# jhollowed/PyTEMDiags

Hardware: AMD Instinct MI355X
Metric: grid-points/sec through full TEM pipeline (ncol*nlev*nt) (higher is better)
Workload: dtype f64; 1 GPU; ne120 (777602 cols) x 72 lev x 30 snapshots per GPU, L=50, 1-degree zonal grid (M=180), ten GM16 Table-A1 outputs; ncol=777602, nlev=72, nt=30, sweeps=latitude-class, single sweep, mirror_paired_sweeps=True

## Files before the change

### include/temx.h

```cpp
#ifndef TEMX_H
#define TEMX_H

#include <stdint.h>

#ifdef __cplusplus
extern "C" {
#endif

typedef struct temx_plan temx_plan;

enum { TEMX_F64 = 0, TEMX_F32 = 1 };

enum {
  TEMX_OK = 0,
  TEMX_EINVAL = -1,
  TEMX_EHIP = -2,
  TEMX_ENOMEM = -3,
  TEMX_ERANK = -4,
  TEMX_ESTATE = -5,
  TEMX_EUNSUPPORTED = -6,
  TEMX_EINTERNAL = -7
};

enum {
  TEMX_DEFER_FINALIZE = 1,
  TEMX_NO_SYMMETRY = 2,
  TEMX_NO_CLASSES = 4,
  TEMX_NO_QR = 8,
  TEMX_LAT_TOL_F32 = 16
};

enum {
  TEMX_OPT_FORM = 1,
  TEMX_OPT_OS_MAP = 2,
  TEMX_OPT_OP_MAP = 3,
  TEMX_OPT_OS_SUBSAMPLE = 4,
  TEMX_OPT_TRACER_ONE_PASS = 5,
  TEMX_OPT_SINGLE_SWEEP_MIN_GROUPS = 6,
  TEMX_OPT_OS_CONTRACT = 7,
  TEMX_OPT_MISSING = 8,
  TEMX_OPT_MIN_COVERAGE = 9,
  TEMX_OPT_MISSING_WEIGHT = 10,
  TEMX_OPT_LAT_BINS = 12,
  TEMX_OPT_BIN_DEGREE = 13,
  TEMX_OPT_OS_SYNC = 11
};
enum {
  TEMX_FORM_AUTO = -1,
  TEMX_FORM_TWO_PASS = 0,
  TEMX_FORM_CLASS_SUMS = 1,
  TEMX_FORM_SINGLE_SWEEP = 2,
  TEMX_FORM_NO_SINGLE_SWEEP = 3,
  TEMX_FORM_MASKED = 4,
  TEMX_FORM_BINNED = 5
};

enum {
  TEMX_MAT_Y0 = 0,
  TEMX_MAT_Y0P = 1,
  TEMX_MAT_GRAM = 2,
  TEMX_MAT_GINV = 3,
  TEMX_MAT_Y0INV = 4,
  TEMX_MAT_GRAM2 = 5,
  TEMX_MAT_GX = 6,
  TEMX_MAT_GSUB = 7,
  TEMX_MAT_COVERAGE = 8
};

enum {
  TEMX_R_VTEM = 0, TEMX_R_OMEGATEM, TEMX_R_WTEM, TEMX_R_PSITEM, TEMX_R_EPFY, TEMX_R_EPFZ,
  TEMX_R_EPDIV, TEMX_R_UTENDEPFD, TEMX_R_UTENDVTEM, TEMX_R_UTENDWTEM, TEMX_NRESULTS
};

enum {
  TEMX_Z_UB = 0, TEMX_Z_VB, TEMX_Z_THETAB, TEMX_Z_WAPB, TEMX_Z_UPVPB, TEMX_Z_UPWAPPB,
  TEMX_Z_VPTPB, TEMX_Z_DUB_DP, TEMX_Z_DTHETAB_DP, TEMX_Z_UBCOSLAT, TEMX_Z_DUBCOSLAT_DLAT,
  TEMX_Z_PSI, TEMX_Z_PSICOSLAT, TEMX_Z_DPSICOSLAT_DLAT, TEMX_Z_DPSI_DP, TEMX_Z_INT_VBDP,
  TEMX_NZONAL
};

enum {
  TEMX_E_UP = 0, TEMX_E_VP, TEMX_E_THETAP, TEMX_E_WAPP, TEMX_E_UPVP, TEMX_E_UPWAPP, TEMX_E_VPTP,
  TEMX_NEDDY
};

int temx_version(void);
const char* temx_last_error(void);
int temx_device_count(void);

int temx_plan_create(temx_plan** out, int device, int64_t ncol, int L, int M,
                     const double* lat_deg_host, const double* lat_out_deg_host, int flags);

int temx_plan_finalize(temx_plan* plan, const double* G_host );

int temx_plan_refine(temx_plan* plan, const double* G2_host );

int temx_plan_set_weights(temx_plan* plan, const double* weights_host );

void temx_plan_destroy(temx_plan* plan);

int temx_plan_is_paired(const temx_plan* plan);
int temx_plan_sweep_mode(const temx_plan* plan);
int temx_plan_one_pass(const temx_plan* plan);
int temx_plan_single_sweep(const temx_plan* plan);

int temx_get_matrix(temx_plan* plan, int which, double* dst, void* stream);

int temx_plan_configure(temx_plan* plan, int option, int value);
int temx_plan_option(const temx_plan* plan, int option);

int temx_plan_set_os_matrices(temx_plan* plan, const double* Gx_host , const double* Gsub_host );


int temx_project(temx_plan* plan, const void* A, int dtype, int64_t D, double* B, void* stream);

int temx_zonal_mean(temx_plan* plan, const void* A, int dtype, int64_t D, double* out,
                    int native, void* stream);

int temx_zonal_mean_from_sums(temx_plan* plan, const double* B, int64_t D, double* out,
                              int native, void* stream);

int temx_plan_set_tem(temx_plan* plan, int nlev, int64_t nt, const double* p_pa_host, double p0);

int temx_tem_stage1(temx_plan* plan, const void* ua, const void* va, const void* ta,
                    const void* wap, int dtype, double* B4, void* stream);

int temx_tem_stage2(temx_plan* plan, const void* ua, const void* va, const void* ta,
                    const void* wap, int dtype, const double* B4, double* B3, void* stream);

int temx_tem_stage2_from_sums(temx_plan* plan, const double* B4, double* B3, void* stream);

int temx_tem_stage3(temx_plan* plan, const double* B3, double* results, double* zonal,
                    void* stream);

int temx_tem_run(temx_plan* plan, const void* ua, const void* va, const void* ta,
                 const void* wap, int dtype, double* results, double* zonal, void* stream);

int temx_tem_os_prepass(temx_plan* plan, const void* ua, const void* va, const void* ta, const void* wap, int dtype,
                        double* As, void* stream);
int temx_tem_os_sweep(temx_plan* plan, const void* ua, const void* va, const void* ta, const void* wap, int dtype,
                      const double* As, int nslices, double* proj, void* stream);
int temx_tem_os_tail(temx_plan* plan, const double* proj_slice, int64_t t0, int64_t nts, double* results,
                     double* zonal, void* stream);
int temx_tracers_os_prepass(temx_plan* plan, int nq, const void* const* q_host, const void* va, const void* wap,
                            int dtype, double* Asq, void* stream);
int temx_tracers_os_sweep(temx_plan* plan, int nq, const void* const* q_host, const void* va, const void* wap,
                          int dtype, const double* Asq, int nslices, double* projq, void* stream);
int temx_tracers_os_tail(temx_plan* plan, int nq, const double* projq_slice, double* const* tres_host,
                         double* const* tzon_host, void* stream);

int temx_tem_tail_from_sums(temx_plan* plan, const double* B4s, const double* B3s, int64_t t0, int64_t nts,
                            double* results, double* zonal, void* stream);
int temx_time_slices(temx_plan* plan, const double* B, int64_t rows, int nslices, double* out, void* stream);

int temx_tem_eddy(temx_plan* plan, const void* ua, const void* va, const void* ta,
                  const void* wap, int dtype, double* const* eddy_ptrs_host, void* stream);

int temx_tem_eddy_rows(temx_plan* plan, const void* ua, const void* va, const void* ta, const void* wap,
                       int dtype, int64_t row0, int64_t nrows, double* const* eddy_ptrs_host ,
                       void* stream);

enum { TEMX_T_ETFY = 0, TEMX_T_ETFZ, TEMX_T_ETDIV, TEMX_T_QTENDETFD, TEMX_T_QTENDVTEM, TEMX_T_QTENDWTEM,
       TEMX_NTRES };
enum { TEMX_TZ_QB = 0, TEMX_TZ_QPVPB, TEMX_TZ_QPWAPPB, TEMX_TZ_DQB_DP, TEMX_TZ_QBCOSLAT,
       TEMX_TZ_DQBCOSLAT_DLAT, TEMX_NTZON };
int temx_tracer_stage1(temx_plan* plan, const void* q, int dtype, double* Bq, void* stream);
int temx_tracer_stage2(temx_plan* plan, const void* q, const void* va, const void* wap, int dtype,
                       const double* Bq, double* Bq2, void* stream);
int temx_tracer_stage3(temx_plan* plan, const double* Bq2, double* tres, double* tzon, void* stream);
int temx_tracer_stage1_sums(temx_plan* plan, const void* q, const void* va, const void* wap, int dtype,
                            double* Bq, void* stream);
int temx_tracer_stage2_from_sums(temx_plan* plan, const double* Bq, double* Bq2, void* stream);
int temx_tracer_run(temx_plan* plan, const void* q, const void* va, const void* wap, int dtype,
                    double* tres, double* tzon, void* stream);
int temx_tracers_run(temx_plan* plan, int nq, const void* const* q_host, const void* va, const void* wap, int dtype,
                     double* const* tres_host, double* const* tzon_host, void* stream);
int temx_tem_tracer_stage1(temx_plan* plan, const void* ua, const void* va, const void* ta, const void* wap,
                           const void* q, int dtype, double* B4, double* Bq, void* stream);
int temx_tem_tracer_run(temx_plan* plan, const void* ua, const void* va, const void* ta, const void* wap,
                        const void* q, int dtype, double* results, double* zonal, double* tres, double* tzon,
                        void* stream);
int temx_tracer_eddy(temx_plan* plan, const void* q, const void* va, const void* wap, int dtype,
                     double* const* ptrs3_host, void* stream);

int temx_status(temx_plan* plan, int* nonfinite, void* stream);


int temx_synth_fields(int device, int64_t ncol, int nlev, int64_t nt, int64_t t0,
                      const double* lat_deg, const double* lon_deg, const double* plev_hpa,
                      int dtype, uint64_t seed, void* ua, void* va, void* ta, void* wap,
                      void* stream);

int temx_mfma_f64_peak(int device, int iters, double* tflops_out);

int temx_kernel_timing(temx_plan* plan, int enable);
int temx_kernel_timing_read(temx_plan* plan, int which, double* avg_ms, int* launches);

// ... 7 lines not shown
```

### pytemdiags_amd/_lib.py

```python
from __future__ import annotations

import ctypes as C
import os

_HERE = os.path.dirname(os.path.abspath(__file__))
LIB_PATH = os.environ.get("TEMX_LIB") or os.path.join(_HERE, "libtemx.so")

ABI_VERSION = 402
F64, F32 = 0, 1
DEFER_FINALIZE = 1
NO_SYMMETRY = 2
NO_CLASSES = 4
NO_QR = 8
LAT_TOL_F32 = 16
MAT_Y0, MAT_Y0P, MAT_GRAM, MAT_GINV, MAT_Y0INV, MAT_GRAM2, MAT_GX, MAT_GSUB = 0, 1, 2, 3, 4, 5, 6, 7
MAT_COVERAGE = 8
OPT_FORM, OPT_OS_MAP, OPT_OP_MAP, OPT_OS_SUBSAMPLE, OPT_TRACER_ONE_PASS, OPT_SINGLE_SWEEP_MIN_GROUPS, OPT_OS_CONTRACT = 1, 2, 3, 4, 5, 6, 7
OPT_MISSING, OPT_MIN_COVERAGE, OPT_MISSING_WEIGHT = 8, 9, 10
OPT_OS_SYNC = 11
OPT_LAT_BINS, OPT_BIN_DEGREE = 12, 13
LAT_BINS_ALLOWED = (128, 256, 512, 1024, 2048)
LAT_BINS_DEFAULT = 512
MISSING_MODES = {"raise": 0, "mask": 1}
FORM_AUTO, FORM_TWO_PASS, FORM_CLASS_SUMS, FORM_SINGLE_SWEEP, FORM_NO_SINGLE_SWEEP = -1, 0, 1, 2, 3
FORM_MASKED = 4
FORM_BINNED = 5
FORM_NAMES = {FORM_TWO_PASS: "two-pass", FORM_CLASS_SUMS: "class-sums", FORM_SINGLE_SWEEP: "single-sweep",
              FORM_MASKED: "masked", FORM_BINNED: "binned"}
FORMS = {"auto": FORM_AUTO, "two-pass": FORM_TWO_PASS, "class-sums": FORM_CLASS_SUMS,
         "single-sweep": FORM_SINGLE_SWEEP, "no-single-sweep": FORM_NO_SINGLE_SWEEP}

RESULT_NAMES = ("vtem", "omegatem", "wtem", "psitem", "epfy", "epfz", "epdiv",
                "utendepfd", "utendvtem", "utendwtem")
ZONAL_NAMES = ("ub", "vb", "thetab", "wapb", "upvpb", "upwappb", "vptpb", "dub_dp", "dthetab_dp",
               "ubcoslat", "dubcoslat_dlat", "psi", "psicoslat", "dpsicoslat_dlat", "dpsi_dp",
               "int_vbdp")
EDDY_NAMES = ("up", "vp", "thetap", "wapp", "upvp", "upwapp", "vptp")
TRACER_RESULT_NAMES = ("etfy", "etfz", "etdiv", "qtendetfd", "qtendvtem", "qtendwtem")
TRACER_ZONAL_NAMES = ("qb", "qpvpb", "qpwappb", "dqb_dp", "qbcoslat", "dqbcoslat_dlat")
TRACER_EDDY_NAMES = ("qp", "qpvp", "qpwapp")

ERRORS = {0: "TEMX_OK", -1: "TEMX_EINVAL", -2: "TEMX_EHIP", -3: "TEMX_ENOMEM", -4: "TEMX_ERANK",
          -5: "TEMX_ESTATE", -6: "TEMX_EUNSUPPORTED", -7: "TEMX_EINTERNAL"}

_vp, _i, _i64, _dp, _u64 = C.c_void_p, C.c_int, C.c_int64, C.POINTER(C.c_double), C.c_uint64
SIGNATURES = [
    ("temx_version", _i, []),
    ("temx_last_error", C.c_char_p, []),
    ("temx_device_count", _i, []),
    ("temx_plan_create", _i, [C.POINTER(_vp), _i, _i64, _i, _i, _dp, _dp, _i]),
    ("temx_plan_finalize", _i, [_vp, _dp]),
    ("temx_plan_refine", _i, [_vp, _dp]),
    ("temx_plan_set_weights", _i, [_vp, _dp]),
    ("temx_plan_destroy", None, [_vp]),
    ("temx_plan_is_paired", _i, [_vp]),
    ("temx_plan_sweep_mode", _i, [_vp]),
    ("temx_plan_one_pass", _i, [_vp]),
    ("temx_plan_single_sweep", _i, [_vp]),
    ("temx_get_matrix", _i, [_vp, _i, _vp, _vp]),
    ("temx_plan_configure", _i, [_vp, _i, _i]),
    ("temx_plan_option", _i, [_vp, _i]),
    ("temx_plan_set_os_matrices", _i, [_vp, _dp, _dp]),
    ("temx_project", _i, [_vp, _vp, _i, _i64, _vp, _vp]),
    ("temx_zonal_mean", _i, [_vp, _vp, _i, _i64, _vp, _i, _vp]),
    ("temx_zonal_mean_from_sums", _i, [_vp, _vp, _i64, _vp, _i, _vp]),
    ("temx_plan_set_tem", _i, [_vp, _i, _i64, _dp, C.c_double]),
    ("temx_tem_stage1", _i, [_vp, _vp, _vp, _vp, _vp, _i, _vp, _vp]),
    ("temx_tem_stage2", _i, [_vp, _vp, _vp, _vp, _vp, _i, _vp, _vp, _vp]),
    ("temx_tem_stage2_from_sums", _i, [_vp, _vp, _vp, _vp]),
    ("temx_tem_stage3", _i, [_vp, _vp, _vp, _vp, _vp]),
    ("temx_tem_run", _i, [_vp, _vp, _vp, _vp, _vp, _i, _vp, _vp, _vp]),
    ("temx_tem_os_prepass", _i, [_vp, _vp, _vp, _vp, _vp, _i, _vp, _vp]),
    ("temx_tem_os_sweep", _i, [_vp, _vp, _vp, _vp, _vp, _i, _vp, _i, _vp, _vp]),
    ("temx_tem_os_tail", _i, [_vp, _vp, _i64, _i64, _vp, _vp, _vp]),
    ("temx_tracers_os_prepass", _i, [_vp, _i, C.POINTER(_vp), _vp, _vp, _i, _vp, _vp]),
    ("temx_tracers_os_sweep", _i, [_vp, _i, C.POINTER(_vp), _vp, _vp, _i, _vp, _i, _vp, _vp]),
    ("temx_tracers_os_tail", _i, [_vp, _i, _vp, C.POINTER(_vp), C.POINTER(_vp), _vp]),
    ("temx_tracers_run", _i, [_vp, _i, C.POINTER(_vp), _vp, _vp, _i, C.POINTER(_vp), C.POINTER(_vp), _vp]),
    ("temx_tem_tail_from_sums", _i, [_vp, _vp, _vp, _i64, _i64, _vp, _vp, _vp]),
    ("temx_time_slices", _i, [_vp, _vp, _i64, _i, _vp, _vp]),
    ("temx_tem_eddy", _i, [_vp, _vp, _vp, _vp, _vp, _i, C.POINTER(_vp), _vp]),
    ("temx_tem_eddy_rows", _i, [_vp, _vp, _vp, _vp, _vp, _i, _i64, _i64, C.POINTER(_vp), _vp]),
    ("temx_tracer_stage1", _i, [_vp, _vp, _i, _vp, _vp]),
    ("temx_tracer_stage2", _i, [_vp, _vp, _vp, _vp, _i, _vp, _vp, _vp]),
    ("temx_tracer_stage3", _i, [_vp, _vp, _vp, _vp, _vp]),
    ("temx_tracer_stage1_sums", _i, [_vp, _vp, _vp, _vp, _i, _vp, _vp]),
    ("temx_tracer_stage2_from_sums", _i, [_vp, _vp, _vp, _vp]),
    ("temx_tracer_run", _i, [_vp, _vp, _vp, _vp, _i, _vp, _vp, _vp]),
    ("temx_tem_tracer_stage1", _i, [_vp, _vp, _vp, _vp, _vp, _vp, _i, _vp, _vp, _vp]),
    ("temx_tem_tracer_run", _i, [_vp, _vp, _vp, _vp, _vp, _vp, _i, _vp, _vp, _vp, _vp, _vp]),
    ("temx_tracer_eddy", _i, [_vp, _vp, _vp, _vp, _i, C.POINTER(_vp), _vp]),
    ("temx_status", _i, [_vp, C.POINTER(_i), _vp]),
    ("temx_synth_fields", _i, [_i, _i64, _i, _i64, _i64, _vp, _vp, _vp, _i, _u64, _vp, _vp, _vp, _vp, _vp]),
    ("temx_mfma_f64_peak", _i, [_i, _i, _dp]),
    ("temx_kernel_timing", _i, [_vp, _i]),
    ("temx_kernel_timing_read", _i, [_vp, _i, _dp, C.POINTER(_i)]),
    ("temx_selftest_exception", _i, [_i]),
]


class TemxError(RuntimeError):
    def __init__(self, code, msg):
        super().__init__("%s (%d): %s" % (ERRORS.get(code, "TEMX_E?"), code, msg))
        self.code = code


_lib = None


def load():
    global _lib
    if _lib is not None:
        return _lib
    if not os.path.exists(LIB_PATH):
        raise RuntimeError(
            "pytemdiags_amd: HIP extension %s is missing. Build it with `make -C pytemdiags_amd/csrc` "
            "or `python -c 'import __graft_entry__ as g; g.build()'`. There is no CPU fallback." % LIB_PATH)
    try:
        import torch
    except ImportError:
        pass
    lib = C.CDLL(LIB_PATH)
    ab_build = "TEMX_LIB" in os.environ
    lib.temx_version.restype = _i
    have = int(lib.temx_version())
    if have != ABI_VERSION:
        msg = "pytemdiags_amd: %s reports ABI version %d, these bindings expect %d" % (LIB_PATH, have, ABI_VERSION)
        if not ab_build:
            raise RuntimeError(msg + "; rebuild it (make -C pytemdiags_amd/csrc)")
        import warnings
        warnings.warn(msg + " (TEMX_LIB build: continuing)")
    for name, res, args in SIGNATURES:
        if ab_build and not hasattr(lib, name):
            def _missing(*_a, _n=name):
                raise TemxError(-6, "symbol %s is missing in the TEMX_LIB build %s" % (_n, LIB_PATH))
            setattr(lib, name, _missing)
            continue
        fn = getattr(lib, name)
        fn.restype = res
        fn.argtypes = args
    _lib = lib
    return lib


_bound = {}


def bind(signatures, version_symbol, expected, header):
    if version_symbol not in _bound:
        lib = load()
        for name, res, args in signatures:
            fn = getattr(lib, name)
            fn.restype = res
            fn.argtypes = args
        have = int(getattr(lib, version_symbol)())
        if have != expected:
            raise RuntimeError("pytemdiags_amd: %s reports %s version %d, these bindings expect %d; rebuild it "
                               "(make -C pytemdiags_amd/csrc)" % (LIB_PATH, header, have, expected))
        _bound[version_symbol] = lib
    return _bound[version_symbol]


def check(rc):
    if rc != 0:
        raise TemxError(rc, load().temx_last_error().decode("utf-8", "replace"))
```

### pytemdiags_amd/csrc/kernels.hpp

```cpp
#pragma once
#include <hip/hip_runtime.h>
#include <stdint.h>

#include <type_traits>

#define TEMX_MFMA4(a, b, c) __builtin_amdgcn_mfma_f64_4x4x4f64((a), (b), (c), 0, 0, 0)

namespace temx {

template <int NF>
struct FieldPtrs {
  const void* p[NF];
};

struct EddyOut {
  double* p[7];
};

template <int KMAX>
__device__ __forceinline__ void basis_row(double xv, int K, const double* __restrict__ norm,
                                          const double* __restrict__ T, double* q) {
  double pm1 = 1.0, pc = xv;
  for (int l = 0; l < K; ++l) {
    double P;
// ... 89 lines not shown
    for (int t = 0; t < TB; ++t) acc[f][t] = 0.0;

  constexpr int YE = 4 * TB * 16;
  constexpr int YJ = (YE + 255) / 256;
  T xn[PD][NFW][4];
  double ys[YJ];
  const int nfull = (int)(N >> 4);
  auto load_x = [&](int chunk, auto slotc, int ti, auto fastc) __attribute__((always_inline)) {
    constexpr int slot = decltype(slotc)::value;
    const int64_t gb = (int64_t)chunk * 16 + ti * 4;
    if (decltype(fastc)::value) {
#pragma unroll
      for (int f = 0; f < NFW; ++f) xn[slot][f][ti] = (fb[f] + gb * D)[loff];
    } else {
      int64_t row = gb + g;
      row = row < N ? row : N - 1;
#pragma unroll
      for (int f = 0; f < NFW; ++f) xn[slot][f][ti] = fb[f][row * D + dcl];
    }
  };
  uint32_t yso[YJ];
#pragma unroll
  for (int j = 0; j < YJ; ++j) {
    const int li = tid + 256 * j;
    const int gi = li / (TB * 16), rem = li % (TB * 16);
    yso[j] = (uint32_t)((gi < 4 ? gi : 3) * gstride * 16 + tb_off * 16 + rem);
  }
  const int64_t ychunk = (int64_t)4 * gstride * 16;
  auto load_ys = [&](int chunk) __attribute__((always_inline)) {
#pragma unroll
    for (int j = 0; j < YJ; ++j) ys[j] = (yblk + (int64_t)chunk * ychunk)[yso[j]];
  };
  auto do_chunk = [&](int chunk, auto slotc, auto fastc) __attribute__((always_inline)) {
    constexpr bool FAST = decltype(fastc)::value;
    constexpr int slot = decltype(slotc)::value;
    double* yst = ystage[(chunk - c0) & 1];
#pragma unroll
    for (int j = 0; j < YJ; ++j)
      if (tid + 256 * j < YE) yst[tid + 256 * j] = ys[j];
    __syncthreads();
    if (FAST || chunk + 1 < c1) load_ys(chunk + 1);
    const bool more = FAST || chunk + PD < c1;
    if (active) {
#pragma unroll
      for (int ti = 0; ti < 4; ++ti) {
        double xs[NFW];
#pragma unroll
        for (int f = 0; f < NFW; ++f) xs[f] = (double)xn[slot][f][ti] * sc[f];
        if (more) load_x(chunk + PD, slotc, ti, fastc);
#pragma unroll
        for (int t = 0; t < TB; ++t) {
          const double ya = yst[(ti * TB + t) * 16 + yoff];
#pragma unroll
          for (int f = 0; f < NFW; ++f) acc[f][t] = TEMX_MFMA4(ya, xs[f], acc[f][t]);
        }
      }
    }
  };
  auto do_group = [&](int chunk, auto fastc) __attribute__((always_inline)) {
    do_chunk(chunk, std::integral_constant<int, 0>{}, fastc);
    if (PD > 1 && (decltype(fastc)::value || chunk + 1 < c1))
      do_chunk(chunk + 1, std::integral_constant<int, (PD > 1 ? 1 : 0)>{}, fastc);
    if (PD > 2 && (decltype(fastc)::value || chunk + 2 < c1))
      do_chunk(chunk + 2, std::integral_constant<int, (PD > 2 ? 2 : 0)>{}, fastc);
  };

  if (c0 < c1) {
    load_ys(c0);
    if (active) {
#pragma unroll
      for (int ti = 0; ti < 4; ++ti) load_x(c0, std::integral_constant<int, 0>{}, ti, std::false_type{});
      if (PD > 1 && c0 + 1 < c1) {
#pragma unroll
        for (int ti = 0; ti < 4; ++ti)
          load_x(c0 + 1, std::integral_constant<int, (PD > 1 ? 1 : 0)>{}, ti, std::false_type{});
      }
      if (PD > 2 && c0 + 2 < c1) {
#pragma unroll
        for (int ti = 0; ti < 4; ++ti)
          load_x(c0 + 2, std::integral_constant<int, (PD > 2 ? 2 : 0)>{}, ti, std::false_type{});
      }
    }
  }
  const int cfast = (c1 < nfull ? c1 : nfull) - (2 * PD - 1);
  int chunk = c0;
  for (; chunk < cfast; chunk += PD) do_group(chunk, std::true_type{});
  for (; chunk < c1; chunk += PD) do_group(chunk, std::false_type{});

  if (dvalid) {
#pragma unroll
    for (int f = 0; f < NFW; ++f)
#pragma unroll
      for (int t = 0; t < TB; ++t) {
        const int l = t * 4 + g;
        if (l < K) partial[(((int64_t)split * NF + f0 + f) * K + l) * D + d] = acc[f][t];
      }
  }
}

struct SliceMap {
  int64_t D = 0;
  int nt = 1, W = 1;
  int64_t chunk = 0;
  int64_t row0 = 0;
};
__device__ __forceinline__ int64_t slice_index(const SliceMap& m, int64_t idx) {
  if (m.D == 0) return idx;
  const int64_t row = idx / m.D, d = idx - row * m.D;
  const int lev = (int)(d / m.nt), t = (int)(d - (int64_t)lev * m.nt);
  const int base = m.nt / m.W, extra = m.nt - base * m.W, tb = extra * (base + 1);
  int w, tl, ntw;
  if (t < tb) { w = t / (base + 1); tl = t - w * (base + 1); ntw = base + 1; }
  else { const int u = t - tb; w = extra + u / base; tl = u - (w - extra) * base; ntw = base; }
  const int nlev = (int)(m.D / m.nt);
  return (int64_t)w * m.chunk + ((m.row0 + row) * nlev + lev) * ntw + tl;
}

__global__ void __launch_bounds__(256)
reduce_partials_kernel(const double* __restrict__ partial, int nsplit, int64_t stride, int64_t n,
                       const double* __restrict__ addend, double* __restrict__ B, int* __restrict__ flag,
                       SliceMap map) {
  __shared__ double sh[16][17];
  const int e = threadIdx.x & 15, sl = threadIdx.x >> 4;
  const int64_t idx = (int64_t)blockIdx.x * 16 + e;
  double s = 0.0;
  if (idx < n)
    for (int sp = sl; sp < nsplit; sp += 16) s += partial[(int64_t)sp * stride + idx];
  sh[sl][e] = s;
  __syncthreads();
  if (sl == 0 && idx < n) {
    double t = 0.0;
#pragma unroll
    for (int j = 0; j < 16; ++j) t += sh[j][e];
    if (addend != nullptr) t += addend[idx];
    B[slice_index(map, idx)] = t;
    if (!(fabs(t) <= 1.79769313486231570815e308)) atomicOr(flag, 1);
  }
}

template <int NS>
__global__ void __launch_bounds__(256)
reduce_partials_flat_kernel(const double* __restrict__ partial, int nsplit, int64_t stride, int64_t n,
                            const double* __restrict__ addend, double* __restrict__ B, int* __restrict__ flag,
                            SliceMap map) {
  const int64_t idx = (int64_t)blockIdx.x * 256 + threadIdx.x;
  if (idx >= n) return;
  double v[NS];
#pragma unroll
  for (int sp = 0; sp < NS; ++sp) v[sp] = partial[(int64_t)(sp < nsplit ? sp : 0) * stride + idx];
  double t = 0.0;
#pragma unroll
  for (int sp = 0; sp < NS; ++sp) t += sp < nsplit ? v[sp] : 0.0;
  if (addend != nullptr) t += addend[idx];
  B[slice_index(map, idx)] = t;
  if (!(fabs(t) <= 1.79769313486231570815e308)) atomicOr(flag, 1);
}

__global__ void __launch_bounds__(256)
reduce_rows_kernel(const double* __restrict__ partial, int nsplit, int64_t stride, int nf, int rows_in, int rows,
                   int64_t D, double* __restrict__ out, int* __restrict__ flag) {
  const int64_t idx = (int64_t)blockIdx.x * 256 + threadIdx.x;
  const int64_t per = (int64_t)rows * D;
  if (idx >= per * nf) return;
  const int64_t f = idx / per, rem = idx - f * per;
  const double* src = partial + f * rows_in * D + rem;
  double t = 0.0;
  for (int sp = 0; sp < nsplit; ++sp) t += src[(int64_t)sp * stride];
  out[idx] = t;
  if (!(fabs(t) <= 1.79769313486231570815e308)) atomicOr(flag, 1);
}
__global__ void __launch_bounds__(256)
reduce_rows_wide_kernel(const double* __restrict__ partial, int nsplit, int64_t stride, int nf, int rows_in, int rows,
                        int64_t D, double* __restrict__ out, int* __restrict__ flag) {
  __shared__ double sh[16][17];
  const int e = threadIdx.x & 15, sl = threadIdx.x >> 4;
  const int64_t idx = (int64_t)blockIdx.x * 16 + e;
  const int64_t per = (int64_t)rows * D;
  const bool ok = idx < per * nf;
  double s = 0.0;
  if (ok) {
    const int64_t f = idx / per, rem = idx - f * per;
    const double* src = partial + f * rows_in * D + rem;
    for (int sp = sl; sp < nsplit; sp += 16) s += src[(int64_t)sp * stride];
  }
  sh[sl][e] = s;
  __syncthreads();
  if (sl == 0 && ok) {
    double t = 0.0;
#pragma unroll
    for (int j = 0; j < 16; ++j) t += sh[j][e];
    out[idx] = t;
    if (!(fabs(t) <= 1.79769313486231570815e308)) atomicOr(flag, 1);
  }
}

__global__ void __launch_bounds__(1024)
solve_kernel(const double* __restrict__ B, int K, int K4, int M, int64_t D,
             const double* __restrict__ Ginv, const double* __restrict__ Y0p,
             double* __restrict__ C, double* __restrict__ Xb) {
  extern __shared__ double slds[];
  double* sb = slds;
  double* scf = slds + (size_t)K4 * 17;
  const int f = blockIdx.y;
  const int64_t d0 = (int64_t)blockIdx.x * 16;
  const int tid = threadIdx.x;
  const int mper = (M + gridDim.z - 1) / gridDim.z;
  const int m0 = blockIdx.z * mper;
  const int m1 = m0 + mper < M ? m0 + mper : M;
  for (int idx = tid; idx < K * 16; idx += 1024) {
    const int k = idx >> 4, dd = idx & 15;
    const int64_t d = d0 + dd;
    sb[k * 17 + dd] = d < D ? B[((int64_t)f * K + k) * D + d] : 0.0;
  }
  __syncthreads();
  for (int idx = tid; idx < K4 * 16; idx += 1024) {
    const int k = idx >> 4, dd = idx & 15;
    const int64_t d = d0 + dd;
    double v = 0.0;
    if (k < K) {
      const double* gr = Ginv + (int64_t)k * K;
      double v0 = 0.0, v1 = 0.0, v2 = 0.0, v3 = 0.0;
      int kk = 0;
      for (; kk + 4 <= K; kk += 4) {
        v0 += gr[kk] * sb[kk * 17 + dd];
        v1 += gr[kk + 1] * sb[(kk + 1) * 17 + dd];
        v2 += gr[kk + 2] * sb[(kk + 2) * 17 + dd];
        v3 += gr[kk + 3] * sb[(kk + 3) * 17 + dd];
      }
      for (; kk < K; ++kk) v0 += gr[kk] * sb[kk * 17 + dd];
      v = (v0 + v1) + (v2 + v3);
    }
    scf[k * 17 + dd] = v;
    if (C != nullptr && blockIdx.z == 0 && d < D) C[((int64_t)f * K4 + k) * D + d] = v;
  }
  __syncthreads();
  if (Xb != nullptr) {
    for (int idx = tid; idx < (m1 - m0) * 16; idx += 1024) {
      const int m = m0 + (idx >> 4), dd = idx & 15;
      const int64_t d = d0 + dd;
      if (d >= D) continue;
      const double* yr = Y0p + (int64_t)m * K;
      double v0 = 0.0, v1 = 0.0, v2 = 0.0, v3 = 0.0;
      int kk = 0;
      for (; kk + 4 <= K; kk += 4) {
        v0 += yr[kk] * scf[kk * 17 + dd];
        v1 += yr[kk + 1] * scf[(kk + 1) * 17 + dd];
        v2 += yr[kk + 2] * scf[(kk + 2) * 17 + dd];
        v3 += yr[kk + 3] * scf[(kk + 3) * 17 + dd];
      }
      for (; kk < K; ++kk) v0 += yr[kk] * scf[kk * 17 + dd];
      Xb[((int64_t)f * M + m) * D + d] = (v0 + v1) + (v2 + v3);
    }
  }
}

constexpr int SOLVE_MB = 16;

template <int TB>
__global__ void __launch_bounds__(256)
solve_mfma_kernel(const double* __restrict__ B, int K, int M, int64_t D, const double* __restrict__ gblk,
                  const double* __restrict__ ypblk, double* __restrict__ C, double* __restrict__ Xb,
                  int mbs ) {
  extern __shared__ double slds[];
  double* sg = slds;
  double* sy = slds + TB * TB * 16;
  const int f = blockIdx.y;
  const int tid = threadIdx.x, lane = tid & 63, wave = tid >> 6;
  const int g = lane >> 4, c = lane & 15;
  const int64_t d = ((int64_t)blockIdx.x * 4 + wave) * 16 + c;
  const bool dvalid = d < D;
  const int64_t dcl = dvalid ? d : D - 1;
  const int mb0 = blockIdx.z * mbs;
  const int nmb_all = (M + 3) >> 2;
  const int nmb = Xb != nullptr ? (nmb_all - mb0 < mbs ? nmb_all - mb0 : mbs) : 0;

  double breg[TB];
#pragma unroll
  for (int t = 0; t < TB; ++t) {
    const int row = 4 * t + g;
    const int rc = row < K ? row : K - 1;
    const double v = B[((int64_t)f * K + rc) * D + dcl];
    breg[t] = row < K ? v : 0.0;
  }
  {
    constexpr int JG = (TB * TB * 16 + 255) / 256, JY = (SOLVE_MB * TB * 16 + 255) / 256;
    double tg[JG], ty[JY];
    const double* yp = ypblk + (int64_t)mb0 * TB * 16;
    const int ny = nmb * TB * 16;
#pragma unroll
    for (int j = 0; j < JG; ++j) tg[j] = gblk[tid + 256 * j < TB * TB * 16 ? tid + 256 * j : 0];
#pragma unroll
    for (int j = 0; j < JY; ++j) ty[j] = yp[tid + 256 * j < ny ? tid + 256 * j : 0];
#pragma unroll
    for (int j = 0; j < JG; ++j)
      if (tid + 256 * j < TB * TB * 16) sg[tid + 256 * j] = tg[j];
#pragma unroll
    for (int j = 0; j < JY; ++j)
      if (tid + 256 * j < ny) sy[tid + 256 * j] = ty[j];
  }
  __syncthreads();

  const uint32_t yoff = (uint32_t)(g * 4 + (lane & 3));
  double creg[TB];
#pragma unroll
  for (int r = 0; r < TB; ++r) creg[r] = 0.0;
#pragma unroll
// ... 618 lines not shown
```

### pytemdiags_amd/csrc/kernels_osc.hpp

```cpp
#pragma once
#include "kernels_op2.hpp"

namespace temx {

struct OscMats {
  const double* Tt;
  const double* G2inv;
  const double* T;
  const double* Gk;
  const double* YqK;
  const double* Yq;
  const double* YqKt;
  const double* Yqt;
  const double* Gx;
};

#ifndef TEMX_OSC_PF
#define TEMX_OSC_PF 4
#endif
constexpr int OSC_PF = TEMX_OSC_PF;

#ifndef TEMX_OSC_W
#define TEMX_OSC_W 4
#endif
constexpr int OSC_W = TEMX_OSC_W;

typedef double osc_d4 __attribute__((ext_vector_type(4)));

template <int MO, int KI, typename Init, typename Out>
__device__ __forceinline__ void osc_mm(const double* __restrict__ blk, int wave, const double* xl, int lane,
                                       Init init, Out out) {
  constexpr int MO16 = (MO + 3) / 4;
  constexpr int MC = (MO16 + OSC_W - 1) / OSC_W;
  constexpr int PF = OSC_PF < KI ? OSC_PF : KI;
  osc_d4 acc[MC];
  double ring[PF][MC];
  const double* __restrict__ b[MC];
#pragma unroll
  for (int j = 0; j < MC; ++j) {
    const int MB = wave + j * OSC_W < MO16 ? wave + j * OSC_W : MO16 - 1;
    b[j] = blk + (size_t)MB * KI * 64 + lane;
#pragma unroll
    for (int i = 0; i < 4; ++i) {
      const int mb = 4 * MB + i;
      acc[j][i] = mb < MO ? init(mb) : 0.0;
    }
  }
  static_for<PF - 1>([&](auto pc) __attribute__((always_inline)) {
    constexpr int p = decltype(pc)::value;
#pragma unroll
    for (int j = 0; j < MC; ++j) ring[p][j] = b[j][p * 64];
  });
  auto step = [&](auto jc, int k) __attribute__((always_inline)) {
    constexpr int r = decltype(jc)::value;
    const int kn = k + PF - 1 < KI ? k + PF - 1 : KI - 1;
#pragma unroll
    for (int j = 0; j < MC; ++j) ring[(r + PF - 1) % PF][j] = b[j][kn * 64];
    const double x = xl[k * 64];
#pragma unroll
    for (int j = 0; j < MC; ++j) acc[j] = __builtin_amdgcn_mfma_f64_16x16x4f64(ring[r][j], x, acc[j], 0, 0, 0);
  };
  constexpr int TRIPS = KI / PF, REM = KI % PF;
#pragma unroll 1
  for (int t = 0; t < TRIPS; ++t)
    static_for<PF>([&](auto jc) __attribute__((always_inline)) { step(jc, t * PF + decltype(jc)::value); });
  static_for<REM>([&](auto jc) __attribute__((always_inline)) { step(jc, TRIPS * PF + decltype(jc)::value); });
#pragma unroll
  for (int j = 0; j < MC; ++j)
    if (wave + j * OSC_W < MO16) {
#pragma unroll
      for (int i = 0; i < 4; ++i) {
        const int mb = 4 * (wave + j * OSC_W) + i;
        if (mb < MO) out(mb, acc[j][i]);
      }
    }
}

struct OscFieldsIn {
  const double* A[4];
  const double* rho[4];
};

__host__ __device__ constexpr int osc_fields_lds(int NBK) { return (2 * NBK + 2 * NBK + 4) * 64; }
__host__ __device__ constexpr int osc_pairs_lds(int NBK) { return (3 * 2 * NBK + 2 * NBK) * 64; }

template <int NBK>
__global__ void __launch_bounds__(OSC_W * 64)
osc_fields_kernel(OscFieldsIn in, OscMats m, int K, int KX, int KR, int NQ, int64_t Dt, int nout,
                  double* __restrict__ B4 , double* __restrict__ At ,
                  double* __restrict__ ab , int64_t Drho, int nts, int nt, int t0) {
  constexpr int NBX = 2 * NBK;
  extern __shared__ double sm[];
  const int f = blockIdx.y;
  const int lane = threadIdx.x & 63, wave = threadIdx.x >> 6;
  const int g = lane >> 4, c = lane & 15;
  const int64_t d = (int64_t)blockIdx.x * 16 + c;
  const bool dvalid = d < Dt;
  const int64_t dcl = dvalid ? d : Dt - 1;
  double* va = sm + lane;
  double* vt0 = va + NBX * 64;
  double* vt1 = vt0 + NBK * 64;
  double* vr = vt1 + NBK * 64;
  const double* __restrict__ Af = in.A[f];
  for (int kb = wave; kb < NBX; kb += OSC_W) {
    const int row = 4 * kb + g;
    const double v = Af[(int64_t)(row < KX ? row : KX - 1) * Dt + dcl];
    va[kb * 64] = row < KX ? v : 0.0;
  }
  if (wave == 0 && f < nout) {
    const int64_t lev = dcl / nts, dg = lev * nt + t0 + (dcl - lev * nts);
#pragma unroll
    for (int kb = 0; kb < 4; ++kb) {
      const int row = 4 * kb + g;
      const double v = in.rho[f][(int64_t)(row < KR ? row : KR - 1) * Drho + dg];
      vr[kb * 64] = row < KR ? v : 0.0;
    }
  }
  __syncthreads();
  auto zero = [](int) { return 0.0; };
  if (gridDim.z == 2 && blockIdx.z == 1) {
    osc_mm<NBX, NBX>(m.Yq, wave, va, lane, zero, [&](int mb, double v) {
      if (dvalid && 4 * mb + g < NQ) At[((int64_t)f * NQ + 4 * mb + g) * Dt + d] = v;
    });
    return;
  }
  osc_mm<NBK, NBK>(m.Tt, wave, va, lane, zero, [&](int mb, double v) { vt0[mb * 64] = v; });
  __syncthreads();
  osc_mm<NBK, NBK>(m.G2inv, wave, vt0, lane, zero, [&](int mb, double v) { vt1[mb * 64] = v; });
  __syncthreads();
  osc_mm<NBK, NBK>(m.T, wave, vt1, lane, zero, [&](int mb, double v) { vt0[mb * 64] = v; });
  __syncthreads();
  if (f < nout) {
    osc_mm<NBK, 4>(m.Gk, wave, vr, lane, [&](int mb) { return va[mb * 64]; }, [&](int mb, double v) { vt1[mb * 64] = v; });
    __syncthreads();
    osc_mm<NBK, NBK>(m.Tt, wave, vt1, lane, zero, [&](int mb, double v) {
      if (dvalid && 4 * mb + g < K) B4[((int64_t)f * K + 4 * mb + g) * Dt + d] = v;
    });
  }
  osc_mm<NBX, NBK>(m.YqK, wave, vt0, lane, zero, [&](int mb, double v) {
    if (dvalid && 4 * mb + g < NQ) ab[((int64_t)f * NQ + 4 * mb + g) * Dt + d] = v;
  });
  if (gridDim.z == 1)
    osc_mm<NBX, NBX>(m.Yq, wave, va, lane, zero, [&](int mb, double v) {
      if (dvalid && 4 * mb + g < NQ) At[((int64_t)f * NQ + 4 * mb + g) * Dt + d] = v;
    });
}

struct OscPairsIn {
  const double* At_a[4];
  const double* At_b[4];
  const double* ab_a[4];
  const double* ab_b[4];
  const double* P[4];
};

template <int NBK>
__global__ void __launch_bounds__(OSC_W * 64)
osc_pairs_kernel(OscPairsIn in, OscMats m, const double* __restrict__ wq2, int K, int KX, int NQ, int64_t Dt,
                 double* __restrict__ B3 ) {
  constexpr int NBX = 2 * NBK;
  extern __shared__ double sm[];
  const int p = blockIdx.y;
  const int lane = threadIdx.x & 63, wave = threadIdx.x >> 6;
  const int g = lane >> 4, c = lane & 15;
  const int64_t d = (int64_t)blockIdx.x * 16 + c;
  const bool dvalid = d < Dt;
  const int64_t dcl = dvalid ? d : Dt - 1;
  double* vU = sm + lane;
  double* vV = vU + NBX * 64;
  double* vc = vV + NBX * 64;
  double* vx = vc + NBX * 64;
  double* vF = vx + NBK * 64;
  const double* __restrict__ Ata = in.At_a[p];
  const double* __restrict__ Atb = in.At_b[p];
  const double* __restrict__ aba = in.ab_a[p];
  const double* __restrict__ abb = in.ab_b[p];
  for (int kb = wave; kb < NBX; kb += OSC_W) {
    const int q = 4 * kb + g;
    const int qc = q < NQ ? q : NQ - 1;
    const double w = q < NQ ? wq2[qc] : 0.0;
    const int64_t o = (int64_t)qc * Dt + dcl;
    const double ta = Ata[o], tb = Atb[o], aa = aba[o], bb = abb[o];
    vU[kb * 64] = w * (bb * ta + aa * tb);
    vV[kb * 64] = w * (aa * bb);
  }
  __syncthreads();
  auto zero = [](int) { return 0.0; };
  osc_mm<NBK, NBX>(m.YqKt, wave, vU, lane, zero, [&](int mb, double v) { vx[mb * 64] = v; });
  osc_mm<NBX, NBX>(m.Yqt, wave, vV, lane, zero, [&](int mb, double v) { vc[mb * 64] = v; });
  __syncthreads();
  const double* __restrict__ Pp = in.P[p];
  osc_mm<NBK, NBX>(m.Gx, wave, vc, lane,
                   [&](int mb) {
                     const int row = 4 * mb + g;
                     const double v = Pp[(int64_t)(row < K ? row : K - 1) * Dt + dcl];
                     return (row < K ? v : 0.0) - vx[mb * 64];
                   },
                   [&](int mb, double v) { vF[mb * 64] = v; });
  __syncthreads();
  osc_mm<NBK, NBK>(m.Tt, wave, vF, lane, zero, [&](int mb, double v) {
    if (dvalid && 4 * mb + g < K) B3[((int64_t)p * K + 4 * mb + g) * Dt + d] = v;
  });
}

}
```

### pytemdiags_amd/csrc/temx.hip

```cpp
#include "../../include/temx.h"
#include "../../include/temx_vert.h"
#include "../../include/temx_layout.h"
#include "../../include/temx_ingest.h"
#include "../../include/temx_clim.h"
#include "../../include/temx_mtracer.h"
#include "../../include/temx_nclim.h"
#include "../../include/temx_gclim.h"
#include "../include/temx_mgclim.h"
#include "../include/temx_wave.h"

#include <hip/hip_runtime.h>

#include <algorithm>
#include <cmath>
#include <cstdarg>
#include <cstdio>
#include <cstdlib>
#include <cstring>
#include <map>
#include <mutex>
#include <new>
#include <stdexcept>
#include <string>
#include <thread>
#include <atomic>
#include <vector>

#include "kernels.hpp"
#include "kernels_sym.hpp"
#include "kernels_cls.hpp"
#include "kernels_op.hpp"
#include "kernels_op2.hpp"
#include "kernels_osc.hpp"
#include "kernels_miss.hpp"
#include "kernels_mtracer.hpp"
#include "kernels_bin.hpp"
#include "kernels_vert.hpp"
#include "kernels_layout.hpp"
#include "kernels_ingest.hpp"
#include "kernels_clim.hpp"
#include "kernels_nclim.hpp"
#include "kernels_gclim.hpp"
#include "kernels_mgclim.hpp"
#include "kernels_wave.hpp"
#include "bin_tables.hpp"
#include "class_tables.hpp"
#include "clim_shapes.hpp"
#include "nclim_shapes.hpp"
#include "dispatch.hpp"
#include "field_args.hpp"
#include "gclim_tables.hpp"
#include "host_math.hpp"
#include "launch_shapes.hpp"
#include "mgclim_shapes.hpp"
#include "wave_tables.hpp"

using namespace temx;

static thread_local std::string g_err;

static int fail(int code, const char* fmt, ...) {
  char buf[512];
  va_list ap;
  va_start(ap, fmt);
  vsnprintf(buf, sizeof buf, fmt, ap);
  va_end(ap);
  g_err = buf;
  return code;
}

#define HIPCHK(expr)                                                                     \
  do {                                                                                   \
    hipError_t e_ = (expr);                                                              \
    if (e_ != hipSuccess) {                                                              \
      (void)hipGetLastError();                                                           \
      return fail(e_ == hipErrorOutOfMemory ? TEMX_ENOMEM : TEMX_EHIP, "%s failed: %s",  \
                  #expr, hipGetErrorString(e_));                                         \
    }                                                                                    \
  } while (0)

#define ARGCHK(expr) \
  do { if (const Refusal r_ = (expr)) return fail(r_.code, "%s", r_.msg); } while (0)

struct DevBuf {
  void* p = nullptr;
  size_t bytes = 0;
  int ensure(size_t need) {
    if (need <= bytes) return TEMX_OK;
    if (p) (void)hipFree(p);
    p = nullptr;
    bytes = 0;
    hipError_t e = hipMalloc(&p, need);
    if (e != hipSuccess) return fail(TEMX_ENOMEM, "hipMalloc(%zu) failed: %s", need, hipGetErrorString(e));
    bytes = need;
    return TEMX_OK;
  }
  void release() {
    if (p) (void)hipFree(p);
    p = nullptr;
    bytes = 0;
  }
  double* d() const { return static_cast<double*>(p); }
};

struct TimedLaunch {
  hipEvent_t a, b;
};

struct temx_plan {
  int device = 0, num_cu = 256;
  int64_t N = 0, nchunk = 0;
  int L = 0, K = 0, TB = 0, K4 = 0, M = 0;
  int stride = 0, nslice = 1;
  bool large = false;
  DevBuf Bs, XB, P3;
  bool finalized = false;
  bool weighted = false;
  int rank = 0;
  DevBuf x, Y0, yblk, yblk_w, Y0p, G, Ginv, norm, flag;
  DevBuf gblk, ypblk;
  bool qbasis = false;
  bool g_checker = false;
  bool ext_G = false;
  bool os_need_global = false;
  DevBuf T, Qp, GinvA, G2, xo, xc;
  int64_t cls_npad = 0;
  const double* yproj_ptr() const { return yblk_w.p ? yblk_w.d() : yblk.d(); }
  std::vector<double> lat_out_deg;
  bool tem = false;
  int nlev = 0;
  int64_t nt = 0, D = 0;
  double p0 = 101325.0;
  DevBuf p, pg, lg, coslat, fcor, colscale;
  DevBuf B4, B3, C4, zb;
  DevBuf Bq, Bq2, Ct, tz;
  Split sp_proj1;
  bool sym = false;
  int TBS = 0;
  int64_t npair = 0, npg = 0, npg_alloc = 0;
  DevBuf rows, ysym;
  Split sp_sproj4, sp_sproj1, sp_seddy;
  Split sp_proj4, sp_eddy;
  bool cls = false;
  int64_t cgroups = 0, cbatches = 0, ncls = 0;
  int64_t cls_max_side = 0;
  std::vector<int> gbatch0;
  DevBuf crow, ycls;
  std::map<int, DevBuf> csplits;
  Split sp_cproj4, sp_cproj1, sp_ceddy, sp_cflux;
  bool os_built = false, os_on = false;
  bool os_valid = false;
  DevBuf Axq, rho_t;
  int TBX = 0, KX = 0, KR = 0, NQ = 0;
  std::vector<double> h_xc, h_cnt;
  std::vector<int> h_crow;
  std::vector<int> sgbatch0;
  int64_t sgroups = 0, sbatches = 0;
  DevBuf ycx, ycx_s, crow_s, rho, rho0, gaunt , wq2, Gx, Gsinv, Ax , Axs ;
  std::vector<double> h_G_own;
  std::vector<double> h_Gx_own;
  std::vector<double> h_Gx, h_Gs;
  std::vector<double> h_T, h_Ginv, h_G, h_Yq;
  DevBuf oscblk, osAt, osAb, osAtq, osAbq, Bqp;
  OscMats osc{};
  bool osc_lds = false;
  int opt_os_contract = -1;
  bool os_barrier = false;
  int opt_os_sync = -1;
  int os_keep = 32;
  int64_t tD = 0, tnt = 0, tt0 = 0;
  int opt_form = -1, opt_os_map = -1, opt_op_map = -1, opt_tracer_one_pass = -1, opt_single_sweep_min_groups = -1;
  bool os_tile = false, op_tile = false;
  bool no_qr = false;
  DevBuf side_crow[2][2], side_gfirst[2][2];
  std::map<int, DevBuf> csplits_s;
  Split sp_os, sp_os_s;
  Split sp_copw;
  bool lcls = false, lone = false, xb_valid = false;
  DevBuf ycls_l, pbuf;
  int64_t ycls_lstride = 0;
  Split sp_lflux;
  bool onepass = false, op_valid = false;
  bool c4_valid = false;
  DevBuf csum, ccnt;
  DevBuf Pq;
  DevBuf csq, Pq2;
  bool tq_valid = false;
  DevBuf partial;
  DevBuf opB, opC;
  int opt_missing = 0, opt_min_cov = 500, opt_miss_w = 10;
  bool miss_built = false;
  bool miss_valid = false;
  int64_t miss_cov_D = -1;
  int NE = 0, NQM = 0;
  DevBuf eblk;
  DevBuf mtab;
  DevBuf mB, mC, mCcov, mcov, mZ;
  bool mt_valid = false;
  DevBuf mtB, mtB2, mtC, mtCcov, mtz;
  int opt_lat_bins = 0;
  int bin_J = 0, bin_KP = 0;
  int bin_built = 0;
  int bin_pass = 0;
  int64_t bin_nchunk = 0;
  std::vector<double> h_lat;
  DevBuf bin_a, bin_chunk, bin_c0, bin_rows, bin_s;
  DevBuf bin_T;
  DevBuf bin_cm, bin_z, bin_cy;
  bool timing = false;
  std::vector<TimedLaunch> timed[2];
};

static int upload(DevBuf& b, const void* src, size_t bytes) {
  int rc = b.ensure(bytes);
  if (rc) return rc;
  HIPCHK(hipMemcpy(b.p, src, bytes, hipMemcpyHostToDevice));
  return TEMX_OK;
}

__global__ void fill_zero_kernel(double2* __restrict__ p, int64_t n) {
  const double2 z = make_double2(0.0, 0.0);
  for (int64_t i = blockIdx.x * (int64_t)blockDim.x + threadIdx.x; i < n; i += (int64_t)gridDim.x * blockDim.x) p[i] = z;
}

static int alloc_write_stream(DevBuf& b, size_t need) {
  need = (need + 15) & ~(size_t)15;
  if (b.bytes >= need) return TEMX_OK;
  int tries = 4;
  if (const char* e = getenv("TEMX_PLACE_TRIES")) tries = std::max(1, std::min(8, atoi(e)));
  if (need < ((size_t)1 << 30)) tries = 1;
  b.release();
  std::vector<DevBuf> cand;
  std::vector<float> ms;
  hipEvent_t ea = nullptr, eb = nullptr;
  if (tries > 1 && (hipEventCreate(&ea) != hipSuccess || hipEventCreate(&eb) != hipSuccess)) tries = 1;
  int best = -1;
  float slowest = 0.f;
  for (int t = 0; t < tries; ++t) {
    size_t fr = 0, tot = 0;
    if (t > 0 && (hipMemGetInfo(&fr, &tot) != hipSuccess || need > fr / 2)) break;
    DevBuf c;
    if (c.ensure(need) != TEMX_OK) {
      if (t == 0) return TEMX_ENOMEM;
      break;
    }
    float best_ms = 1e30f;
    for (int rep = 0; rep < (tries > 1 ? 2 : 1); ++rep) {
      if (ea) (void)hipEventRecord(ea, nullptr);
      hipLaunchKernelGGL(fill_zero_kernel, dim3(2048), dim3(256), 0, nullptr, static_cast<double2*>(c.p), (int64_t)(need / 16));
      if (ea) {
        float m = 0.f;
        (void)hipEventRecord(eb, nullptr);
        if (hipEventSynchronize(eb) == hipSuccess && hipEventElapsedTime(&m, ea, eb) == hipSuccess) best_ms = std::min(best_ms, m);
      }
    }
    cand.push_back(c);
    ms.push_back(best_ms);
    if (best < 0 || best_ms < ms[(size_t)best]) best = t;
    slowest = std::max(slowest, best_ms);
    if ((double)need / (best_ms * 1e-3) >= 6.1e12 || ms[(size_t)best] < 0.92f * slowest) break;
  }
  if (ea) (void)hipEventDestroy(ea);
  if (eb) (void)hipEventDestroy(eb);
  HIPCHK(hipDeviceSynchronize());
  HIPCHK(hipGetLastError());
  for (size_t i = 0; i < cand.size(); ++i)
    if ((int)i == best) b = cand[i]; else cand[i].release();
  return TEMX_OK;
}

static int lds_attr_once(std::atomic<uint64_t>& done, int device, const void* fn, int bytes) {
  const uint64_t bit = 1ull << (device & 63);
  if (done.load(std::memory_order_acquire) & bit) return TEMX_OK;
  HIPCHK(hipFuncSetAttribute(fn, hipFuncAttributeMaxDynamicSharedMemorySize, bytes));
  done.fetch_or(bit, std::memory_order_release);
  return TEMX_OK;
}

template <auto Kern>
static std::atomic<uint64_t> lds_attr_done{0};

template <auto Kern, typename... A>
__attribute__((noinline))
static int launch(dim3 grid, dim3 block, size_t lds_bytes, hipStream_t st, A... args) {
  hipLaunchKernelGGL(Kern, grid, block, lds_bytes, st, args...);
  HIPCHK(hipGetLastError());
  return TEMX_OK;
}
template <auto Kern, int attr_bytes = 0, typename... A>
static int launch_lds(int device, dim3 grid, dim3 block, size_t lds_bytes, hipStream_t st, A... args) {
  const int limit = attr_bytes ? attr_bytes : (int)lds_bytes;
  if (int rc = lds_attr_once(lds_attr_done<Kern>, device, reinterpret_cast<const void*>(Kern), limit)) return rc;
  return launch<Kern>(grid, block, lds_bytes, st, args...);
}

static int bad_dtype() { return fail(TEMX_EINVAL, "dtype must be TEMX_F64 or TEMX_F32"); }
template <typename F>
static int by_dtype(int dtype, F&& f) {
  int rc = TEMX_OK;
  return dispatch_dtype(dtype, rc, f) ? rc : bad_dtype();
}

template <typename F>
static int by_basis_rows(int K, F&& f) { return K <= 64 ? f(Int<64>{}) : f(Int<512>{}); }

template <typename T>
static int upload(DevBuf& b, const std::vector<T>& v) { return upload(b, v.data(), v.size() * sizeof(T)); }
static int os_upload_blocks(temx_plan* pl);

static int set_ginv(temx_plan* pl, const double* Gi_host) {
  HIPCHK(hipMemcpy(pl->Ginv.p, Gi_host, (size_t)pl->K * pl->K * 8, hipMemcpyHostToDevice));
  pl->h_Ginv.assign(Gi_host, Gi_host + (size_t)pl->K * pl->K);
  if (pl->os_built)
    if (int rc = os_upload_blocks(pl)) return rc;
  if (pl->K > 64) return TEMX_OK;
  std::vector<double> Gp((size_t)4 * pl->TB * pl->K, 0.0);
  std::copy(Gi_host, Gi_host + (size_t)pl->K * pl->K, Gp.begin());
  return upload(pl->gblk, pack_blocks4(Gp.data(), 4 * pl->TB, pl->K, pl->TB));
}

constexpr size_t kMaxTimedLaunches = 256;

static void time_begin(temx_plan* pl, int which, hipStream_t st, TimedLaunch& tl) {
  tl.a = tl.b = nullptr;
  if (!pl->timing || pl->timed[which].size() >= kMaxTimedLaunches) return;
  (void)hipEventCreate(&tl.a);
  (void)hipEventCreate(&tl.b);
  (void)hipEventRecord(tl.a, st);
}
static void time_end(temx_plan* pl, int which, hipStream_t st, TimedLaunch& tl) {
  if (!pl->timing || tl.a == nullptr) return;
  (void)hipEventRecord(tl.b, st);
  pl->timed[which].push_back(tl);
}

struct ProjCfgC { static constexpr int NFW = 4, PD = 1, WPS = 2; };
struct ProjCfgE { static constexpr int NFW = 1, PD = 2, WPS = 3; };
struct ProjCfg1 { static constexpr int NFW = 1, PD = 2, WPS = 2; };

static int pick_dpw(int ndt, int maxdpw) {
  int best = maxdpw;
  double bw = 1e9;
  for (int d = maxdpw; d >= 1; d >>= 1) {
    const double w = (double)(((ndt + d - 1) / d) * d) / ndt;
    if (w < bw - 0.05) {
      bw = w;
      best = d;
    }
  }
  return best;
}
static int proj_dpw(int NF, int ndt) {
  if (NF == 1) return 4;
  return pick_dpw(ndt, 4) == 1 ? 1 : 4;
}
static int proj_wps(int NF, int dpw) {
  if (NF == 1) return ProjCfg1::WPS;
  return dpw == 1 ? ProjCfgE::WPS : ProjCfgC::WPS;
}

constexpr int SYM_PROJ_E_WPS = 3;
struct ProjCfg3 { static constexpr int NFW = 3, PD = 1, WPS = 2; };

template <int NF>
static int launch_project(temx_plan* pl, const FieldPtrs<NF>& fp, int dtype, int64_t D,
                          const double* colscale, int sfield, double* partial, const Split& sp,
                          hipStream_t st, int tb_off = 0, int Kloc = -1) {
  if (Kloc < 0) Kloc = pl->K;
  return by_dtype(dtype, [&](auto t) {
    using T = typename decltype(t)::type;
    auto go = [&](auto cfg) {
      using Cfg = decltype(cfg);
      return dispatch(TBValues{}, pl->TB, [&](auto tb) {
        return launch<project_kernel<T, NF, Cfg::NFW, decltype(tb)::value, Cfg::PD, Cfg::WPS>>(
            dim3(sp.grid), dim3(256), 0, st, fp, pl->N, D, Kloc, pl->yproj_ptr(), pl->stride, tb_off, pl->nchunk, colscale,
            sfield, partial, sp.nsplit, sp.ndt);
      });
    };
    if constexpr (NF == 1) return go(ProjCfg1{});
    else if constexpr (NF == 3) return go(ProjCfg3{});
    else return sp.dpw == 1 ? go(ProjCfgE{}) : go(ProjCfgC{});
  });
}

static int launch_reduce(temx_plan* pl, const double* partial, int nsplit, int64_t n, double* B,
                         hipStream_t st, int64_t stride = -1, const double* addend = nullptr,
                         const SliceMap& map = SliceMap(), int* flag = nullptr) {
  if (stride < 0) stride = n;
  if (flag == nullptr) flag = static_cast<int*>(pl->flag.p);
  if (nsplit <= 16 && n >= 32768) {
    const dim3 grid((unsigned)((n + 255) / 256));
    if (nsplit <= 2)
      hipLaunchKernelGGL(reduce_partials_flat_kernel<2>, grid, dim3(256), 0, st, partial, nsplit, stride, n, addend, B, flag, map);
    else if (nsplit <= 4)
      hipLaunchKernelGGL(reduce_partials_flat_kernel<4>, grid, dim3(256), 0, st, partial, nsplit, stride, n, addend, B, flag, map);
    else if (nsplit <= 8)
      hipLaunchKernelGGL(reduce_partials_flat_kernel<8>, grid, dim3(256), 0, st, partial, nsplit, stride, n, addend, B, flag, map);
    else
      hipLaunchKernelGGL(reduce_partials_flat_kernel<16>, grid, dim3(256), 0, st, partial, nsplit, stride, n, addend, B, flag, map);
    HIPCHK(hipGetLastError());
    return TEMX_OK;
  }
  const int64_t blocks = (n + 15) / 16;
  hipLaunchKernelGGL(reduce_partials_kernel, dim3((unsigned)blocks), dim3(256), 0, st, partial, nsplit, stride, n,
                     addend, B, flag, map);
  HIPCHK(hipGetLastError());
  return TEMX_OK;
}

static int launch_reduce_rows(temx_plan* pl, const double* partial, int nsplit, int64_t stride, int nf, int rows_in,
                              int rows, int64_t D, double* out, hipStream_t st) {
  const int64_t n = (int64_t)nf * rows * D;
  if (nsplit > 16)
    hipLaunchKernelGGL(reduce_rows_wide_kernel, dim3((unsigned)((n + 15) / 16)), dim3(256), 0, st, partial, nsplit, stride,
                       nf, rows_in, rows, D, out, static_cast<int*>(pl->flag.p));
  else
    hipLaunchKernelGGL(reduce_rows_kernel, dim3((unsigned)((n + 255) / 256)), dim3(256), 0, st, partial, nsplit, stride,
                       nf, rows_in, rows, D, out, static_cast<int*>(pl->flag.p));
  HIPCHK(hipGetLastError());
  return TEMX_OK;
}

static int launch_solve(temx_plan* pl, const double* B, int NF, int64_t D, double* C, double* Xb,
                        hipStream_t st) {
  if (pl->K <= 64) {
    const int nmb = (pl->M + 3) / 4;
    const int gx = (int)(((D + 15) / 16 + 3) / 4);
    int mbs = SOLVE_MB;
    while (mbs > 4 && (int64_t)gx * NF * ((nmb + mbs - 1) / mbs) < pl->num_cu / 2) mbs -= 4;
    dim3 grid((unsigned)gx, NF, Xb ? (nmb + mbs - 1) / mbs : 1);
    return dispatch(TBValues{}, pl->TB, [&](auto tb) {
      constexpr int TBv = decltype(tb)::value;
      const size_t slds = ((size_t)TBv * TBv + (size_t)SOLVE_MB * TBv) * 16 * sizeof(double);
      return launch_lds<solve_mfma_kernel<TBv>>(pl->device, grid, dim3(256), slds, st, B, pl->K, pl->M, D, pl->gblk.d(),
                                                pl->ypblk.d(), C, Xb, mbs);
    });
  }
  const int ms = Xb ? (pl->M + 63) / 64 : 1;
  dim3 grid((unsigned)((D + 15) / 16), NF, ms);
  const size_t slds = (size_t)2 * pl->K4 * 17 * sizeof(double);
  return launch_lds<solve_kernel, 160 * 1024>(pl->device, grid, dim3(1024), slds, st, B, pl->K, pl->K4, pl->M, D,
      pl->Ginv.d(), pl->Qp.d(), C, Xb);
}

template <typename T, int MODE, int KIND>
static int launch_eddy_t(temx_plan* pl, const FieldPtrs<4>& fp, const double* C, double* partial,
                         const Split& sp, const EddyOut& eo, hipStream_t st) {
  constexpr int NFR = (KIND == 1 || KIND == 3) ? 3 : 4;
  return dispatch(DpwValues{}, sp.dpw, [&](auto dpw) {
    return dispatch(TBValues{}, pl->TB, [&](auto tb) {
      constexpr int DPW = decltype(dpw)::value, TBv = decltype(tb)::value;
      const size_t lds = ((size_t)DPW * NFR * TBv * 64 + 8 * EDDY_GR * TBv * 16) * sizeof(double);
      return launch_lds<eddy_kernel<T, TBv, MODE, DPW, KIND>>(pl->device, dim3(sp.grid), dim3(512), lds, st, fp, pl->N, pl->D,
                                                              pl->K, pl->yblk.d(), pl->nchunk, pl->colscale.d(), C, partial,
                                                              sp.nsplit, sp.ndt, eo);
    });
  });
}

static int launch_recon(temx_plan* pl, int64_t D, const double* C, double* out, hipStream_t st,
                        int64_t row0 = 0, int64_t nrows = -1) {
  if (nrows < 0) nrows = pl->N - row0;
  const int64_t nch = (nrows + 15) / 16;
  const double* yb0 = pl->yblk.d() + (row0 / 4) * pl->stride * 16;
  Split sp = choose_split(D, nch, 2 * pl->num_cu);
  dim3 grid(sp.grid), block(256);
  if (pl->large) {
    for (int sl = 0; sl < pl->nslice; ++sl)
      hipLaunchKernelGGL(recon_kernel<16>, grid, block, (size_t)4 * 16 * 64 * sizeof(double), st, nrows, D, yb0, pl->stride,
          16 * sl, nch, C + (int64_t)64 * sl * D, out, sl > 0 ? 1 : 0, sp.nsplit, sp.ndt);
    HIPCHK(hipGetLastError());
    return TEMX_OK;
  }
  return dispatch(TBValues{}, pl->TB, [&](auto tb) {
    constexpr int TBv = decltype(tb)::value;
    return launch<recon_kernel<TBv>>(grid, block, (size_t)4 * TBv * 64 * sizeof(double), st, nrows, D, yb0, pl->stride, 0,
        nch, C, out, 0, sp.nsplit, sp.ndt);
  });
}

template <int NF>
static int project_all(temx_plan* pl, const FieldPtrs<NF>& fp, int dtype, int64_t D, const double* colscale,
                       int sfield, const Split& sp, double* B, hipStream_t st) {
  int rc;
  if (!pl->large) {
    if ((rc = launch_project<NF>(pl, fp, dtype, D, colscale, sfield, pl->partial.d(), sp, st))) return rc;
    return launch_reduce(pl, pl->partial.d(), sp.nsplit, (int64_t)NF * pl->K * D, B, st);
  }
  if ((rc = pl->Bs.ensure((size_t)NF * 64 * D * 8))) return rc;
  for (int sl = 0; sl < pl->nslice; ++sl) {
    const int Ks = std::min(64, pl->K - 64 * sl);
    if ((rc = launch_project<NF>(pl, fp, dtype, D, colscale, sfield, pl->partial.d(), sp, st, 16 * sl, Ks))) return rc;
    if ((rc = launch_reduce(pl, pl->partial.d(), sp.nsplit, (int64_t)NF * Ks * D, pl->Bs.d(), st))) return rc;
    for (int f = 0; f < NF; ++f)
      HIPCHK(hipMemcpyAsync(B + ((int64_t)f * pl->K + 64 * sl) * D, pl->Bs.d() + (int64_t)f * Ks * D,
                            (size_t)Ks * D * 8, hipMemcpyDeviceToDevice, st));
  }
  return TEMX_OK;
}

static double sym_tol_deg(double dflt) {
  double tol = dflt;
  if (const char* e = getenv("TEMX_SYM_TOL_DEG")) {
    const double t = atof(e);
    if (t > 0.0 && t < 1e-3) tol = t;
  }
  return tol;
}

static int cached_cuts(std::map<int, DevBuf>& cache, const std::vector<int>& gbatch0, int64_t ngroups, int64_t nbatches,
                       int nsub, bool group_aligned, const int2** out) {
  const int key = group_aligned ? -nsub : nsub;
  auto it = cache.find(key);
  if (it == cache.end()) {
    DevBuf b;
    if (int rc = upload(b, work_cuts(gbatch0, ngroups, nbatches, nsub, group_aligned))) return rc;
    it = cache.emplace(key, b).first;
  }
  *out = static_cast<const int2*>(it->second.p);
  return TEMX_OK;
}
static int class_cuts_dev(temx_plan* pl, int nsub, const int2** out, bool group_aligned = false) {
  return cached_cuts(pl->csplits, pl->gbatch0, pl->cgroups, pl->cbatches, nsub, group_aligned, out);
}
static int os_cuts_dev(temx_plan* pl, bool sub, int nsub, const int2** out) {
  if (!sub) return class_cuts_dev(pl, nsub, out, true);
  return cached_cuts(pl->csplits_s, pl->sgbatch0, pl->sgroups, pl->sbatches, nsub, true, out);
}

#ifndef TEMX_CLS_E_WPS
#define TEMX_CLS_E_WPS 3
#endif
#ifndef TEMX_CLS_E_PD
#define TEMX_CLS_E_PD 2
#endif
#ifndef TEMX_CLS_OP_WPS
#define TEMX_CLS_OP_WPS 1
#endif
#ifndef TEMX_CLS_OP_PD
#define TEMX_CLS_OP_PD 3
#endif
#ifndef TEMX_CLS_MINCHUNK
#define TEMX_CLS_MINCHUNK 1
#endif
#ifndef TEMX_CLS_OP_PD_F32
#define TEMX_CLS_OP_PD_F32 6
#endif
#ifndef TEMX_CLS_E_PD_F32
#define TEMX_CLS_E_PD_F32 4
#endif
#ifndef TEMX_CLS_Q_PD_F32
#define TEMX_CLS_Q_PD_F32 2
#endif
constexpr int CLS_PROJ_E_WPS = TEMX_CLS_E_WPS, CLS_PROJ_E_PD = TEMX_CLS_E_PD;
template <typename T>
constexpr int cls_proj_pd(bool op, int nfw) {
  constexpr bool f32 = sizeof(T) == 4;
  return op ? (f32 ? TEMX_CLS_OP_PD_F32 : TEMX_CLS_OP_PD)
            : (nfw == 1 ? (f32 ? TEMX_CLS_E_PD_F32 : CLS_PROJ_E_PD) : (f32 ? TEMX_CLS_Q_PD_F32 : 2));
}

template <int NF>
static int launch_project_cls(temx_plan* pl, const FieldPtrs<NF>& fp, int dtype, int64_t D,
                              const double* colscale, int sfield, double* partial, const Split& sp,
                              hipStream_t st) {
  return by_dtype(dtype, [&](auto t) {
    using T = typename decltype(t)::type;
    const int2* cuts = nullptr;
    if (int rc = class_cuts_dev(pl, sp.nsplit, &cuts)) return rc;
    auto go = [&](auto nfw, auto wps) {
      return dispatch(TBSValues{}, pl->TBS, [&](auto tbs) {
        constexpr int NFW = decltype(nfw)::value, WPS = decltype(wps)::value;
        return launch<project_cls_kernel<T, NF, NFW, decltype(tbs)::value, WPS, cls_proj_pd<T>(false, NFW), false>>(
            dim3(sp.grid), dim3(256), 0, st, fp, D, pl->K, pl->ycls.d(), static_cast<const int4*>(pl->crow.p), cuts, colscale,
            sfield, partial, sp.nsplit, sp.ndt, (double*)nullptr);
      });
    };
    return NF == 1 || sp.dpw == 1 ? go(Int<1>{}, Int<CLS_PROJ_E_WPS>{}) : go(Int<NF>{}, Int<2>{});
  });
}

template <int KIND>
static int launch_sweep_op(temx_plan* pl, const FieldPtrs<4>& fp, int dtype, double* partial, const Split& sp,
                           hipStream_t st) {
  double* sums = KIND == 0 ? pl->csum.d() : pl->csq.d();
  return by_dtype(dtype, [&](auto t) {
    using T = typename decltype(t)::type;
    const int2* cuts = nullptr;
    if (int rc = class_cuts_dev(pl, sp.nsplit, &cuts, true)) return rc;
    dim3 grid(sp.grid), block(256);
    constexpr int PDv = KIND == 1 ? (sizeof(T) == 4 ? 4 : 2) : (sizeof(T) == 4 ? TEMX_CLS_OP_PD_F32 : TEMX_CLS_OP_PD);
    const int64_t wcols = (pl->D + 63) / 64 * 64;
    const bool row_map = sizeof(T) == 8 && !pl->op_tile && wcols * 100 <= pl->D * 115;
    constexpr int PDr = 2;
    return dispatch(TBSValues{}, pl->TBS, [&](auto tbs) {
      constexpr int TBSv = decltype(tbs)::value;
      if (row_map)
        return launch<sweep_opr_kernel<double, TBSv, PDr, KIND>>(grid, block, 0, st, fp, pl->D, pl->K, pl->ycls.d(),
                                                                 static_cast<const int4*>(pl->crow.p), cuts, pl->colscale.d(),
                                                                 partial, sp.nsplit, sp.ndt, sums);
      return launch<sweep_op_kernel<T, TBSv, PDv, KIND>>(grid, block, 0, st, fp, pl->D, pl->K, pl->ycls.d(),
          static_cast<const int4*>(pl->crow.p), cuts, pl->colscale.d(), partial, sp.nsplit, sp.ndt, sums);
    });
  });
}

template <typename T>
static int launch_sweep_opw2_t(temx_plan* pl, const FieldPtrs<5>& fp, double* partial, const Split& sp, hipStream_t st) {
  const int2* cuts = nullptr;
  if (int rc = class_cuts_dev(pl, sp.nsplit * 4, &cuts, true)) return rc;
  dim3 grid(sp.grid), block(256);
  constexpr int PDv = sizeof(T) == 4 ? TEMX_CLS_OP_PD_F32 : TEMX_CLS_OP_PD;
  return dispatch(TBSValues{}, pl->TBS, [&](auto tbs) {
    return launch<sweep_opw_kernel<T, decltype(tbs)::value, PDv, 2>>(grid, block, 0, st, fp, pl->D, pl->K, pl->ycls.d(),
        static_cast<const int4*>(pl->crow.p), cuts, pl->colscale.d(), partial, sp.nsplit, sp.ndt, pl->csum.d(),
        pl->csq.d());
  });
}

template <typename T, int MODE, int KIND>
static int launch_eddy_cls_t(temx_plan* pl, const FieldPtrs<4>& fp, const double* C, double* partial,
                             const Split& sp, const EddyOut& eo, hipStream_t st) {
  constexpr int NFR = KIND == 0 ? 4 : 3;
  return dispatch(DpwValues{}, sp.dpw, [&](auto dpw) {
    constexpr int DPW = decltype(dpw)::value;
    const int2* cuts = nullptr;
    if (int rc = class_cuts_dev(pl, sp.nsplit * (8 / DPW), &cuts)) return rc;
    return dispatch(TBSValues{}, pl->TBS, [&](auto tbs) {
      constexpr int TBSv = decltype(tbs)::value;
      const size_t lds = ((size_t)DPW * NFR * 2 * TBSv * 64 + 8 * 2 * TBSv * 16) * sizeof(double);
      return launch_lds<eddy_cls_kernel<T, TBSv, MODE, DPW, KIND>>(pl->device, dim3(sp.grid), dim3(512), lds, st, fp, pl->D,
          pl->K, pl->K4, pl->ycls.d(), static_cast<const int4*>(pl->crow.p), cuts, pl->colscale.d(), C, partial, sp.nsplit,
          sp.ndt, eo);
    });
  });
}

template <int KIND>
static int launch_flux_cls(temx_plan* pl, const double* C, double* partial, const Split& sp, hipStream_t st) {
  return dispatch(DpwValues{}, sp.dpw, [&](auto dpw) {
    return dispatch(TBSValues{}, pl->TBS, [&](auto tbs) {
      constexpr int DPW = decltype(dpw)::value, TBSv = decltype(tbs)::value;
      const size_t lds = ((size_t)DPW * 4 * 2 * TBSv * 64 + 8 * 2 * TBSv * 16) * sizeof(double);
      return launch_lds<flux_cls_kernel<TBSv, DPW, KIND>>(pl->device, dim3(sp.grid), dim3(512), lds, st, pl->D, pl->K,
          pl->K4, pl->ycls.d(), pl->csum.d(), pl->csq.d(), pl->ccnt.d(), pl->cgroups, C, partial, sp.nsplit, sp.ndt);
    });
  });
}

static int launch_class_sums(temx_plan* pl, const FieldPtrs<4>& fp, int dtype, hipStream_t st) {
  const Split& sp = pl->sp_cproj4;
  const int2* cuts = nullptr;
  if (int rc = class_cuts_dev(pl, sp.nsplit, &cuts, true)) return rc;
  dim3 grid(sp.grid), block(256);
  return by_dtype(dtype, [&](auto t) {
    using T = typename decltype(t)::type;
    return launch<project_cls_kernel<T, 4, 4, 2, TEMX_CLS_OP_WPS, cls_proj_pd<T>(true, 4), true, false>>(grid, block, 0,
        st, fp, pl->D, pl->K, (const double*)nullptr, static_cast<const int4*>(pl->crow.p), cuts, pl->colscale.d(), 2,
        (double*)nullptr, sp.nsplit, sp.ndt, pl->csum.d());
  });
}

template <int NQ>
static int project_sums(temx_plan* pl, const double* rec, int RS, int row0, double* B, hipStream_t st) {
  const Split& sp = pl->sp_cflux;
  const int64_t D = pl->D;
  dim3 grid(sp.grid), block(512);
  int rc;
  for (int sl = 0; sl < pl->nslice; ++sl) {
    const int Ks = std::min(64, pl->K - 64 * sl);
    rc = dispatch(DpwValues{}, sp.dpw, [&](auto dpw) {
      constexpr int DPW = decltype(dpw)::value;
      const size_t lds = ((size_t)DPW * NQ * 16 * 64 + 8 * 256) * sizeof(double);
      return launch_lds<sums_project_kernel<NQ, DPW>>(pl->device, grid, block, lds, st, D, pl->K, 64 * sl,
                                                      pl->ycls_l.d() + sl * pl->ycls_lstride, rec, RS, row0, pl->cgroups,
                                                      pl->partial.d(), sp.nsplit, sp.ndt);
    });
    if (rc) return rc;
    if ((rc = launch_reduce(pl, pl->partial.d(), sp.nsplit, (int64_t)NQ * Ks * D, pl->Bs.d(), st))) return rc;
    for (int q = 0; q < NQ; ++q)
      HIPCHK(hipMemcpyAsync(B + ((int64_t)q * pl->K + 64 * sl) * D, pl->Bs.d() + (int64_t)q * Ks * D,
                            (size_t)Ks * D * 8, hipMemcpyDeviceToDevice, st));
  }
  return TEMX_OK;
}

static int launch_flux_large(temx_plan* pl, const double* C, hipStream_t st) {
  const Split& sp = pl->sp_lflux;
  dim3 grid(sp.grid), block(512);
  return dispatch(SliceValues{}, pl->nslice, [&](auto ns) {
    constexpr int NS = decltype(ns)::value;
    const size_t lds = ((size_t)NS * 4 * 16 * 64 + 8 * 256) * sizeof(double);
    return launch_lds<flux_large_kernel<NS>>(pl->device, grid, block, lds, st, pl->D, pl->K, pl->K4, pl->ycls_l.d(),
        pl->ycls_lstride, pl->csum.d(), pl->ccnt.d(), pl->cgroups, C, pl->pbuf.d(), sp.nsplit, sp.ndt);
  });
}

template <int NF>
static int launch_project_sym(temx_plan* pl, const FieldPtrs<NF>& fp, int dtype, int64_t D,
                              const double* colscale, int sfield, double* partial, const Split& sp,
                              hipStream_t st) {
  return by_dtype(dtype, [&](auto t) {
    using T = typename decltype(t)::type;
    auto go = [&](auto nfw, auto wps) {
      return dispatch(TBSValues{}, pl->TBS, [&](auto tbs) {
        return launch<project_sym_kernel<T, NF, decltype(nfw)::value, decltype(tbs)::value, decltype(wps)::value>>(
            dim3(sp.grid), dim3(256), 0, st, fp, D, pl->K, pl->ysym.d(), static_cast<const int*>(pl->rows.p), pl->npg,
            pl->npg_alloc * 4, colscale, sfield, partial, sp.nsplit, sp.ndt);
      });
    };
    return NF == 4 && sp.dpw == 1 ? go(Int<1>{}, Int<SYM_PROJ_E_WPS>{}) : go(Int<NF>{}, Int<2>{});
  });
}

template <typename T, int MODE, int KIND>
static int launch_eddy_sym_t(temx_plan* pl, const FieldPtrs<4>& fp, const double* C, double* partial,
                             const Split& sp, const EddyOut& eo, hipStream_t st) {
  constexpr int NFR = KIND == 0 ? 4 : 3;
  return dispatch(DpwValues{}, sp.dpw, [&](auto dpw) {
    return dispatch(TBSValues{}, pl->TBS, [&](auto tbs) {
      constexpr int DPW = decltype(dpw)::value, TBSv = decltype(tbs)::value;
      const size_t lds = ((size_t)DPW * NFR * 2 * TBSv * 64 + 8 * 2 * TBSv * 16) * sizeof(double);
      return launch_lds<eddy_sym_kernel<T, TBSv, MODE, DPW, KIND>>(pl->device, dim3(sp.grid), dim3(512), lds, st, fp, pl->D,
          pl->K, pl->K4, pl->ysym.d(), static_cast<const int*>(pl->rows.p), pl->npg, pl->npg_alloc * 4, pl->npair,
          pl->colscale.d(), C, partial, sp.nsplit, sp.ndt, eo);
    });
  });
}

static inline bool unfused_stage2(const temx_plan* pl) { return pl->large || pl->weighted; }

static inline hipStream_t S_(void* s) { return static_cast<hipStream_t>(s); }
static inline const Split& eddy_split(const temx_plan* pl) {
  return pl->cls ? pl->sp_ceddy : (pl->sym ? pl->sp_seddy : pl->sp_eddy);
}
static inline int eddy_slabs(const temx_plan* pl) {
  if (pl->cls) return pl->sp_ceddy.nsplit;
  return eddy_split(pl).nsplit * (8 / eddy_split(pl).dpw);
}
static inline bool sym_project(const temx_plan* pl, int nf) {
  return pl->sym && (nf == 4 ? pl->sp_sproj4.nsplit : pl->sp_sproj1.nsplit) > 0;
}

template <int KIND>
static int run_eddy(temx_plan* pl, const FieldPtrs<4>& fp, int dtype, const double* C, double* partial,
                    const EddyOut* eo, hipStream_t st) {
  const EddyOut none{};
  return by_dtype(dtype, [&](auto t) {
    using T = typename decltype(t)::type;
    auto go = [&](auto mode) {
      constexpr int MODE = decltype(mode)::value;
      const EddyOut& o = MODE ? *eo : none;
      if (pl->cls) return launch_eddy_cls_t<T, MODE, KIND>(pl, fp, C, partial, pl->sp_ceddy, o, st);
      if (pl->sym) return launch_eddy_sym_t<T, MODE, KIND>(pl, fp, C, partial, pl->sp_seddy, o, st);
      return launch_eddy_t<T, MODE, KIND>(pl, fp, C, partial, pl->sp_eddy, o, st);
    };
    return eo ? go(Int<1>{}) : go(Int<0>{});
  });
}

static FieldPtrs<4> four(const void* a, const void* b, const void* c, const void* d) {
  FieldPtrs<4> fp;
  fp.p[0] = a; fp.p[1] = b; fp.p[2] = c; fp.p[3] = d;
  return fp;
}


static int build_os_tables(temx_plan* pl) {
  if (pl->os_built) return TEMX_OK;
  const int K = pl->K, L = pl->L;
  const int KX = 2 * L + 1;
  const int TBX = pl->TBS == 7 ? 13 : (pl->TBS == 4 ? 8 : 4);
  const int KR = std::min(16, K);
  pl->KX = KX;
  pl->TBX = TBX;
  pl->KR = KR;
  int rc;
  const char* ess = getenv("TEMX_OS_SUBSAMPLE");
  const ClassSubsample ss = class_subsample(pl->h_crow, pl->h_xc, pl->gbatch0, pl->cgroups, ess ? std::max(4, atoi(ess)) : pl->os_keep);
  pl->sgbatch0 = ss.gbatch0;
  pl->sgroups = ss.ngroups;
  pl->sbatches = ss.nbatch;
  if ((rc = upload(pl->crow_s, ss.crow))) return rc;
  for (int sub = 0; sub < 2; ++sub) {
    SideTables stb;
    if (sub) build_side_tables(ss.crow, ss.gbatch0, ss.ngroups, stb);
    else build_side_tables(pl->h_crow, pl->gbatch0, pl->cgroups, stb);
    for (int sd = 0; sd < 2; ++sd) {
      if ((rc = upload(pl->side_crow[sub][sd], stb.crow[sd]))) return rc;
      if ((rc = upload(pl->side_gfirst[sub][sd], stb.gfirst[sd]))) return rc;
    }
  }
  {
    std::vector<double> nx((size_t)8 * TBX + 8, 0.0);
    for (int l = 0; l < KX; ++l) nx[(size_t)l] = std::sqrt((2.0 * l + 1.0) / (4.0 * M_PI));
    DevBuf nd, xs;
    if (!(rc = upload(nd, nx)) && !(rc = upload(xs, ss.xc)) && !(rc = pl->ycx.ensure((size_t)(pl->cgroups + 1) * 2 * TBX * 16 * 8)) &&
        !(rc = pl->ycx_s.ensure((size_t)(pl->sgroups + 1) * 2 * TBX * 16 * 8))) {
      hipLaunchKernelGGL(cls_basis_kernel<512>, dim3((unsigned)((pl->cls_npad + 255) / 256)), dim3(256), 0, 0, pl->xc.d(),
                         pl->ncls, pl->cls_npad, KX, TBX, nd.d(), (const double*)nullptr, pl->ycx.d());
      const int64_t np = (pl->sgroups + 1) * 4;
      hipLaunchKernelGGL(cls_basis_kernel<512>, dim3((unsigned)((np + 255) / 256)), dim3(256), 0, 0, xs.d(), pl->sgroups * 4,
                         np, KX, TBX, nd.d(), (const double*)nullptr, pl->ycx_s.d());
      const hipError_t e = hipDeviceSynchronize();
      if (e != hipSuccess) rc = fail(TEMX_EHIP, "extended class basis failed: %s", hipGetErrorString(e));
    }
    nd.release();
    xs.release();
    if (rc) return rc;
  }
  {
    pl->h_Gs = subsample_gram(pl->h_xc, pl->h_cnt, pl->cgroups, ss.S, KR);
    std::vector<long double> Li;
    std::vector<double> Gi((size_t)KR * KR, 0.0);
    if (spd_factor(pl->h_Gs.data(), KR, Li) == 0) {
      inverse_from_factor(Li, KR, Gi.data());
    } else if (pl->ext_G) {
      pl->os_need_global = true;
    } else {
      return fail(TEMX_ERANK, "the subsample of latitude classes does not determine a degree-%d reference", KR - 1);
    }
    if ((rc = upload(pl->Gsinv, Gi))) return rc;
  }
  {
    const int nq = 2 * L + 2;
    pl->NQ = nq;
    const QuadBasis qb = quadrature_basis(nq, KX);
    pl->h_Yq.assign(qb.Y.begin(), qb.Y.end());
    if ((rc = upload(pl->gaunt, pl->h_Yq))) return rc;
    if ((rc = upload(pl->wq2, std::vector<double>(qb.w2.begin(), qb.w2.end())))) return rc;
  }
  pl->h_Gx = extended_gram(pl->h_xc, pl->h_cnt, pl->ncls, K, KX, (int)std::max(1u, std::min(16u, std::thread::hardware_concurrency())));
  pl->h_Gx_own = pl->h_Gx;
  if ((rc = upload(pl->Gx, pl->h_Gx))) return rc;
  pl->os_built = true;
  return os_upload_blocks(pl);
}

static int os_upload_blocks(temx_plan* pl) {
  if (pl->h_T.empty() || pl->h_Ginv.empty() || pl->h_G.empty() || pl->h_Yq.empty() || pl->h_Gx.empty()) return TEMX_OK;
  const int K = pl->K, KX = pl->KX, KR = pl->KR, NQ = pl->NQ;
  const int NBK = pl->TB, NBX = 2 * pl->TBX;
  if (4 * NBK < K || 4 * NBX < KX || 4 * NBX < NQ) return fail(TEMX_EUNSUPPORTED, "single-sweep contraction: no instantiation for L = %d", pl->L);
  std::vector<double> blk;
  size_t off[9];
  const double* T = pl->h_T.data();
  const double* Yq = pl->h_Yq.data();
  off[0] = blk.size(); append_blocks16(blk, T, K, K, K, true, NBK, NBK);
  off[1] = blk.size(); append_blocks16(blk, pl->h_Ginv.data(), K, K, K, false, NBK, NBK);
  off[2] = blk.size(); append_blocks16(blk, T, K, K, K, false, NBK, NBK);
  off[3] = blk.size(); append_blocks16(blk, pl->h_G.data(), K, KR, K, false, NBK, 4);
  off[4] = blk.size(); append_blocks16(blk, Yq, NQ, K, KX, false, NBX, NBK);
  off[5] = blk.size(); append_blocks16(blk, Yq, NQ, KX, KX, false, NBX, NBX);
  off[6] = blk.size(); append_blocks16(blk, Yq, K, NQ, KX, true, NBK, NBX);
  off[7] = blk.size(); append_blocks16(blk, Yq, KX, NQ, KX, true, NBX, NBX);
  off[8] = blk.size(); append_blocks16(blk, pl->h_Gx.data(), K, KX, KX, false, NBK, NBX);
  HIPCHK(hipDeviceSynchronize());
  if (int rc = upload(pl->oscblk, blk.data(), blk.size() * 8)) return rc;
  const double* b = pl->oscblk.d();
  pl->osc = OscMats{b + off[0], b + off[1], b + off[2], b + off[3], b + off[4], b + off[5], b + off[6], b + off[7], b + off[8]};
  return TEMX_OK;
}

#ifndef TEMX_OS_DEFER
#define TEMX_OS_DEFER 1
#endif
template <typename T, int KIND>
static int launch_sweep_os_t(temx_plan* pl, const FieldPtrs<4>& fp, bool sub, const double* rho, double* partial,
                             const Split& sp, hipStream_t st) {
  using KD = OsKind<KIND>;
  const int2* cuts = nullptr;
  if (int rc = os_cuts_dev(pl, sub, sp.nsplit, &cuts)) return rc;
  dim3 grid(sp.grid), block(256);
  constexpr int NBR = 2;
  constexpr int PDv = sizeof(T) == 4 ? 4 : 2;
  constexpr int DF = TEMX_OS_DEFER;
  const bool tile_map = pl->os_tile;
  double* px = partial;
  double* pp = sub ? nullptr : partial + (int64_t)sp.nsplit * KD::NFX * pl->KX * pl->D;
  int rc = TEMX_OK;
  const bool listed = dispatch_strict(OsPairs{}, pl->TBS, pl->TBX, rc, [&](auto pair) {
    constexpr int TBSv = decltype(pair)::first, TBXv = decltype(pair)::second;
    if constexpr (KIND == 3) {
      if (tile_map) return fail(TEMX_EUNSUPPORTED, "two tracers per sweep: row-map sweeps only");
    }
    if constexpr (KIND != 3) if (tile_map) {
      const size_t lds = ((size_t)4 * (DF ? 2 : 1) * 2 * TBXv * 16 + (size_t)4 * KD::NF * 2 * NBR * 64 +
                          (size_t)4 * KD::NP * 2 * TBSv * 64) * 8;
      return launch_lds<sweep_os_kernel<T, TBSv, TBXv, NBR, PDv, KIND, DF>>(pl->device, grid, block, lds, st, fp, pl->D,
          pl->K, pl->KX, sub ? pl->ycx_s.d() : pl->ycx.d(), static_cast<const int4*>(sub ? pl->crow_s.p : pl->crow.p), cuts,
          pl->colscale.d(), rho, pl->KR, px, pp, sp.nsplit, sp.ndt);
    }
    if (sizeof(T) == 4) {
      if (pl->cls_max_side > 8 * TEMX_F32_SIDE_CAP)
        return fail(TEMX_EUNSUPPORTED, "single sweep of fp32 fields: a latitude class of this plan has %lld members on one "
                    "side, and the sweep sums a side in fp32; create the plan with TEMX_LAT_TOL_F32",
                    (long long)pl->cls_max_side);
      const size_t lds = ((size_t)2 * 2 * TBXv * 16 + 16 + (size_t)4 * KD::NF * 2 * NBR * 64 +
                          (size_t)8 * (KD::NP - KD::NPR) * TBSv * 64 + (size_t)(KD::NF + KD::NP) * 512) * 8;
      const int si = sub ? 1 : 0;
      return launch_lds<sweep_os2_kernel<float, TBSv, TBXv, NBR, 2, KIND>>(
          pl->device, grid, dim3(512), lds, st, fp, pl->D, pl->K, pl->KX, sub ? pl->ycx_s.d() : pl->ycx.d(),
          static_cast<const int4*>(pl->side_crow[si][0].p), static_cast<const int4*>(pl->side_crow[si][1].p),
          static_cast<const int*>(pl->side_gfirst[si][0].p), static_cast<const int*>(pl->side_gfirst[si][1].p),
          cuts, pl->colscale.d(), rho, pl->KR, px, pp, sp.nsplit, sp.ndt);
    }
    constexpr size_t lds = ((size_t)2 * 2 * TBXv * 16 + 16 + (size_t)4 * KD::NF * 2 * NBR * 64 +
                            (size_t)4 * (KD::NP - KD::NPR) * 2 * TBSv * 64 + (size_t)2 * (KD::NF + KD::NP) * 256 + 2) * 8;
    static_assert(lds <= 163840, "the single sweep's workgroup fits the LDS of a compute unit");
    auto go = [&](auto handoff) {
      return launch_lds<sweep_osr_kernel<double, TBSv, TBXv, NBR, 2, KIND, decltype(handoff)::value>>(pl->device, grid,
          block, lds, st, fp, pl->D, pl->K, pl->KX, sub ? pl->ycx_s.d() : pl->ycx.d(),
          static_cast<const int4*>(sub ? pl->crow_s.p : pl->crow.p), cuts, pl->colscale.d(), rho, pl->KR, px, pp, sp.nsplit,
          sp.ndt, static_cast<int*>(pl->flag.p) + 1);
    };
    return pl->os_barrier ? go(Int<0>{}) : go(Int<1>{});
  });
  return listed ? rc : fail(TEMX_EUNSUPPORTED, "single-sweep form: no instantiation for L = %d", pl->L);
}

template <int KIND>
static int launch_sweep_os(temx_plan* pl, const FieldPtrs<4>& fp, int dtype, bool sub, const double* rho, double* partial,
                           const Split& sp, hipStream_t st) {
  return dtype == TEMX_F64 ? launch_sweep_os_t<double, KIND>(pl, fp, sub, rho, partial, sp, st)
                           : launch_sweep_os_t<float, KIND>(pl, fp, sub, rho, partial, sp, st);
}

static bool os_supported(const temx_plan* pl) {
  if (!pl->cls || pl->large || pl->weighted || !pl->qbasis || pl->h_crow.empty()) return false;
  const int tbx = (pl->L + 1 + 3) / 4;
  return (pl->TBS == 7 && tbx <= 13) || (pl->TBS == 4 && tbx <= 8) || (pl->TBS == 2 && tbx <= 4);
}

static bool os_active(const temx_plan* pl, int dtype) {
  (void)dtype;
  return pl->os_on;
}

static void set_tail(temx_plan* pl, int64_t t0, int64_t nts) {
  if (pl->tt0 != t0 || pl->tnt != nts) pl->c4_valid = pl->os_valid = pl->op_valid = pl->tq_valid = pl->xb_valid = false;
  pl->tt0 = t0;
  pl->tnt = nts;
  pl->tD = (int64_t)pl->nlev * nts;
}
static inline bool tail_is_whole(const temx_plan* pl) { return pl->tt0 == 0 && pl->tnt == pl->nt; }

static int tem_stage3_impl(temx_plan* pl, const double* B3, double* results, double* zonal, hipStream_t st);
static int tem_epilogue(temx_plan* pl, double* results, double* zonal, hipStream_t st);
static int bin_project_op(temx_plan* pl, const void* A, int dtype, int64_t D, double* B, hipStream_t st);
static int bin_zonal_mean(temx_plan* pl, const void* A, int dtype, int64_t D, double* out, int native, hipStream_t st);
static int miss_check(const temx_plan* pl);
static int miss_zonal_mean(temx_plan* pl, const void* A, int dtype, int64_t D, double* out, int native, hipStream_t st);
static int tracer_stage3_impl(temx_plan* pl, const double* Bq2, double* tres, double* tzon, hipStream_t st);

static SliceMap slice_map(const temx_plan* pl, int nsl, int64_t rows_total, int64_t row0) {
  SliceMap m;
  if (nsl <= 1) return m;
  m.D = pl->D;
  m.nt = (int)pl->nt;
  m.W = nsl;
  m.chunk = rows_total * pl->nlev * ((pl->nt + nsl - 1) / nsl);
  m.row0 = row0;
  return m;
}

template <int NBK>
static int launch_osc_t(temx_plan* pl, const OscFieldsIn& fin, int nf, int nout, double* Bf, double* At, double* ab,
                        const OscPairsIn& pin, int np, double* Bp, int64_t Dt, hipStream_t st) {
  const unsigned gx = (unsigned)((Dt + 15) / 16);
  hipLaunchKernelGGL((osc_fields_kernel<NBK>), dim3(gx, nf, 2), dim3(OSC_W * 64), (size_t)osc_fields_lds(NBK) * 8, st, fin, pl->osc, pl->K,
                     pl->KX, pl->KR, pl->NQ, Dt, nout, Bf, At, ab, pl->D, (int)pl->tnt, (int)pl->nt, (int)pl->tt0);
  HIPCHK(hipGetLastError());
  hipLaunchKernelGGL((osc_pairs_kernel<NBK>), dim3(gx, np), dim3(OSC_W * 64), (size_t)osc_pairs_lds(NBK) * 8, st, pin, pl->osc, pl->wq2.d(),
                     pl->K, pl->KX, pl->NQ, Dt, Bp);
  HIPCHK(hipGetLastError());
  return TEMX_OK;
}
static int launch_osc(temx_plan* pl, const OscFieldsIn& fin, int nf, int nout, double* Bf, double* At, double* ab,
                      const OscPairsIn& pin, int np, double* Bp, int64_t Dt, hipStream_t st) {
  if (pl->TB == 13 && pl->TBX == 13) return launch_osc_t<13>(pl, fin, nf, nout, Bf, At, ab, pin, np, Bp, Dt, st);
  if (pl->TB == 8 && pl->TBX == 8) return launch_osc_t<8>(pl, fin, nf, nout, Bf, At, ab, pin, np, Bp, Dt, st);
  if (pl->TB == 4 && pl->TBX == 4) return launch_osc_t<4>(pl, fin, nf, nout, Bf, At, ab, pin, np, Bp, Dt, st);
  return fail(TEMX_EUNSUPPORTED, "single-sweep contraction: no instantiation for L = %d", pl->L);
}

static int os_prepass(temx_plan* pl, const FieldPtrs<4>& fp, int dtype, double* As, hipStream_t st) {
  int rc;
  const int64_t D = pl->D, KD4 = (int64_t)4 * pl->KX * D;
  pl->op_valid = pl->c4_valid = pl->tq_valid = pl->os_valid = false;
  if ((rc = launch_sweep_os<0>(pl, fp, dtype, true, pl->rho0.d(), pl->partial.d(), pl->sp_os_s, st))) return rc;
  return launch_reduce_rows(pl, pl->partial.d(), pl->sp_os_s.nsplit, KD4, 4, pl->KX, pl->KR, D, As, st);
}

static int os_sweep(temx_plan* pl, const FieldPtrs<4>& fp, int dtype, const double* As, int nsl, double* proj, hipStream_t st) {
  int rc;
  const int64_t D = pl->D;
  const int64_t KD4 = (int64_t)4 * pl->KX * D, KD3 = (int64_t)3 * pl->K * D;
  pl->op_valid = pl->c4_valid = pl->tq_valid = pl->os_valid = false;
  hipLaunchKernelGGL(os_ref_solve_kernel, dim3((unsigned)((D + 15) / 16), 4), dim3(256), 0, st, As, pl->KR, pl->KR, D,
                     pl->Gsinv.d(), pl->rho.d());
  HIPCHK(hipGetLastError());
  TimedLaunch tl{};
  time_begin(pl, 0, st, tl);
  rc = launch_sweep_os<0>(pl, fp, dtype, false, pl->rho.d(), pl->partial.d(), pl->sp_os, st);
  time_end(pl, 0, st, tl);
  if (rc) return rc;
  const int64_t rows = (int64_t)4 * pl->KX + 3 * pl->K;
  if ((rc = launch_reduce(pl, pl->partial.d(), pl->sp_os.nsplit, KD4, proj, st, -1, nullptr, slice_map(pl, nsl, rows, 0)))) return rc;
  return launch_reduce(pl, pl->partial.d() + (int64_t)pl->sp_os.nsplit * KD4, pl->sp_os.nsplit, KD3, nsl > 1 ? proj : proj + KD4, st, -1,
                       nullptr, slice_map(pl, nsl, rows, (int64_t)4 * pl->KX));
}

static int os_tail(temx_plan* pl, const double* proj_s, int64_t t0, int64_t nts, double* results, double* zonal, hipStream_t st) {
  int rc;
  set_tail(pl, t0, nts);
  const int64_t Dt = pl->tD;
  const int64_t rows = (int64_t)4 * pl->KX + 3 * pl->K;
  if (proj_s != pl->Ax.d())
    HIPCHK(hipMemcpyAsync(pl->Ax.p, proj_s, (size_t)rows * Dt * 8, hipMemcpyDeviceToDevice, st));
  {
    TimedLaunch t2{};
    time_begin(pl, 1, st, t2);
    const size_t lds = os_contract_lds(pl->K, pl->KX, pl->NQ) * 8;
    const double* Pp = pl->Ax.d() + (int64_t)4 * pl->KX * Dt;
    if (pl->osc_lds) {
      OsFields in;
      for (int f = 0; f < 4; ++f) {
        in.A[f] = pl->Ax.d() + (int64_t)f * pl->KX * Dt;
        in.rho[f] = pl->rho.d() + (int64_t)f * pl->KR * pl->D;
      }
      rc = launch_lds<os_contract_kernel<0>, 160 * 1024>(pl->device, dim3((unsigned)((Dt + OSC - 1) / OSC)), dim3(256), lds,
          st, in, Pp, pl->K, pl->KX, pl->KR, pl->NQ, Dt, pl->T.d(), pl->Ginv.d(), pl->G.d(), pl->Gx.d(), pl->gaunt.d(),
          pl->wq2.d(), pl->B4.d(), pl->B3.d(), pl->D, (int)nts, (int)pl->nt, (int)t0);
      if (rc) return rc;
    } else {
      using KD = OsKind<0>;
      const int64_t QD = (int64_t)pl->NQ * Dt;
      OscFieldsIn fin;
      OscPairsIn pin{};
      for (int f = 0; f < 4; ++f) {
        fin.A[f] = pl->Ax.d() + (int64_t)f * pl->KX * Dt;
        fin.rho[f] = pl->rho.d() + (int64_t)f * pl->KR * pl->D;
      }
      for (int k = 0; k < 3; ++k) {
        pin.At_a[k] = pl->osAt.d() + KD::pa(k) * QD; pin.At_b[k] = pl->osAt.d() + KD::pb(k) * QD;
        pin.ab_a[k] = pl->osAb.d() + KD::pa(k) * QD; pin.ab_b[k] = pl->osAb.d() + KD::pb(k) * QD;
        pin.P[k] = Pp + (int64_t)k * pl->K * Dt;
      }
      if ((rc = launch_osc(pl, fin, 4, 4, pl->B4.d(), pl->osAt.d(), pl->osAb.d(), pin, 3, pl->B3.d(), Dt, st))) return rc;
    }
    time_end(pl, 1, st, t2);
  }
  if ((rc = launch_solve(pl, pl->B4.d(), 4, Dt, pl->C4.d(), pl->zb.d(), st))) return rc;
  if ((rc = tem_stage3_impl(pl, pl->B3.d(), results, zonal, st))) return rc;
  pl->c4_valid = true;
  pl->os_valid = true;
  return TEMX_OK;
}

static int tem_run_os(temx_plan* pl, const FieldPtrs<4>& fp, int dtype, double* results, double* zonal, void* stream) {
  hipStream_t st = S_(stream);
  int rc;
  if ((rc = os_prepass(pl, fp, dtype, pl->Axs.d(), st))) return rc;
  if ((rc = os_sweep(pl, fp, dtype, pl->Axs.d(), 1, pl->Ax.d(), st))) return rc;
  return os_tail(pl, pl->Ax.d(), 0, pl->nt, results, zonal, st);
}

static int tracer_ws(temx_plan* pl);

static int tracer_os_ws(temx_plan* pl, int nq) {
  const int64_t D = pl->D;
  int rc;
  if ((rc = tracer_ws(pl))) return rc;
  if ((rc = pl->Axq.ensure((size_t)nq * (pl->KX + 2 * pl->K + pl->KR) * D * 8))) return rc;
  if ((rc = pl->osAtq.ensure((size_t)nq * pl->NQ * D * 8))) return rc;
  if ((rc = pl->osAbq.ensure((size_t)nq * pl->NQ * D * 8))) return rc;
  if ((rc = pl->Bqp.ensure((size_t)nq * 3 * pl->K * D * 8))) return rc;
  return pl->rho_t.ensure((size_t)4 * pl->KR * D * 8);
}

static int tracer_os_prepass(temx_plan* pl, int nq, const FieldPtrs<4>& fp, int dtype, double* Asq, hipStream_t st) {
  int rc;
  const int64_t D = pl->D;
  if ((rc = tracer_os_ws(pl, nq))) return rc;
  pl->tq_valid = false;
  rc = nq == 2 ? launch_sweep_os<3>(pl, fp, dtype, true, pl->rho0.d(), pl->partial.d(), pl->sp_os_s, st)
               : launch_sweep_os<1>(pl, fp, dtype, true, pl->rho0.d(), pl->partial.d(), pl->sp_os_s, st);
  if (rc) return rc;
  return launch_reduce_rows(pl, pl->partial.d(), pl->sp_os_s.nsplit, (int64_t)nq * pl->KX * D, nq, pl->KX, pl->KR, D, Asq, st);
}

static int tracer_os_sweep(temx_plan* pl, int nq, const FieldPtrs<4>& fp, int dtype, const double* Asq, int nsl, double* projq,
                           hipStream_t st) {
  int rc;
  const int64_t D = pl->D, KXD = (int64_t)pl->KX * D, KD = (int64_t)pl->K * D, KRD = (int64_t)pl->KR * D;
  if ((rc = tracer_os_ws(pl, nq))) return rc;
  pl->tq_valid = false;
  hipLaunchKernelGGL(os_ref_solve_kernel, dim3((unsigned)((D + 15) / 16), nq), dim3(256), 0, st, Asq, pl->KR, pl->KR, D,
                     pl->Gsinv.d(), pl->rho_t.d());
  HIPCHK(hipGetLastError());
  HIPCHK(hipMemcpyAsync(pl->rho_t.d() + nq * KRD, pl->rho.d() + 1 * KRD, (size_t)KRD * 8, hipMemcpyDeviceToDevice, st));
  HIPCHK(hipMemcpyAsync(pl->rho_t.d() + (nq + 1) * KRD, pl->rho.d() + 3 * KRD, (size_t)KRD * 8, hipMemcpyDeviceToDevice, st));
  rc = nq == 2 ? launch_sweep_os<3>(pl, fp, dtype, false, pl->rho_t.d(), pl->partial.d(), pl->sp_os, st)
               : launch_sweep_os<1>(pl, fp, dtype, false, pl->rho_t.d(), pl->partial.d(), pl->sp_os, st);
  if (rc) return rc;
  const int64_t rows = (int64_t)nq * (pl->KX + 2 * pl->K);
  if ((rc = launch_reduce(pl, pl->partial.d(), pl->sp_os.nsplit, nq * KXD, projq, st, -1, nullptr, slice_map(pl, nsl, rows, 0)))) return rc;
  return launch_reduce(pl, pl->partial.d() + (int64_t)pl->sp_os.nsplit * nq * KXD, pl->sp_os.nsplit, 2 * nq * KD,
                       nsl > 1 ? projq : projq + nq * KXD, st, -1, nullptr, slice_map(pl, nsl, rows, (int64_t)nq * pl->KX));
}

static int tracer_os_tail(temx_plan* pl, int nq, const double* projq_s, double* const* tres, double* const* tzon, hipStream_t st) {
  int rc;
  const int64_t Dt = pl->tD, KXD = (int64_t)pl->KX * Dt, KDt = (int64_t)pl->K * Dt, KRD = (int64_t)pl->KR * pl->D;
  double* Bq = pl->Bqp.d();
  double* Bq2 = pl->Bqp.d() + nq * KDt;
  if (pl->osc_lds) {
    if (nq != 1) return fail(TEMX_EUNSUPPORTED, "two tracers per sweep need the contraction on the matrix cores (TEMX_OPT_OS_CONTRACT = 0)");
    const size_t lds = os_contract_lds(pl->K, pl->KX, pl->NQ) * 8;
    OsFields in{};
    in.A[0] = projq_s;
    in.A[1] = pl->Ax.d() + 1 * KXD;
    in.A[2] = pl->Ax.d() + 3 * KXD;
    in.rho[0] = pl->rho_t.d();
    in.rho[1] = pl->rho.d() + 1 * KRD;
    in.rho[2] = pl->rho.d() + 3 * KRD;
    rc = launch_lds<os_contract_kernel<1>, 160 * 1024>(pl->device, dim3((unsigned)((Dt + OSC - 1) / OSC)), dim3(256), lds,
        st, in, projq_s + KXD, pl->K, pl->KX, pl->KR, pl->NQ, Dt, pl->T.d(), pl->Ginv.d(), pl->G.d(), pl->Gx.d(),
        pl->gaunt.d(), pl->wq2.d(), Bq, Bq2, pl->D, (int)pl->tnt, (int)pl->nt, (int)pl->tt0);
    if (rc) return rc;
  } else {
    const int64_t QD = (int64_t)pl->NQ * Dt;
    OscFieldsIn fin{};
    OscPairsIn pin{};
    const int other[2] = {1, 3};
    for (int i = 0; i < nq; ++i) {
      fin.A[i] = projq_s + i * KXD;
      fin.rho[i] = pl->rho_t.d() + i * KRD;
      for (int k = 0; k < 2; ++k) {
        const int p = 2 * i + k;
        pin.At_a[p] = pl->osAtq.d() + i * QD; pin.ab_a[p] = pl->osAbq.d() + i * QD;
        pin.At_b[p] = pl->osAt.d() + other[k] * QD; pin.ab_b[p] = pl->osAb.d() + other[k] * QD;
        pin.P[p] = projq_s + nq * KXD + (int64_t)p * KDt;
      }
    }
    if ((rc = launch_osc(pl, fin, nq, nq, Bq, pl->osAtq.d(), pl->osAbq.d(), pin, 2 * nq, Bq2, Dt, st))) return rc;
  }
  const size_t slab = (size_t)pl->K4 * Dt * 8;
  for (int i = 0; i < nq; ++i) {
    if ((rc = launch_solve(pl, Bq + i * KDt, 1, Dt, pl->Ct.d(), pl->tz.d(), st))) return rc;
    HIPCHK(hipMemcpyAsync((char*)pl->Ct.p + slab, (char*)pl->C4.p + slab, slab, hipMemcpyDeviceToDevice, st));
    HIPCHK(hipMemcpyAsync((char*)pl->Ct.p + 2 * slab, (char*)pl->C4.p + 3 * slab, slab, hipMemcpyDeviceToDevice, st));
    if ((rc = tracer_stage3_impl(pl, Bq2 + 2 * i * KDt, tres[i], tzon ? tzon[i] : nullptr, st))) return rc;
  }
  return TEMX_OK;
}

static FieldPtrs<4> tracer_fields(int nq, const void* const* q, const void* va, const void* wap) {
  return nq == 2 ? four(q[0], q[1], va, wap) : four(q[0], va, wap, nullptr);
}

static int tracer_run_os(temx_plan* pl, int nq, const void* const* q, const void* va, const void* wap, int dtype,
                         double* const* tres, double* const* tzon, void* stream) {
  hipStream_t st = S_(stream);
  int rc;
  if ((rc = tracer_os_ws(pl, nq))) return rc;
  const FieldPtrs<4> fp = tracer_fields(nq, q, va, wap);
  double* Asq = pl->Axq.d() + (int64_t)nq * (pl->KX + 2 * pl->K) * pl->D;
  if ((rc = tracer_os_prepass(pl, nq, fp, dtype, Asq, st))) return rc;
  if ((rc = tracer_os_sweep(pl, nq, fp, dtype, Asq, 1, pl->Axq.d(), st))) return rc;
  return tracer_os_tail(pl, nq, pl->Axq.d(), tres, tzon, st);
}

#define TEMX_CATCH                                                                                     \
  catch (const std::bad_alloc&) { return fail(TEMX_ENOMEM, "out of host memory"); }                   \
  catch (const std::exception& e_) { return fail(TEMX_EINTERNAL, "unexpected C++ exception: %s", e_.what()); } \
  catch (...) { return fail(TEMX_EINTERNAL, "unexpected C++ exception"); }

static inline bool miss_mode(const temx_plan* pl) { return pl->opt_missing == 1; }
static inline bool bin_mode(const temx_plan* pl) { return pl->opt_lat_bins > 0; }
static inline bool bin_refused(const temx_plan* pl) { return bin_mode(pl) && pl->bin_pass == 0; }
struct BinPass {
  temx_plan* pl;
  explicit BinPass(temx_plan* p) : pl(p) { ++pl->bin_pass; }
  ~BinPass() { --pl->bin_pass; }
};
static int bin_refuse(const char* what) {
  return fail(TEMX_EUNSUPPORTED, "%s is not available while latitude bins are in effect (TEMX_OPT_LAT_BINS): the binned form "
              "serves temx_tem_run, temx_project and temx_zonal_mean", what);
}

static inline dim3 bin_sweep_grid(const temx_plan* pl, int64_t D) {
  const int Dw = (int)((D + 63) / 64);
  return dim3((unsigned)(pl->bin_nchunk * ((Dw + 3) / 4)));
}

template <int NF>
static int launch_bin_moments(temx_plan* pl, const FieldPtrs<NF>& fp, int dtype, int64_t D, const double* colscale, int sfield,
                              hipStream_t st) {
  const int Dw = (int)((D + 63) / 64);
  if ((int64_t)pl->bin_nchunk * ((Dw + 3) / 4) >= ((int64_t)1 << 31)) return fail(TEMX_EUNSUPPORTED, "latitude bins: too many work units");
  const dim3 grid = bin_sweep_grid(pl, D);
  const int4* ch = static_cast<const int4*>(pl->bin_chunk.p);
  const int* rows = static_cast<const int*>(pl->bin_rows.p);
  return by_dtype(dtype, [&](auto t) {
    return dispatch(BinJValues{}, pl->bin_J, [&](auto j) {
      return launch<bin_moments_kernel<typename decltype(t)::type, NF, decltype(j)::value>>(
          grid, dim3(256), 0, st, fp, D, Dw, ch, rows, pl->bin_s.d(), colscale, sfield, pl->bin_cm.d());
    });
  });
}

static inline double miss_thr(const temx_plan* pl) { return pl->opt_min_cov / 1000.0; }
static inline double miss_omt(const temx_plan* pl) { return 1.0 - std::pow(10.0, -(double)pl->opt_miss_w); }
static int miss_refuse(const char* what) {
// ... 352 lines not shown
      w.ginv.release();
    }
    for (DevBuf* b : {&lat, &lon, &lat_out, &partial, &B, &C, &flag}) b->release();
  }
};

template <int NF, int TBv> struct WaveCfg {
  static constexpr int WPS = NF == 1 ? ProjCfg1::WPS : (TBv <= 16 ? ProjCfgE::WPS : 2), DPW = NF == 1 ? 4 : 1;
};
template <int NF>
static Split wave_split(const temx_plan* pl, int64_t D, int tb) {
  const int wps = tb <= 16 ? WaveCfg<NF, 16>::WPS : WaveCfg<NF, 32>::WPS;
  return choose_split(D, pl->nchunk, wps * pl->num_cu, WaveCfg<NF, 16>::DPW);
}

static int wave_reduce(temxk_wave* w, const double* partial, int nsplit, int64_t stride, int64_t n, double* B, hipStream_t st) {
  return launch_reduce(w->pl, partial, nsplit, n, B, st, stride, nullptr, SliceMap(), static_cast<int*>(w->flag.p));
}

template <int NF>
static int wave_sweep(temxk_wave* w, const WaveM& wm, const FieldPtrs<NF>& fp, int dtype, int64_t D, const double* colscale,
                      int sfield, double* B, hipStream_t st) {
  temx_plan* pl = w->pl;
  const WaveShape& sh = wm.sh;
  size_t need = 0;
  for (int sl = 0; sl < sh.nslice; ++sl)
    need = std::max(need, (size_t)wave_split<NF>(pl, D, wave_slice_tb(sh, sl)).nsplit * NF * wave_slice_cols(sh, sl) * D * 8);
  int rc = w->partial.ensure(need);
  if (rc) return rc;
  for (int sl = 0; sl < sh.nslice; ++sl) {
    const int Ks = wave_slice_cols(sh, sl);
    const Split sp = wave_split<NF>(pl, D, wave_slice_tb(sh, sl));
    rc = by_dtype(dtype, [&](auto t) {
      using T = typename decltype(t)::type;
      return dispatch(WaveTBValues{}, wave_slice_tb(sh, sl), [&](auto tb) {
        constexpr int TBv = decltype(tb)::value;
        return launch<project_kernel<T, NF, 1, TBv, 2, WaveCfg<NF, TBv>::WPS>>(
            dim3(sp.grid), dim3(256), 0, st, fp, pl->N, D, Ks, (const double*)wm.yblk.d(), sh.gstride, WAVE_SLICE_TB * sl,
            pl->nchunk, colscale, sfield, w->partial.d(), sp.nsplit, sp.ndt);
      });
    });
    if (rc) return rc;
    if (sh.nslice == 1) return wave_reduce(w, w->partial.d(), sp.nsplit, (int64_t)NF * Ks * D, (int64_t)NF * Ks * D, B, st);
    for (int f = 0; f < NF; ++f)
      if ((rc = wave_reduce(w, w->partial.d() + (int64_t)f * Ks * D, sp.nsplit, (int64_t)NF * Ks * D, (int64_t)Ks * D,
                            B + ((int64_t)f * sh.Kc + 4 * WAVE_SLICE_TB * sl) * D, st)))
        return rc;
  }
  return TEMX_OK;
}

static int wave_solve(const WaveM& wm, int nf, int64_t D, const double* B, double* C, hipStream_t st) {
  hipLaunchKernelGGL(wave_solve_kernel, dim3((unsigned)((D + 63) / 64), (unsigned)((wm.sh.Kc + 3) / 4), (unsigned)nf), dim3(256),
                     0, st, B, wm.sh.Kc, D, (const double*)wm.ginv.d(), C);
  HIPCHK(hipGetLastError());
  return TEMX_OK;
}

static int wave_ensure(temxk_wave* w, int nf, int64_t D) {
  int rc;
  if ((rc = w->B.ensure((size_t)nf * w->kc_max * D * 8))) return rc;
  return w->C.ensure((size_t)nf * w->kc_max * D * 8);
}

static int wave_build_m(temxk_wave* w, WaveM& wm) {
  temx_plan* pl = w->pl;
  const WaveShape& sh = wm.sh;
  const int m = wm.m, L = pl->L, Kc = sh.Kc;
  const int64_t N = pl->N, npad = pl->nchunk * 16;
  double r = (2.0 * m + 1.0) / (4.0 * M_PI);
  for (int k = 1; k <= m; ++k) r *= (2.0 * k - 1.0) / (2.0 * k);
  const double pmm_norm = ((m & 1) ? -1.0 : 1.0) * std::sqrt(2.0) * std::sqrt(r);
  int rc;
  if ((rc = wm.yblk.ensure((size_t)npad * sh.kpad * 8))) return rc;
  if ((rc = wm.pz.ensure((size_t)pl->M * sh.ndeg * 8))) return rc;
  if ((rc = wm.ginv.ensure((size_t)Kc * Kc * 8))) return rc;
  DevBuf Ym, Z;
  struct Free {
    DevBuf &a, &b;
    ~Free() { a.release(); b.release(); }
  } free_{Ym, Z};
  if ((rc = Ym.ensure((size_t)N * Kc * 8))) return rc;
  if ((rc = Z.ensure((size_t)N * Kc * 8))) return rc;
  hipLaunchKernelGGL(wave_basis_kernel, dim3((unsigned)((npad + 255) / 256)), dim3(256), 0, nullptr, (const double*)w->lat.d(),
                     (const double*)w->lon.d(), N, npad, m, L, pmm_norm, sh.gstride, Ym.d(), wm.yblk.d());
  HIPCHK(hipGetLastError());
  hipLaunchKernelGGL(wave_ztable_kernel, dim3((unsigned)((pl->M + 255) / 256)), dim3(256), 0, nullptr,
                     (const double*)w->lat_out.d(), pl->M, m, L, pmm_norm, wm.pz.d());
  HIPCHK(hipGetLastError());
  if ((rc = wave_ensure(w, 1, Kc))) return rc;
  FieldPtrs<1> fp;
  fp.p[0] = Ym.p;
  if ((rc = wave_sweep<1>(w, wm, fp, TEMX_F64, Kc, nullptr, -1, w->B.d(), nullptr))) return rc;
  std::vector<double> G((size_t)Kc * Kc), Gi((size_t)Kc * Kc), F;
  HIPCHK(hipMemcpy(G.data(), w->B.p, G.size() * 8, hipMemcpyDeviceToHost));
  for (double v : G)
    if (!std::isfinite(v)) return fail(TEMX_ERANK, "zonal wavenumber m = %d: the Gram matrix of the basis is not finite", m);
  if (const int piv = wave_cholesky(G.data(), Kc, F))
    return fail(TEMX_ERANK, "zonal wavenumber m = %d: the Gram matrix of its %d basis columns is not positive definite "
                "(pivot %d): the grid does not resolve this wavenumber at L = %d", m, Kc, piv - 1, L);
  wave_inverse_from_factor(F, Kc, Gi.data());
  HIPCHK(hipMemcpy(wm.ginv.p, Gi.data(), Gi.size() * 8, hipMemcpyHostToDevice));
  if ((rc = temx_zonal_mean(pl, Ym.p, TEMX_F64, Kc, Z.d(), 1, nullptr))) return rc;
  hipLaunchKernelGGL(wave_deflate_kernel, dim3((unsigned)((N * Kc + 255) / 256)), dim3(256), 0, nullptr, (const double*)Ym.d(),
                     (const double*)Z.d(), N, Kc, sh.gstride, wm.yblk.d());
  HIPCHK(hipGetLastError());
  HIPCHK(hipDeviceSynchronize());
  return TEMX_OK;
}

static int wave_plan_refused(const temx_plan* pl) {
  if (pl->weighted) return fail(TEMX_EUNSUPPORTED, "zonal wavenumbers are not available on a plan in weights mode");
  if (miss_mode(pl)) return fail(TEMX_EUNSUPPORTED, "zonal wavenumbers are not available in missing-value mode (TEMX_OPT_MISSING = 1)");
  if (bin_mode(pl)) return fail(TEMX_EUNSUPPORTED, "zonal wavenumbers are not available while latitude bins are in effect (TEMX_OPT_LAT_BINS)");
  if (pl->ext_G)
    return fail(TEMX_EUNSUPPORTED, "zonal wavenumbers are not available on a plan finalised with a Gram matrix from outside "
                "(an ncol-sharded job): the fit runs over all columns of the grid");
  return TEMX_OK;
}

extern "C" {

int temx_version(void) { return 402; }

const char* temx_last_error(void) { return g_err.c_str(); }

int temx_device_count(void) try {
  int n = 0;
  if (hipGetDeviceCount(&n) != hipSuccess) return 0;
  return n;
} TEMX_CATCH

void temx_plan_destroy(temx_plan* pl) {
  if (!pl) return;
  (void)hipSetDevice(pl->device);
  DevBuf* bufs[] = {&pl->x, &pl->Y0, &pl->yblk, &pl->yblk_w, &pl->Y0p, &pl->G, &pl->Ginv, &pl->norm,
                    &pl->flag, &pl->p, &pl->pg, &pl->lg, &pl->coslat, &pl->fcor, &pl->colscale,
                    &pl->B4, &pl->B3, &pl->C4, &pl->zb, &pl->partial, &pl->opB, &pl->opC,
                    &pl->Bq, &pl->Bq2, &pl->Ct, &pl->tz, &pl->rows, &pl->ysym, &pl->Bs, &pl->XB, &pl->P3};
  for (DevBuf* b : bufs) b->release();
  pl->crow.release();
  pl->ycls.release();
  pl->csum.release();
  pl->ccnt.release();
  pl->Pq.release();
  pl->csq.release();
  pl->Pq2.release();
  pl->ycls_l.release();
  pl->pbuf.release();
  pl->gblk.release();
  pl->ypblk.release();
  for (DevBuf* b : {&pl->T, &pl->Qp, &pl->GinvA, &pl->G2, &pl->xo, &pl->xc, &pl->ycx, &pl->ycx_s, &pl->crow_s, &pl->side_crow[0][0], &pl->side_crow[0][1], &pl->side_crow[1][0], &pl->side_crow[1][1],
                    &pl->side_gfirst[0][0], &pl->side_gfirst[0][1], &pl->side_gfirst[1][0], &pl->side_gfirst[1][1], &pl->rho,
                    &pl->rho0, &pl->gaunt, &pl->wq2, &pl->Axq, &pl->rho_t, &pl->Gx, &pl->Gsinv, &pl->Ax, &pl->Axs, &pl->oscblk, &pl->osAt, &pl->osAb, &pl->osAtq, &pl->osAbq, &pl->Bqp})
    b->release();
  for (DevBuf* b : {&pl->eblk, &pl->mtab, &pl->mB, &pl->mC, &pl->mCcov, &pl->mcov, &pl->mZ}) b->release();
  for (DevBuf* b : {&pl->mtB, &pl->mtB2, &pl->mtC, &pl->mtCcov, &pl->mtz}) b->release();
  for (DevBuf* b : {&pl->bin_a, &pl->bin_chunk, &pl->bin_c0, &pl->bin_rows, &pl->bin_s, &pl->bin_T, &pl->bin_cm, &pl->bin_z, &pl->bin_cy}) b->release();
  for (auto& kv : pl->csplits_s) kv.second.release();
  for (auto& kv : pl->csplits) kv.second.release();
  for (int w = 0; w < 2; ++w)
    for (auto& tl : pl->timed[w]) {
      (void)hipEventDestroy(tl.a);
      (void)hipEventDestroy(tl.b);
    }
  delete pl;
}

static int build_basis(temx_plan* pl, const double* rowscale_dev, const double* T, double* Y0c, double* yblk) {
  const int64_t npad = pl->nchunk * 16;
  return by_basis_rows(pl->K, [&](auto r) {
    return launch<basis_kernel<decltype(r)::value>>(dim3((unsigned)((npad + 255) / 256)), dim3(256), 0, nullptr, pl->x.d(),
        pl->N, npad, pl->K, pl->stride, pl->norm.d(), rowscale_dev, T, Y0c, yblk);
  });
}

static int build_out_basis(temx_plan* pl, const double* T, double* dst, bool blocks) {
  const int64_t mch = (pl->M + 15) / 16;
  const int rc = by_basis_rows(pl->K, [&](auto r) {
    return launch<basis_kernel<decltype(r)::value>>(dim3((unsigned)((mch * 16 + 255) / 256)), dim3(256), 0, nullptr,
        pl->xo.d(), (int64_t)pl->M, mch * 16, pl->K, pl->stride, pl->norm.d(), (const double*)nullptr, T, dst,
        (double*)nullptr);
  });
  if (rc) return rc;
  HIPCHK(hipDeviceSynchronize());
  if (blocks && pl->K <= 64) {
    std::vector<double> yp((size_t)pl->M * pl->K);
    HIPCHK(hipMemcpy(yp.data(), dst, yp.size() * 8, hipMemcpyDeviceToHost));
    return upload(pl->ypblk, pack_blocks4(yp.data(), pl->M, pl->K, pl->TB));
  }
  return TEMX_OK;
}

static int build_cls_basis(temx_plan* pl, const double* T) {
  const unsigned nb = (unsigned)((pl->cls_npad + 255) / 256);
  return by_basis_rows(pl->K, [&](auto r) {
    constexpr int R = decltype(r)::value;
    if (pl->lcls) {
      for (int sl = 0; sl < pl->nslice; ++sl)
        hipLaunchKernelGGL(cls_basis_slice_kernel<R>, dim3(nb), dim3(256), 0, 0, pl->xc.d(), pl->ncls, pl->cls_npad, pl->K,
            64 * sl, pl->norm.d(), T, pl->ycls_l.d() + sl * pl->ycls_lstride);
    } else if (pl->cls) {
      hipLaunchKernelGGL(cls_basis_kernel<R>, dim3(nb), dim3(256), 0, 0, pl->xc.d(), pl->ncls, pl->cls_npad, pl->K, pl->TBS,
                         pl->norm.d(), T, pl->ycls.d());
    }
    HIPCHK(hipGetLastError());
    return (int)TEMX_OK;
  });
}

static int build_sym_basis(temx_plan* pl, const double* T) {
  if (!pl->sym) return TEMX_OK;
  const int64_t n4 = pl->npg_alloc * 4;
  return by_basis_rows(pl->K, [&](auto r) {
    return launch<sym_basis_kernel<decltype(r)::value>>(dim3((unsigned)((n4 + 255) / 256)), dim3(256), 0, nullptr, pl->x.d(),
                                                        static_cast<const int*>(pl->rows.p), pl->npair, n4, pl->K, pl->TBS,
                                                        pl->norm.d(), T, pl->ysym.d());
  });
}

static int build_all_bases(temx_plan* pl, const double* T) {
  int rc;
  if ((rc = build_basis(pl, nullptr, T, nullptr, pl->yblk.d()))) return rc;
  if ((rc = build_cls_basis(pl, T))) return rc;
  if ((rc = build_sym_basis(pl, T))) return rc;
  if ((rc = build_out_basis(pl, T, pl->Qp.d(), true))) return rc;
  HIPCHK(hipDeviceSynchronize());
  return TEMX_OK;
}

int temx_plan_create(temx_plan** out, int device, int64_t ncol, int L, int M,
                     const double* lat_deg_host, const double* lat_out_deg_host, int flags) try {
  if (!out || !lat_deg_host || !lat_out_deg_host) return fail(TEMX_EINVAL, "null argument");
  *out = nullptr;
  if (ncol < 1 || M < 1 || L < 0) return fail(TEMX_EINVAL, "ncol, M must be >= 1 and L >= 0");
  if (L > 511) return fail(TEMX_EUNSUPPORTED, "L = %d: this version supports L <= 511", L);
  int ndev = 0;
  HIPCHK(hipGetDeviceCount(&ndev));
  if (device < 0 || device >= ndev) return fail(TEMX_EHIP, "device %d not available (%d visible)", device, ndev);
  HIPCHK(hipSetDevice(device));
  hipDeviceProp_t prop;
  HIPCHK(hipGetDeviceProperties(&prop, device));
  if (strncmp(prop.gcnArchName, "gfx950", 6) != 0)
    return fail(TEMX_EUNSUPPORTED, "libtemx is built for gfx950 (MI355X); device is %s", prop.gcnArchName);

  temx_plan* pl = new temx_plan();
  pl->device = device;
  pl->no_qr = (flags & TEMX_NO_QR) != 0;
  const double tol_dflt = (flags & TEMX_LAT_TOL_F32) ? 1e-8 : 1e-11;
  pl->num_cu = prop.multiProcessorCount > 0 ? prop.multiProcessorCount : 256;
  pl->N = ncol;
  pl->nchunk = (ncol + 15) / 16;
  pl->L = L;
  pl->K = L + 1;
  pl->TB = pl->K <= 16 ? 4 : (pl->K <= 32 ? 8 : (pl->K <= 52 ? 13 : 16));
  pl->stride = pl->TB;
  if (pl->K > 64) {
    pl->large = true;
    pl->nslice = (pl->K + 63) / 64;
    pl->stride = 16 * pl->nslice;
  }
  pl->K4 = 4 * pl->stride;
  pl->M = M;
  pl->lat_out_deg.assign(lat_out_deg_host, lat_out_deg_host + M);
  pl->h_lat.assign(lat_deg_host, lat_deg_host + ncol);
  int rc = TEMX_OK;
  auto bail = [&](int code) {
    temx_plan_destroy(pl);
    return code;
  };

  const double d2r = M_PI / 180.0;
  std::vector<double> xs((size_t)std::max<int64_t>(ncol, M));
  for (int64_t i = 0; i < ncol; ++i) xs[i] = std::cos((90.0 - lat_deg_host[i]) * d2r);
  if ((rc = upload(pl->x, xs.data(), (size_t)ncol * 8))) return bail(rc);
  std::vector<double> norm((size_t)std::max(64, pl->K4), 0.0);
  for (int l = 0; l < pl->K; ++l) norm[l] = std::sqrt((2.0 * l + 1.0) / (4.0 * M_PI));
  if ((rc = upload(pl->norm, norm.data(), norm.size() * 8))) return bail(rc);
  const int zero[2] = {0, 0};
  if ((rc = upload(pl->flag, zero, sizeof(zero)))) return bail(rc);

  if ((rc = pl->Y0.ensure((size_t)ncol * pl->K * 8))) return bail(rc);
  if ((rc = pl->yblk.ensure((size_t)(pl->nchunk + 1) * 4 * pl->stride * 16 * 8))) return bail(rc);
  if (hipMemset(pl->yblk.p, 0, pl->yblk.bytes) != hipSuccess) return bail(fail(TEMX_EHIP, "hipMemset of the Y0 blocks failed"));
  if ((rc = build_basis(pl, nullptr, nullptr, pl->Y0.d(), pl->yblk.d()))) return bail(rc);

  for (int m = 0; m < M; ++m) xs[m] = std::cos((90.0 - lat_out_deg_host[m]) * d2r);
  if ((rc = upload(pl->xo, xs.data(), (size_t)M * 8))) return bail(rc);
  if ((rc = pl->Y0p.ensure((size_t)M * pl->K * 8))) return bail(rc);
  if ((rc = pl->Qp.ensure((size_t)M * pl->K * 8))) return bail(rc);
  if ((rc = build_out_basis(pl, nullptr, pl->Y0p.d(), false))) return bail(rc);
  if ((rc = build_out_basis(pl, nullptr, pl->Qp.d(), true))) return bail(rc);

  {
    if ((rc = pl->G.ensure((size_t)pl->K * pl->K * 8))) return bail(rc);
    if ((rc = pl->Ginv.ensure((size_t)pl->K * pl->K * 8))) return bail(rc);
    Split sp = choose_split(pl->K, pl->nchunk, 2 * pl->num_cu);
    if ((rc = pl->partial.ensure((size_t)sp.nsplit * std::min(pl->K, 64) * pl->K * 8))) return bail(rc);
    FieldPtrs<1> fp;
    fp.p[0] = pl->Y0.p;
    if ((rc = project_all<1>(pl, fp, TEMX_F64, pl->K, nullptr, -1, sp, pl->G.d(), 0))) return bail(rc);
    hipError_t e = hipDeviceSynchronize();
    if (e != hipSuccess) return bail(fail(TEMX_EHIP, "gram kernel failed: %s", hipGetErrorString(e)));
  }
  {
    const int nhalf = (pl->K + 1) / 2;
    const int tbs = (nhalf + 3) / 4;
    pl->TBS = tbs <= 2 ? 2 : (tbs <= 4 ? 4 : (tbs <= 7 ? 7 : 8));
  }
  {
    const char* e0 = getenv("TEMX_NO_SYM");
    const char* e1 = getenv("TEMX_NO_CLS");
    ClassTables ct;
    if ((!pl->large || pl->K <= 256) && !(flags & (TEMX_NO_SYMMETRY | TEMX_NO_CLASSES)) && !(e0 && e0[0] == '1') &&
        !(e1 && e1[0] == '1') &&
        build_classes(lat_deg_host, ncol, ct, sym_tol_deg(tol_dflt), (flags & TEMX_LAT_TOL_F32) ? (size_t)TEMX_F32_SIDE_CAP : 0, TEMX_F32_SIDE_KEEP)) {
      if ((rc = upload(pl->crow, ct.crow.data(), ct.crow.size() * sizeof(int)))) return bail(rc);

      if ((rc = upload(pl->ccnt, ct.cnt.data(), ct.cnt.size() * 8))) return bail(rc);
      if ((rc = upload(pl->xc, ct.xc.data(), ct.xc.size() * 8))) return bail(rc);
      pl->h_xc = ct.xc;
      pl->h_cnt = ct.cnt;
      pl->h_crow = ct.crow;
      if (const char* dp = getenv("TEMX_DUMP_CROW")) {
        if (FILE* fh = fopen(dp, "wb")) {
          const int32_t hdr[2] = {(int32_t)ct.ngroups, (int32_t)ct.crow.size()};
          fwrite(hdr, 4, 2, fh);
          fwrite(ct.gbatch0.data(), 4, (size_t)ct.ngroups + 1, fh);
          fwrite(ct.crow.data(), 4, ct.crow.size(), fh);
          fclose(fh);
        }
      }
      pl->cls_npad = (ct.ngroups + 1) * 4;
      pl->gbatch0 = std::move(ct.gbatch0);
      pl->cgroups = ct.ngroups;
      pl->cbatches = ct.nbatch;
      pl->ncls = ct.ncls;
      pl->cls_max_side = ct.max_side;
      if (pl->large) {
        pl->ycls_lstride = (ct.ngroups + 1) * 256;
        if ((rc = pl->ycls_l.ensure((size_t)pl->nslice * pl->ycls_lstride * 8))) return bail(rc);
// ... 212 lines not shown
  HIPCHK(hipSetDevice(pl->device));
  hipStream_t st = S_(stream);
  const size_t KK = (size_t)pl->K * pl->K * 8;
  switch (which) {
    case TEMX_MAT_Y0:
      HIPCHK(hipMemcpyAsync(dst, pl->Y0.p, (size_t)pl->N * pl->K * 8, hipMemcpyDeviceToDevice, st));
      return TEMX_OK;
    case TEMX_MAT_Y0P:
      HIPCHK(hipMemcpyAsync(dst, pl->Y0p.p, (size_t)pl->M * pl->K * 8, hipMemcpyDeviceToDevice, st));
      return TEMX_OK;
    case TEMX_MAT_GRAM:
      if (!pl->h_G_own.empty()) {
        HIPCHK(hipStreamSynchronize(st));
        HIPCHK(hipMemcpy(dst, pl->h_G_own.data(), KK, hipMemcpyHostToDevice));
        return TEMX_OK;
      }
      HIPCHK(hipMemcpyAsync(dst, pl->G.p, KK, hipMemcpyDeviceToDevice, st));
      return TEMX_OK;
    case TEMX_MAT_GINV:
      if (!pl->finalized) return fail(TEMX_ESTATE, "plan not finalised");
      HIPCHK(hipMemcpyAsync(dst, pl->GinvA.p, KK, hipMemcpyDeviceToDevice, st));
      return TEMX_OK;
    case TEMX_MAT_Y0INV:
      if (!pl->finalized) return fail(TEMX_ESTATE, "plan not finalised");
      hipLaunchKernelGGL(y0inv_kernel, dim3((unsigned)((pl->N + 255) / 256)), dim3(256), 0, st, pl->Y0.d(),
                         pl->GinvA.d(), pl->N, pl->K, dst);
      HIPCHK(hipGetLastError());
      return TEMX_OK;
    case TEMX_MAT_GRAM2: {
      if (!pl->finalized) return fail(TEMX_ESTATE, "plan not finalised");
      if (!pl->qbasis) {
        std::vector<double> I((size_t)pl->K * pl->K, 0.0);
        for (int k = 0; k < pl->K; ++k) I[(size_t)k * pl->K + k] = 1.0;
        HIPCHK(hipStreamSynchronize(st));
        HIPCHK(hipMemcpy(dst, I.data(), KK, hipMemcpyHostToDevice));
        return TEMX_OK;
      }
      if (int rc2 = gram_of_q(pl)) return rc2;
      HIPCHK(hipMemcpyAsync(dst, pl->G2.p, KK, hipMemcpyDeviceToDevice, st));
      return TEMX_OK;
    }
    case TEMX_MAT_GX:
    case TEMX_MAT_GSUB: {
      if (!pl->os_built) return fail(TEMX_ESTATE, "the single-sweep tables are not built (temx_plan_set_tem on a plan that takes that form)");
      const std::vector<double>& h = which == TEMX_MAT_GX ? pl->h_Gx_own : pl->h_Gs;
      HIPCHK(hipStreamSynchronize(st));
      HIPCHK(hipMemcpy(dst, h.data(), h.size() * 8, hipMemcpyHostToDevice));
      return TEMX_OK;
    }
    case TEMX_MAT_COVERAGE:
      if (pl->miss_cov_D < 0) return fail(TEMX_ESTATE, "no masked run on this plan yet (TEMX_OPT_MISSING = 1)");
      HIPCHK(hipMemcpyAsync(dst, pl->mcov.p, (size_t)pl->M * pl->miss_cov_D * 8, hipMemcpyDeviceToDevice, st));
      return TEMX_OK;
    default:
      return fail(TEMX_EINVAL, "unknown matrix id %d", which);
  }
} TEMX_CATCH

int temx_plan_set_os_matrices(temx_plan* pl, const double* Gx_host, const double* Gs_host) try {
  if (!pl || !Gx_host || !Gs_host) return fail(TEMX_EINVAL, "null argument");
  if (!pl->os_built) return fail(TEMX_ESTATE, "the single-sweep tables are not built");
  HIPCHK(hipSetDevice(pl->device));
  const int KR = pl->KR;
  std::vector<long double> Li;
  std::vector<double> Gi((size_t)KR * KR);
  if (spd_factor(Gs_host, KR, Li) != 0)
    return fail(TEMX_ERANK, "the subsample of latitude classes does not determine a degree-%d reference", KR - 1);
  inverse_from_factor(Li, KR, Gi.data());
  HIPCHK(hipDeviceSynchronize());
  if (int rc = upload(pl->Gsinv, Gi.data(), Gi.size() * 8)) return rc;
  if (int rc = upload(pl->Gx, Gx_host, (size_t)pl->K * pl->KX * 8)) return rc;
  pl->h_Gx.assign(Gx_host, Gx_host + (size_t)pl->K * pl->KX);
  if (int rc = os_upload_blocks(pl)) return rc;
  pl->os_need_global = false;
  pl->os_valid = false;
  return TEMX_OK;
} TEMX_CATCH

int temx_project(temx_plan* pl, const void* A, int dtype, int64_t D, double* B, void* stream) try {
  if (pl && miss_mode(pl)) return miss_refuse("temx_project");
  if (!pl || !A || !B) return fail(TEMX_EINVAL, "null argument");
  if (D < 1 || D >= ((int64_t)1 << 28)) return fail(TEMX_EINVAL, "D must be in [1, 2^28)");
  HIPCHK(hipSetDevice(pl->device));
  if (bin_mode(pl)) return bin_project_op(pl, A, dtype, D, B, S_(stream));
  FieldPtrs<1> fp;
  fp.p[0] = A;
  if (pl->cls) {
    Split spc = choose_split(D, std::max<int64_t>(1, pl->cbatches / 4), CLS_PROJ_E_WPS * pl->num_cu, 4);
    int rcc = pl->partial.ensure((size_t)spc.nsplit * pl->K * D * 8);
    if (rcc) return rcc;
    if ((rcc = launch_project_cls<1>(pl, fp, dtype, D, nullptr, -1, pl->partial.d(), spc, S_(stream)))) return rcc;
    return launch_reduce(pl, pl->partial.d(), spc.nsplit, (int64_t)pl->K * D, B, S_(stream));
  }
  Split sp = choose_split(D, pl->nchunk, 2 * pl->num_cu);
  int rc = pl->partial.ensure((size_t)sp.nsplit * std::min(pl->K, 64) * D * 8);
  if (rc) return rc;
  return project_all<1>(pl, fp, dtype, D, nullptr, -1, sp, B, S_(stream));
} TEMX_CATCH

int temx_zonal_mean_from_sums(temx_plan* pl, const double* B, int64_t D, double* out, int native,
                              void* stream) try {
  if (pl && miss_mode(pl)) return miss_refuse("temx_zonal_mean_from_sums");
  if (pl && bin_refused(pl)) return bin_refuse("temx_zonal_mean_from_sums");
  if (!pl || !B || !out) return fail(TEMX_EINVAL, "null argument");
  if (!pl->finalized) return fail(TEMX_ESTATE, "plan not finalised");
  HIPCHK(hipSetDevice(pl->device));
  int rc;
  if (!native) return launch_solve(pl, B, 1, D, nullptr, out, S_(stream));
  if ((rc = pl->opC.ensure((size_t)pl->K4 * D * 8))) return rc;
  if ((rc = launch_solve(pl, B, 1, D, pl->opC.d(), nullptr, S_(stream)))) return rc;
  return launch_recon(pl, D, pl->opC.d(), out, S_(stream));
} TEMX_CATCH

int temx_zonal_mean(temx_plan* pl, const void* A, int dtype, int64_t D, double* out, int native,
                    void* stream) try {
  if (!pl || !A || !out) return fail(TEMX_EINVAL, "null argument");
  if (!pl->finalized) return fail(TEMX_ESTATE, "plan not finalised");
  if (miss_mode(pl)) return miss_zonal_mean(pl, A, dtype, D, out, native, S_(stream));
  if (bin_mode(pl)) return bin_zonal_mean(pl, A, dtype, D, out, native, S_(stream));
  int rc = pl->opB.ensure((size_t)pl->K * std::max<int64_t>(D, 1) * 8);
  if (rc) return rc;
  if ((rc = temx_project(pl, A, dtype, D, pl->opB.d(), stream))) return rc;
  return temx_zonal_mean_from_sums(pl, pl->opB.d(), D, out, native, stream);
} TEMX_CATCH

struct FormChoice {
  bool two_pass;
  bool force_op;
  int os;
};
static FormChoice form_choice(const temx_plan* pl) {
  FormChoice c{false, false, -1};
  if (bin_mode(pl)) return FormChoice{true, false, 0};
  switch (pl->opt_form) {
    case TEMX_FORM_TWO_PASS: c.two_pass = true; c.os = 0; break;
    case TEMX_FORM_CLASS_SUMS: c.force_op = true; c.os = 0; break;
    case TEMX_FORM_SINGLE_SWEEP: c.force_op = true; c.os = 1; break;
    case TEMX_FORM_NO_SINGLE_SWEEP: c.os = 0; break;
    default: break;
  }
  if (const char* e = getenv("TEMX_TWO_PASS")) c.two_pass = e[0] == '1';
  if (const char* e = getenv("TEMX_ONE_PASS")) c.force_op = c.force_op || e[0] == '1';
  if (const char* e = getenv("TEMX_SINGLE_SWEEP")) c.os = e[0] == '0' ? 0 : (e[0] == '1' ? 1 : c.os);
  return c;
}
static bool tile_map(int opt, const char* env) {
  if (const char* e = getenv(env)) return !strcmp(e, "tile");
  return opt == 1;
}
static bool os_barrier_wanted(const temx_plan* pl) {
  if (const char* e = getenv("TEMX_OS_SYNC")) return !strcmp(e, "barrier");
  return pl->opt_os_sync == 1;
}
static bool tracer_one_pass_wanted(const temx_plan* pl) {
  if (const char* e = getenv("TEMX_TRACER_ONE_PASS")) return e[0] == '1';
  return pl->opt_tracer_one_pass == 1;
}

static int bin_check(const temx_plan* pl);
static int bin_set_tem(temx_plan* pl);

int temx_plan_configure(temx_plan* pl, int option, int value) try {
  if (!pl) return fail(TEMX_EINVAL, "null plan");
  switch (option) {
    case TEMX_OPT_FORM:
      if (value < -1 || value > TEMX_FORM_NO_SINGLE_SWEEP) return fail(TEMX_EINVAL, "TEMX_OPT_FORM: unknown form %d", value);
      pl->opt_form = value;
      break;
    case TEMX_OPT_OS_MAP: pl->opt_os_map = value; break;
    case TEMX_OPT_OP_MAP: pl->opt_op_map = value; break;
    case TEMX_OPT_TRACER_ONE_PASS: pl->opt_tracer_one_pass = value; break;
    case TEMX_OPT_OS_SUBSAMPLE:
      if (value < 4) return fail(TEMX_EINVAL, "TEMX_OPT_OS_SUBSAMPLE: at least 4 class-groups");
      if (pl->os_built && value != pl->os_keep) return fail(TEMX_ESTATE, "the single-sweep tables of this plan are built: set the subsample before temx_plan_set_tem");
      pl->os_keep = value;
      break;
    case TEMX_OPT_SINGLE_SWEEP_MIN_GROUPS: pl->opt_single_sweep_min_groups = value; break;
    case TEMX_OPT_OS_CONTRACT: pl->opt_os_contract = value; break;
    case TEMX_OPT_MISSING:
      if (value != 0 && value != 1) return fail(TEMX_EINVAL, "TEMX_OPT_MISSING: 0 (raise) or 1 (mask), got %d", value);
      if (value == 1) {
        if (bin_mode(pl)) return fail(TEMX_EUNSUPPORTED, "missing-value mode is not available while latitude bins are in effect (TEMX_OPT_LAT_BINS)");
        if (int rc = miss_check(pl)) return rc;
      }
      pl->opt_missing = value;
      pl->miss_valid = false;
      break;
    case TEMX_OPT_MIN_COVERAGE:
      if (value < 0 || value > 1000) return fail(TEMX_EINVAL, "TEMX_OPT_MIN_COVERAGE: per mille in 0..1000, got %d", value);
      pl->opt_min_cov = value;
      break;
    case TEMX_OPT_MISSING_WEIGHT:
      if (value < 4 || value > 14) return fail(TEMX_EINVAL, "TEMX_OPT_MISSING_WEIGHT: tau = 10^-value, value in 4..14, got %d", value);
      pl->opt_miss_w = value;
      break;
    case TEMX_OPT_OS_SYNC:
      if (value != 0 && value != 1) return fail(TEMX_EINVAL, "TEMX_OPT_OS_SYNC: 0 (flags) or 1 (barriers), got %d", value);
      pl->opt_os_sync = value;
      break;
    case TEMX_OPT_LAT_BINS: {
      const int B = value == -1 ? BIN_DEFAULT : value;
      if (B != 0) {
        if (!bin_count_ok(B)) return fail(TEMX_EINVAL, "TEMX_OPT_LAT_BINS: 0 (off), -1 (default, %d) or one of 128, 256, 512, 1024, 2048, got %d", BIN_DEFAULT, value);
        if (int rc = bin_check(pl)) return rc;
        if (bin_degree(pl->L, B) == 0)
          return fail(TEMX_EINVAL, "TEMX_OPT_LAT_BINS: (L, B) = (%d, %d): no Chebyshev degree up to %d keeps the basis rows to %.0e; use more bins",
                      pl->L, B, BIN_MAX_DEGREE, BIN_BOUND);
      }
      pl->opt_lat_bins = B;
      pl->bin_J = B ? bin_degree(pl->L, B) : 0;
      break;
    }
    case TEMX_OPT_BIN_DEGREE: return fail(TEMX_EINVAL, "TEMX_OPT_BIN_DEGREE is chosen by the library (read it with temx_plan_option)");
    default: return fail(TEMX_EINVAL, "unknown option %d", option);
  }
  pl->tem = false;
  return TEMX_OK;
} TEMX_CATCH

int temx_plan_option(const temx_plan* pl, int option) try {
  if (!pl) return -1;
  switch (option) {
    case TEMX_OPT_FORM:
      if (miss_mode(pl)) return TEMX_FORM_MASKED;
      if (bin_mode(pl)) return TEMX_FORM_BINNED;
      return pl->os_on ? TEMX_FORM_SINGLE_SWEEP : ((pl->cls && pl->onepass) || (pl->lcls && pl->lone) ? TEMX_FORM_CLASS_SUMS : TEMX_FORM_TWO_PASS);
    case TEMX_OPT_OS_MAP: return tile_map(pl->opt_os_map, "TEMX_OS_MAP") ? 1 : 0;
    case TEMX_OPT_OP_MAP: return tile_map(pl->opt_op_map, "TEMX_OP_MAP") ? 1 : 0;
    case TEMX_OPT_TRACER_ONE_PASS: return tracer_one_pass_wanted(pl) ? 1 : 0;
    case TEMX_OPT_OS_SUBSAMPLE: return pl->os_keep;
    case TEMX_OPT_SINGLE_SWEEP_MIN_GROUPS: return pl->opt_single_sweep_min_groups;
    case TEMX_OPT_OS_CONTRACT: return pl->osc_lds ? 1 : 0;
    case TEMX_OPT_MISSING: return pl->opt_missing;
    case TEMX_OPT_MIN_COVERAGE: return pl->opt_min_cov;
    case TEMX_OPT_MISSING_WEIGHT: return pl->opt_miss_w;
    case TEMX_OPT_OS_SYNC: return os_barrier_wanted(pl) ? 1 : 0;
    case TEMX_OPT_LAT_BINS: return pl->opt_lat_bins;
    case TEMX_OPT_BIN_DEGREE: return pl->bin_J;
    default: return -1;
  }
} TEMX_CATCH

int temx_plan_set_tem(temx_plan* pl, int nlev, int64_t nt, const double* p_pa_host, double p0) try {
  if (!pl || !p_pa_host) return fail(TEMX_EINVAL, "null argument");
  if (nlev < 2 || nt < 1) return fail(TEMX_EINVAL, "need nlev >= 2 and nt >= 1");
  if ((int64_t)nlev * nt >= ((int64_t)1 << 28)) return fail(TEMX_EINVAL, "nlev*nt must be < 2^28");
  if (pl->M < 2) return fail(TEMX_EINVAL, "need at least 2 zonal-mean latitudes");
  HIPCHK(hipSetDevice(pl->device));
  std::vector<double> p(p_pa_host, p_pa_host + nlev);
  for (int j = 1; j < nlev; ++j)
    if (!(p[j] > p[j - 1])) return fail(TEMX_EINVAL, "pressure must be strictly ascending (front end flips)");
  pl->tem = false;
  pl->onepass = pl->lone = pl->op_valid = pl->xb_valid = pl->tq_valid = false;
  pl->os_on = pl->os_valid = false;
  pl->miss_valid = pl->mt_valid = false;
  pl->os_tile = tile_map(pl->opt_os_map, "TEMX_OS_MAP");
  {
    const char* e = getenv("TEMX_OS_CONTRACT");
    pl->osc_lds = e ? !strcmp(e, "lds") : pl->opt_os_contract == 1;
  }
  pl->op_tile = tile_map(pl->opt_op_map, "TEMX_OP_MAP");
  pl->os_barrier = os_barrier_wanted(pl);
  pl->nlev = nlev;
  pl->nt = nt;
  pl->D = (int64_t)nlev * nt;
  pl->tD = pl->D;
  pl->tnt = nt;
  pl->tt0 = 0;
  pl->p0 = p0;
  const int M = pl->M;
  const int64_t D = pl->D;
  int rc;
  const TemTables tt = tem_tables(p, nt, p0, pl->lat_out_deg);
  if ((rc = upload(pl->p, p))) return rc;
  if ((rc = upload(pl->pg, tt.pg))) return rc;
  if ((rc = upload(pl->lg, tt.lg))) return rc;
  if ((rc = upload(pl->coslat, tt.coslat))) return rc;
  if ((rc = upload(pl->fcor, tt.fcor))) return rc;
  if ((rc = upload(pl->colscale, tt.colscale))) return rc;

  const int ndt_ = (int)((D + 15) / 16);
  const int pdpw = proj_dpw(4, ndt_);
  pl->sp_proj4 = choose_split(D, pl->nchunk, proj_wps(4, pdpw) * pl->num_cu, pdpw);
  const int edpw = pick_dpw(ndt_, 4);
  pl->sp_eddy = choose_split(D, pl->nchunk / (8 / edpw), pl->num_cu, edpw);
  const size_t need =
      (size_t)std::max(pl->sp_proj4.nsplit * 4, pl->sp_eddy.nsplit * (8 / edpw) * 3) * pl->K * D * 8;
  if ((rc = pl->partial.ensure(need))) return rc;
  if ((rc = pl->B4.ensure((size_t)4 * pl->K * D * 8))) return rc;
  if ((rc = pl->B3.ensure((size_t)3 * pl->K * D * 8))) return rc;
  if ((rc = pl->C4.ensure((size_t)4 * pl->K4 * D * 8))) return rc;
  if ((rc = pl->zb.ensure((size_t)8 * M * D * 8))) return rc;
  pl->sp_proj1 = choose_split(D, pl->nchunk, 2 * pl->num_cu);
  if (unfused_stage2(pl)) {
    const size_t need3 = (size_t)pl->sp_proj1.nsplit * 3 * 64 * D * 8;
    if ((rc = pl->partial.ensure(std::max(need3, pl->partial.bytes)))) return rc;
  }
  pl->lone = false;
  pl->xb_valid = false;
  pl->op_valid = false;
  if (pl->lcls) {
    const size_t need_cs = (size_t)pl->cgroups * ndt_ * 14 * 64 * 8, need_pb = (size_t)pl->cgroups * ndt_ * 3 * 128 * 8;
    size_t fr = 0, tot = 0;
    if (ndt_ >= 4 && !form_choice(pl).two_pass && hipMemGetInfo(&fr, &tot) == hipSuccess &&
        (pl->csum.bytes >= need_cs || need_cs + need_pb < fr / 2) && alloc_write_stream(pl->csum, need_cs) == TEMX_OK &&
        pl->pbuf.ensure(need_pb) == TEMX_OK) {
      HIPCHK(hipMemset(pl->csum.p, 0, pl->csum.bytes));
      HIPCHK(hipMemset(pl->pbuf.p, 0, pl->pbuf.bytes));
      const int64_t cunits = std::max<int64_t>(1, pl->cbatches / 4);
      pl->sp_cproj4 = choose_split(D, cunits, TEMX_CLS_OP_WPS * pl->num_cu, 4, 8);
      pl->sp_cflux = choose_split(D, std::max<int64_t>(1, pl->cgroups / (8 / edpw)), pl->num_cu, edpw, TEMX_CLS_MINCHUNK);
      pl->sp_lflux = choose_split(D, std::max<int64_t>(1, pl->cgroups / 8), pl->num_cu, 1, TEMX_CLS_MINCHUNK);
      const size_t need4 = (size_t)pl->sp_cflux.nsplit * 4 * 64 * D * 8;
      if ((rc = pl->partial.ensure(std::max(need4, pl->partial.bytes)))) return rc;
      if ((rc = pl->Bs.ensure((size_t)4 * 64 * D * 8))) return rc;
      const int2* cuts_unused = nullptr;
      if ((rc = class_cuts_dev(pl, pl->sp_cproj4.nsplit, &cuts_unused, true))) return rc;
      pl->lone = true;
    }
  }
  if (pl->cls) {
    const bool quad = pick_dpw(ndt_, 4) == 4;
    const int64_t cunits = std::max<int64_t>(1, pl->cbatches / 4);
    pl->sp_cproj4 = choose_split(D, cunits, (quad ? 2 : CLS_PROJ_E_WPS) * pl->num_cu, quad ? 4 : 1, TEMX_CLS_MINCHUNK);
    Split sp_op = choose_split(D, cunits, TEMX_CLS_OP_WPS * pl->num_cu, 4, 8);
    pl->sp_cproj1 = choose_split(D, cunits, CLS_PROJ_E_WPS * pl->num_cu, 4, TEMX_CLS_MINCHUNK);
    pl->sp_ceddy = choose_split(D, cunits / (8 / edpw), pl->num_cu, edpw, TEMX_CLS_MINCHUNK);
    const size_t need3 = (size_t)std::max({pl->sp_cproj4.nsplit * 4, pl->sp_ceddy.nsplit * (8 / edpw) * 3,
                                           pl->sp_cproj1.nsplit}) * pl->K * D * 8;
    if ((rc = pl->partial.ensure(std::max(need3, pl->partial.bytes)))) return rc;
    pl->onepass = false;
    pl->op_valid = false;
    {
      const FormChoice fc = form_choice(pl);
      const bool force = fc.force_op;
      const bool quad_op = ndt_ >= 4 && (force || (double)pl->N * (double)D >= 1.2e7);
      if (quad_op && !fc.two_pass) {
        const size_t need_cs = (size_t)pl->cgroups * ndt_ * 8 * 64 * 8;
        size_t fr = 0, tot = 0;
        bool have = pl->csum.bytes >= need_cs;
        if (!have && hipMemGetInfo(&fr, &tot) == hipSuccess && need_cs < fr / 2 && alloc_write_stream(pl->csum, need_cs) == TEMX_OK) {
          HIPCHK(hipMemset(pl->csum.p, 0, pl->csum.bytes));
          have = true;
        }
        if (have) {
          pl->onepass = true;
          pl->sp_cproj4 = sp_op;
          pl->sp_cflux = choose_split(D, std::max<int64_t>(1, pl->cgroups / (8 / edpw)), pl->num_cu, edpw, TEMX_CLS_MINCHUNK);
          const size_t need4 = (size_t)std::max(pl->sp_cflux.nsplit * 3, sp_op.nsplit * 7) * pl->K * D * 8;
          if ((rc = pl->partial.ensure(std::max(need4, pl->partial.bytes)))) return rc;
          if ((rc = pl->Pq.ensure((size_t)3 * pl->K * D * 8))) return rc;
          pl->sp_copw = choose_split(D, std::max<int64_t>(1, cunits / 4), pl->num_cu, 1, 8);
          {
            const bool off = fc.os == 0, forced = fc.os == 1;
            const int64_t min_groups = pl->opt_single_sweep_min_groups >= 0 ? pl->opt_single_sweep_min_groups : 640;
            bool want = !off && os_supported(pl) && (forced || pl->cgroups >= min_groups);
            if (want) {
              rc = build_os_tables(pl);
              if (rc == TEMX_ERANK) want = false;
              else if (rc) return rc;
            }
            if (want) {
              pl->sp_os = choose_split(D, cunits, pl->num_cu, 4, 8);
              pl->sp_os_s = choose_split(D, std::max<int64_t>(1, pl->sbatches / 4), pl->num_cu, 4, 2);
              const size_t per = ((size_t)4 * pl->KX + 3 * pl->K) * D * 8;
              if ((rc = pl->partial.ensure(std::max((size_t)std::max(pl->sp_os.nsplit, pl->sp_os_s.nsplit) * per, pl->partial.bytes)))) return rc;
              if ((rc = pl->Ax.ensure(((size_t)4 * pl->KX + 3 * pl->K) * D * 8))) return rc;
              if ((rc = pl->Axs.ensure((size_t)4 * pl->KR * D * 8))) return rc;
              if ((rc = pl->osAt.ensure((size_t)4 * pl->NQ * D * 8))) return rc;
              if ((rc = pl->osAb.ensure((size_t)4 * pl->NQ * D * 8))) return rc;
              if ((rc = pl->rho.ensure((size_t)4 * pl->KR * D * 8))) return rc;
              if ((rc = pl->rho0.ensure((size_t)4 * pl->KR * D * 8))) return rc;
              HIPCHK(hipMemset(pl->rho0.p, 0, pl->rho0.bytes));
              const int2* cu = nullptr;
              if ((rc = os_cuts_dev(pl, false, pl->sp_os.nsplit, &cu))) return rc;
              if ((rc = os_cuts_dev(pl, true, pl->sp_os_s.nsplit, &cu))) return rc;
              pl->os_on = true;
            }
          }
        }
      }
    }
    const int2* cuts_unused = nullptr;
    if (pl->onepass && (rc = class_cuts_dev(pl, pl->sp_cproj4.nsplit, &cuts_unused, true))) return rc;
    if (pl->onepass && (rc = class_cuts_dev(pl, pl->sp_copw.nsplit * 4, &cuts_unused, true))) return rc;
    for (int nsub : {pl->sp_cproj4.nsplit, pl->sp_cproj1.nsplit, pl->sp_ceddy.nsplit * (8 / edpw)})
      if ((rc = class_cuts_dev(pl, nsub, &cuts_unused))) return rc;
  }
  if (pl->sym) {
    const int64_t nch = (pl->npg + SYM_PROJ_CH - 1) / SYM_PROJ_CH;
    pl->sp_sproj4 = Split();
    pl->sp_sproj1 = Split();
    if (pick_dpw(ndt_, 4) == 4) {
      pl->sp_sproj4 = choose_split(D, nch, 2 * pl->num_cu, 4);
      pl->sp_sproj1 = choose_split(D, nch, 2 * pl->num_cu, 4);
    } else {
      pl->sp_sproj4 = choose_split(D, nch, SYM_PROJ_E_WPS * pl->num_cu, 1);
    }
    pl->sp_seddy = choose_split(D, pl->npg / (8 / edpw), pl->num_cu, edpw);
    const size_t need2 = (size_t)std::max({pl->sp_sproj4.nsplit * 4, pl->sp_seddy.nsplit * (8 / edpw) * 3,
                                           pl->sp_sproj1.nsplit}) * pl->K * D * 8;
    if ((rc = pl->partial.ensure(std::max(need2, pl->partial.bytes)))) return rc;
  }
  if (bin_mode(pl) && (rc = bin_set_tem(pl))) return rc;
  pl->tem = true;
  return TEMX_OK;
} TEMX_CATCH

static int tem_ready(temx_plan* pl) {
  if (!pl) return fail(TEMX_EINVAL, "null plan");
  if (!pl->finalized) return fail(TEMX_ESTATE, "plan not finalised");
  if (!pl->tem) return fail(TEMX_ESTATE, "temx_plan_set_tem has not been called");
  return TEMX_OK;
}

int temx_tem_stage1(temx_plan* pl, const void* ua, const void* va, const void* ta, const void* wap,
                    int dtype, double* B4, void* stream) try {
  if (pl && miss_mode(pl)) return miss_refuse("temx_tem_stage1");
  if (pl && bin_refused(pl)) return bin_refuse("temx_tem_stage1");
  int rc = tem_ready(pl);
  if (rc) return rc;
  if (!ua || !va || !ta || !wap || !B4) return fail(TEMX_EINVAL, "null argument");
  HIPCHK(hipSetDevice(pl->device));
  hipStream_t st = S_(stream);
  FieldPtrs<4> fp;
  fp.p[0] = ua; fp.p[1] = va; fp.p[2] = ta; fp.p[3] = wap;
  if (pl->large) set_tail(pl, 0, pl->nt);
  if (pl->large && pl->lone) {
    pl->op_valid = false;
    if ((rc = launch_class_sums(pl, fp, dtype, st))) return rc;
    if ((rc = project_sums<4>(pl, pl->csum.d(), 7, 0, B4, st))) return rc;
    pl->op_valid = true;
    return TEMX_OK;
  }
  if (pl->large) return project_all<4>(pl, fp, dtype, pl->D, pl->colscale.d(), 2, pl->sp_proj4, B4, st);
  TimedLaunch tl{};
  time_begin(pl, 0, st, tl);
  const bool sp4 = sym_project(pl, 4);
  const Split& sp = pl->cls ? pl->sp_cproj4 : (sp4 ? pl->sp_sproj4 : pl->sp_proj4);
  const bool op = pl->cls && pl->onepass;
  set_tail(pl, 0, pl->nt);
  pl->op_valid = false;
  pl->os_valid = false;
  pl->c4_valid = false;
  pl->tq_valid = false;
  rc = op      ? launch_sweep_op<0>(pl, fp, dtype, pl->partial.d(), sp, st)
       : pl->cls ? launch_project_cls<4>(pl, fp, dtype, pl->D, pl->colscale.d(), 2, pl->partial.d(), sp, st)
       : sp4   ? launch_project_sym<4>(pl, fp, dtype, pl->D, pl->colscale.d(), 2, pl->partial.d(), sp, st)
               : launch_project<4>(pl, fp, dtype, pl->D, pl->colscale.d(), 2, pl->partial.d(), sp, st);
  time_end(pl, 0, st, tl);
  if (rc) return rc;
  const int64_t KD = (int64_t)pl->K * pl->D;
  if (!op) return launch_reduce(pl, pl->partial.d(), sp.nsplit, 4 * KD, B4, st);
  if ((rc = launch_reduce(pl, pl->partial.d(), sp.nsplit, 4 * KD, B4, st, 7 * KD))) return rc;
  if ((rc = launch_reduce(pl, pl->partial.d() + 4 * KD, sp.nsplit, 3 * KD, pl->Pq.d(), st, 7 * KD))) return rc;
  pl->op_valid = true;
  return TEMX_OK;
} TEMX_CATCH

static int large_ws(temx_plan* pl) {
  const size_t nd = (size_t)pl->N * pl->D * 8;
  int rc;
  size_t fr = 0, tot = 0;
  const size_t have = pl->XB.bytes + pl->P3.bytes;
  if (have < 8 * nd && hipMemGetInfo(&fr, &tot) == hipSuccess && 8 * nd - have > fr)
    return fail(TEMX_ENOMEM, "the unfused second sweep (L > 63 without latitude classes, or a weighted plan) needs "
                             "%zu bytes of workspace (8 x ncol x nlev x nt doubles), %zu are free; process the "
                             "snapshots in smaller blocks (temx_plan_set_tem with a smaller nt)", 8 * nd - have, fr);
  if ((rc = pl->XB.ensure(5 * nd))) return rc;
  return pl->P3.ensure(3 * nd);
}

static int launch_eddy_from_xbar(temx_plan* pl, const FieldPtrs<4>& fp, int dtype, const FieldPtrs<4>& xb,
                                 const double* colscale, const EddyOut& eo, hipStream_t st, int64_t nrows = -1) {
  if (nrows < 0) nrows = pl->N;
  dim3 grid((unsigned)(pl->num_cu * 8)), block(256);
  if (dtype == TEMX_F64)
    hipLaunchKernelGGL(eddy_from_xbar_kernel<double>, grid, block, 0, st, fp, xb, nrows, pl->D, colscale, eo);
  else if (dtype == TEMX_F32)
    hipLaunchKernelGGL(eddy_from_xbar_kernel<float>, grid, block, 0, st, fp, xb, nrows, pl->D, colscale, eo);
  else
    return bad_dtype();
  HIPCHK(hipGetLastError());
  return TEMX_OK;
}

static FieldPtrs<4> native_means(temx_plan* pl, int a, int b, int c, int d) {
  const int64_t nd = pl->N * pl->D;
  FieldPtrs<4> xb;
  xb.p[0] = pl->XB.d() + a * nd; xb.p[1] = pl->XB.d() + b * nd;
  xb.p[2] = pl->XB.d() + c * nd; xb.p[3] = pl->XB.d() + d * nd;
  return xb;
}

static int ensure_xb(temx_plan* pl, hipStream_t st) {
  if (pl->xb_valid) return TEMX_OK;
  int rc;
  if ((rc = large_ws(pl))) return rc;
  const int64_t nd = pl->N * pl->D;
  for (int f = 0; f < 4; ++f)
    if ((rc = launch_recon(pl, pl->D, pl->C4.d() + (int64_t)f * pl->K4 * pl->D, pl->XB.d() + f * nd, st))) return rc;
  pl->xb_valid = true;
  return TEMX_OK;
}

static int tem_stage2_large(temx_plan* pl, const FieldPtrs<4>& fp, int dtype, const double* B4, double* B3,
                            hipStream_t st) {
  int rc;
  if ((rc = large_ws(pl))) return rc;
  const int64_t nd = pl->N * pl->D;
  if ((rc = launch_solve(pl, B4, 4, pl->D, pl->C4.d(), pl->zb.d(), st))) return rc;
  pl->c4_valid = true;
  for (int f = 0; f < 4; ++f)
    if ((rc = launch_recon(pl, pl->D, pl->C4.d() + (int64_t)f * pl->K4 * pl->D, pl->XB.d() + f * nd, st))) return rc;
  EddyOut eo{};
  FieldPtrs<3> f3;
  for (int i = 0; i < 3; ++i) {
    eo.p[4 + i] = pl->P3.d() + i * nd;
    f3.p[i] = eo.p[4 + i];
  }
  pl->xb_valid = true;
  if ((rc = launch_eddy_from_xbar(pl, fp, dtype, native_means(pl, 0, 1, 2, 3), pl->colscale.d(), eo, st))) return rc;
  return project_all<3>(pl, f3, TEMX_F64, pl->D, nullptr, -1, pl->sp_proj1, B3, st);
}

int temx_tem_stage2(temx_plan* pl, const void* ua, const void* va, const void* ta, const void* wap,
                    int dtype, const double* B4, double* B3, void* stream) try {
  if (pl && miss_mode(pl)) return miss_refuse("temx_tem_stage2");
  if (pl && bin_refused(pl)) return bin_refuse("temx_tem_stage2");
// ... 1436 lines not shown
```

### pytemdiags_amd/engine.py

```python
from __future__ import annotations

import ctypes as C

import numpy as np
import torch

from . import _lib
from ._lib import check

_DT = {torch.float64: _lib.F64, torch.float32: _lib.F32}


def _ptr(t):
    return C.c_void_p(t.data_ptr())


def _dbl(a):
    a = np.ascontiguousarray(a, dtype=np.float64)
    return a, a.ctypes.data_as(C.POINTER(C.c_double))


def lat_bins_value(lat_bins):
    if lat_bins is None or lat_bins is False:
        return 0
    if lat_bins is True:
        return -1
    if isinstance(lat_bins, (int, np.integer)) and (int(lat_bins) == 0 or int(lat_bins) in _lib.LAT_BINS_ALLOWED):
        return int(lat_bins)
    raise ValueError("lat_bins must be True, 0 or one of %s, got %r" % (_lib.LAT_BINS_ALLOWED, lat_bins))


class Plan:

    def __init__(self, lat_deg, lat_out_deg, L, device=0, defer_finalize=False, symmetry=True, classes=True, qr=True,
                 form=None, fp32_fields=False, lat_bins=None):
        self._h = C.c_void_p()
        self.lib = _lib.load()
        if isinstance(device, torch.device):
            device = device.index or 0
        self.device_index = int(device)
        self.device = torch.device("cuda", self.device_index)
        lat, plat = _dbl(lat_deg)
        lat_out, plat_out = _dbl(lat_out_deg)
        self.N, self.M, self.L, self.K = int(lat.size), int(lat_out.size), int(L), int(L) + 1
        self.lat_out = lat_out
        self.nlev = self.nt = self.D = None
        self.form_requested = "auto"
        check(self.lib.temx_plan_create(C.byref(self._h), self.device_index, self.N, self.L, self.M,
                                        plat, plat_out, (_lib.DEFER_FINALIZE if defer_finalize else 0)
                                        | (0 if symmetry else _lib.NO_SYMMETRY)
                                        | (0 if classes else _lib.NO_CLASSES)
                                        | (0 if qr else _lib.NO_QR)
                                        | (_lib.LAT_TOL_F32 if fp32_fields else 0)))
        if form is not None:
            self.configure(form=form)
        if lat_bins is not None:
            self.configure(lat_bins=lat_bins)

    @property
    def paired(self):
        return bool(self.lib.temx_plan_is_paired(self._h))

    @property
    def sweep_mode(self):
        return int(self.lib.temx_plan_sweep_mode(self._h))

    @property
    def one_pass(self):
        return bool(self.lib.temx_plan_one_pass(self._h))

    @property
    def single_sweep(self):
        return bool(self.lib.temx_plan_single_sweep(self._h))

    @property
    def tracer_one_pass(self):
        return self.one_pass and self.option(_lib.OPT_TRACER_ONE_PASS) == 1

    def configure(self, form=None, os_map=None, op_map=None, os_subsample=None, tracer_one_pass=None,
                  single_sweep_min_groups=None, os_contract=None, missing=None, min_coverage=None,
                  missing_weight=None, os_sync=None, lat_bins=None):
        def put(opt, val):
            check(self.lib.temx_plan_configure(self._h, opt, int(val)))
        if missing is not None:
            if missing not in _lib.MISSING_MODES:
                raise ValueError("missing must be 'raise' or 'mask', got %r" % (missing,))
            put(_lib.OPT_MISSING, _lib.MISSING_MODES[missing])
        if min_coverage is not None:
            mc = float(min_coverage)
            if not 0.0 <= mc <= 1.0:
                raise ValueError("min_coverage must lie in [0, 1], got %r" % (min_coverage,))
            put(_lib.OPT_MIN_COVERAGE, int(round(mc * 1000)))
        if missing_weight is not None:
            e = -np.log10(float(missing_weight))
            if not (float(missing_weight) > 0 and abs(e - round(e)) < 1e-9 and 4 <= round(e) <= 14):
                raise ValueError("missing_weight must be 10^-n with n in 4..14, got %r" % (missing_weight,))
            put(_lib.OPT_MISSING_WEIGHT, int(round(e)))
        if form is not None:
            put(_lib.OPT_FORM, _lib.FORMS[form] if isinstance(form, str) else form)
            self.form_requested = form
        for opt, val in ((_lib.OPT_OS_MAP, os_map), (_lib.OPT_OP_MAP, op_map)):
            if val is not None:
                put(opt, {"row": 0, "tile": 1}[val] if isinstance(val, str) else val)
        if os_subsample is not None:
            put(_lib.OPT_OS_SUBSAMPLE, os_subsample)
        if tracer_one_pass is not None:
            put(_lib.OPT_TRACER_ONE_PASS, 1 if tracer_one_pass else 0)
        if single_sweep_min_groups is not None:
            put(_lib.OPT_SINGLE_SWEEP_MIN_GROUPS, single_sweep_min_groups)
        if os_contract is not None:
            put(_lib.OPT_OS_CONTRACT, {"mfma": 0, "lds": 1}[os_contract] if isinstance(os_contract, str) else os_contract)
        if lat_bins is not None:
            put(_lib.OPT_LAT_BINS, lat_bins_value(lat_bins))
        if os_sync is not None:
            put(_lib.OPT_OS_SYNC, {"flags": 0, "barrier": 1}[os_sync] if isinstance(os_sync, str) else os_sync)
        self.nlev = self.nt = self.D = None

    def option(self, opt):
        return int(self.lib.temx_plan_option(self._h, int(opt)))

    @property
    def lat_bins(self):
        return self.option(_lib.OPT_LAT_BINS)

    @property
    def bin_degree(self):
        return self.option(_lib.OPT_BIN_DEGREE)

    @property
    def sweep_form(self):
        return _lib.FORM_NAMES.get(self.option(_lib.OPT_FORM), "two-pass")

    @property
    def missing(self):
        return "mask" if self.option(_lib.OPT_MISSING) == 1 else "raise"

    def coverage(self):
        D = getattr(self, "_cov_D", None) or self.D or 1
        out = torch.empty((self.M, D), dtype=torch.float64, device=self.device)
        check(self.lib.temx_get_matrix(self._h, _lib.MAT_COVERAGE, _ptr(out), self._stream()))
        return out

    def close(self):
        if getattr(self, "_h", None) is not None and self._h.value:
            self.lib.temx_plan_destroy(self._h)
            self._h = C.c_void_p()

    def __del__(self):
        try:
            self.close()
        except Exception:
            pass

    def _stream(self):
        return C.c_void_p(torch.cuda.current_stream(self.device).cuda_stream)

    def _field(self, A, D=None):
        if not isinstance(A, torch.Tensor):
            raise TypeError("device tensors expected")
        if A.device != self.device:
            raise ValueError("tensor on %s, plan on %s" % (A.device, self.device))
        if A.dtype not in _DT:
            raise TypeError("dtype must be float64 or float32, got %s" % A.dtype)
        if A.shape[0] != self.N:
            raise ValueError("leading dimension must be ncol = %d" % self.N)
        A = A.contiguous()
        if D is not None and A.numel() != self.N * D:
            raise ValueError("field has %d elements, expected %d x %d" % (A.numel(), self.N, D))
        return A

    def finalize(self, G=None):
        if G is None:
            check(self.lib.temx_plan_finalize(self._h, None))
        else:
            g, pg = _dbl(G)
            assert g.shape == (self.K, self.K)
            check(self.lib.temx_plan_finalize(self._h, pg))

    def refine(self, G2=None):
        if G2 is None:
            check(self.lib.temx_plan_refine(self._h, None))
        else:
            g, pg = _dbl(G2)
            assert g.shape == (self.K, self.K)
            check(self.lib.temx_plan_refine(self._h, pg))

    def set_weights(self, weights):
        w, pw = _dbl(weights)
        assert w.size == self.N
        check(self.lib.temx_plan_set_weights(self._h, pw))

    def matrix(self, which):
        shape = {_lib.MAT_Y0: (self.N, self.K), _lib.MAT_Y0P: (self.M, self.K),
                 _lib.MAT_GRAM: (self.K, self.K), _lib.MAT_GINV: (self.K, self.K),
                 _lib.MAT_GRAM2: (self.K, self.K),
                 _lib.MAT_GX: (self.K, self.KX), _lib.MAT_GSUB: (self.KR, self.KR),
                 _lib.MAT_Y0INV: (self.K, self.N)}[which]
        out = torch.empty(shape, dtype=torch.float64, device=self.device)
        check(self.lib.temx_get_matrix(self._h, which, _ptr(out), self._stream()))
        return out

    def project(self, A):
        A = self._field(A)
        D = A.numel() // self.N
        B = torch.empty((self.K, D), dtype=torch.float64, device=self.device)
        check(self.lib.temx_project(self._h, _ptr(A), _DT[A.dtype], D, _ptr(B), self._stream()))
        return B

    def zonal_mean(self, A, native=False):
        A = self._field(A)
        D = A.numel() // self.N
        out = torch.empty((self.N if native else self.M,) + tuple(A.shape[1:]), dtype=torch.float64,
                          device=self.device)
        check(self.lib.temx_zonal_mean(self._h, _ptr(A), _DT[A.dtype], D, _ptr(out), 1 if native else 0,
                                       self._stream()))
        self._cov_D = D
        return out

    def zonal_mean_from_sums(self, B, trailing_shape, native=False):
        D = int(B.shape[1])
        out = torch.empty((self.N if native else self.M,) + tuple(trailing_shape), dtype=torch.float64,
                          device=self.device)
        check(self.lib.temx_zonal_mean_from_sums(self._h, _ptr(B.contiguous()), D, _ptr(out),
                                                 1 if native else 0, self._stream()))
        return out

    def set_tem(self, nlev, nt, p_pa, p0=101325.0):
        p, pp = _dbl(p_pa)
        assert p.size == nlev
        check(self.lib.temx_plan_set_tem(self._h, int(nlev), int(nt), pp, float(p0)))
        self.nlev, self.nt, self.D = int(nlev), int(nt), int(nlev) * int(nt)
        self.tem_args = (int(nlev), int(nt), p.copy(), float(p0))

    def _four(self, ua, va, ta, wap):
        if self.D is None:
            raise _lib.TemxError(-5, "temx_plan_set_tem has not been called")
        fs = [self._field(x, self.D) for x in (ua, va, ta, wap)]
        if len({f.dtype for f in fs}) != 1:
            raise TypeError("ua, va, ta, wap must share one dtype")
        return fs, _DT[fs[0].dtype]

    def _alloc_results(self, want_zonal):
        res = torch.empty((len(_lib.RESULT_NAMES), self.M, self.nlev, self.nt), dtype=torch.float64,
                          device=self.device)
        zon = None
        if want_zonal:
            zon = torch.empty((len(_lib.ZONAL_NAMES), self.M, self.nlev, self.nt), dtype=torch.float64,
                              device=self.device)
        return res, zon

    def tem_run(self, ua, va, ta, wap, want_zonal=False, out=None):
        (u, v, t, w), dt = self._four(ua, va, ta, wap)
        res, zon = out if out is not None else self._alloc_results(want_zonal)
        check(self.lib.temx_tem_run(self._h, _ptr(u), _ptr(v), _ptr(t), _ptr(w), dt, _ptr(res),
                                    _ptr(zon) if zon is not None else None, self._stream()))
        self._cov_D = self.D
        return res, zon

    @property
    def KX(self):
        return 2 * self.L + 1

    @property
    def KR(self):
        return min(16, self.K)

    @property
    def os_rows(self):
# ... 519 lines not shown
```

Before: 192.0 billion grid-points/s.

## Shorten the single-sweep kernel chain with a fused prepass, reduce and folded solve

Adds a new "short" chain for the single-sweep pipeline, and it is the default. A dedicated column-split prepass kernel sums into per-split partials using a Legendre table. A combined reduce-and-solve kernel replaces the separate prepass reduction and reference solve. The two partial reductions are merged into one launch, and the solve and synthesis matrices (Ginv*T and Qp*Ginv*T) are precomposed on the host so the tail kernels write zonal outputs directly, skipping intermediate B3/B4 products and launches. The cost is more code paths, host-side long-double composition when the plan is built, and possible rounding differences from the folded matrices.

```diff
diff --git a/include/temx.h b/include/temx.h
--- a/include/temx.h
+++ b/include/temx.h
@@ -43,6 +43,7 @@
   TEMX_OPT_MISSING_WEIGHT = 10,
   TEMX_OPT_LAT_BINS = 12,
   TEMX_OPT_BIN_DEGREE = 13,
+  TEMX_OPT_OS_CHAIN = 14,
   TEMX_OPT_OS_SYNC = 11
 };
 enum {
diff --git a/pytemdiags_amd/_lib.py b/pytemdiags_amd/_lib.py
--- a/pytemdiags_amd/_lib.py
+++ b/pytemdiags_amd/_lib.py
@@ -19,6 +19,7 @@
 OPT_MISSING, OPT_MIN_COVERAGE, OPT_MISSING_WEIGHT = 8, 9, 10
 OPT_OS_SYNC = 11
 OPT_LAT_BINS, OPT_BIN_DEGREE = 12, 13
+OPT_OS_CHAIN = 14
 LAT_BINS_ALLOWED = (128, 256, 512, 1024, 2048)
 LAT_BINS_DEFAULT = 512
 MISSING_MODES = {"raise": 0, "mask": 1}
diff --git a/pytemdiags_amd/csrc/kernels.hpp b/pytemdiags_amd/csrc/kernels.hpp
--- a/pytemdiags_amd/csrc/kernels.hpp
+++ b/pytemdiags_amd/csrc/kernels.hpp
@@ -265,6 +265,52 @@
 #pragma unroll
   for (int sp = 0; sp < NS; ++sp) t += sp < nsplit ? v[sp] : 0.0;
   if (addend != nullptr) t += addend[idx];
+  B[slice_index(map, idx)] = t;
+  if (!(fabs(t) <= 1.79769313486231570815e308)) atomicOr(flag, 1);
+}
+
+__device__ __forceinline__ const double* reduce2_src(const double* partial, int nsplit, int64_t n1, int64_t n2, int64_t idx,
+                                                     int64_t& stride) {
+  if (idx < n1) { stride = n1; return partial + idx; }
+  stride = n2;
+  return partial + (int64_t)nsplit * n1 + (idx - n1);
+}
+__global__ void __launch_bounds__(256)
+reduce_partials2_kernel(const double* __restrict__ partial, int nsplit, int64_t n1, int64_t n2, double* __restrict__ B,
+                        int* __restrict__ flag, SliceMap map) {
+  __shared__ double sh[16][17];
+  const int e = threadIdx.x & 15, sl = threadIdx.x >> 4;
+  const int64_t idx = (int64_t)blockIdx.x * 16 + e, n = n1 + n2;
+  double s = 0.0;
+  if (idx < n) {
+    int64_t stride;
+    const double* src = reduce2_src(partial, nsplit, n1, n2, idx, stride);
+    for (int sp = sl; sp < nsplit; sp += 16) s += src[(int64_t)sp * stride];
+  }
+  sh[sl][e] = s;
+  __syncthreads();
+  if (sl == 0 && idx < n) {
+    double t = 0.0;
+#pragma unroll
+    for (int j = 0; j < 16; ++j) t += sh[j][e];
+    B[slice_index(map, idx)] = t;
+    if (!(fabs(t) <= 1.79769313486231570815e308)) atomicOr(flag, 1);
+  }
+}
+template <int NS>
+__global__ void __launch_bounds__(256)
+reduce_partials2_flat_kernel(const double* __restrict__ partial, int nsplit, int64_t n1, int64_t n2, double* __restrict__ B,
+                             int* __restrict__ flag, SliceMap map) {
+  const int64_t idx = (int64_t)blockIdx.x * 256 + threadIdx.x;
+  if (idx >= n1 + n2) return;
+  int64_t stride;
+  const double* src = reduce2_src(partial, nsplit, n1, n2, idx, stride);
+  double v[NS];
+#pragma unroll
+  for (int sp = 0; sp < NS; ++sp) v[sp] = src[(int64_t)(sp < nsplit ? sp : 0) * stride];
+  double t = 0.0;
+#pragma unroll
+  for (int sp = 0; sp < NS; ++sp) t += sp < nsplit ? v[sp] : 0.0;
   B[slice_index(map, idx)] = t;
   if (!(fabs(t) <= 1.79769313486231570815e308)) atomicOr(flag, 1);
 }
diff --git a/pytemdiags_amd/csrc/kernels_osc.hpp b/pytemdiags_amd/csrc/kernels_osc.hpp
--- a/pytemdiags_amd/csrc/kernels_osc.hpp
+++ b/pytemdiags_amd/csrc/kernels_osc.hpp
@@ -13,6 +13,9 @@
   const double* YqKt;
   const double* Yqt;
   const double* Gx;
+  const double* Mc;
+  const double* Mz;
+  const double* Mab;
 };
 
 #ifndef TEMX_OSC_PF
@@ -76,6 +79,55 @@
     }
 }
 
+template <int MC, int KI, typename Out>
+__device__ __forceinline__ void osc_mm_rows(const double* __restrict__ blk, int MO, int wave, const double* xl, int lane,
+                                            Out out) {
+  constexpr int PF = OSC_PF < KI ? OSC_PF : KI;
+  const int MO16 = (MO + 3) / 4;
+#pragma unroll 1
+  for (int base = 0; base < MO16; base += OSC_W * MC) {
+    osc_d4 acc[MC];
+    double ring[PF][MC];
+    const double* __restrict__ b[MC];
+#pragma unroll
+    for (int j = 0; j < MC; ++j) {
+      const int MB = base + wave + j * OSC_W < MO16 ? base + wave + j * OSC_W : MO16 - 1;
+      b[j] = blk + (size_t)MB * KI * 64 + lane;
+#pragma unroll
+      for (int i = 0; i < 4; ++i) acc[j][i] = 0.0;
+    }
+    static_for<PF - 1>([&](auto pc) __attribute__((always_inline)) {
+      constexpr int p = decltype(pc)::value;
+#pragma unroll
+      for (int j = 0; j < MC; ++j) ring[p][j] = b[j][p * 64];
+    });
+    auto step = [&](auto jc, int k) __attribute__((always_inline)) {
+      constexpr int r = decltype(jc)::value;
+      const int kn = k + PF - 1 < KI ? k + PF - 1 : KI - 1;
+#pragma unroll
+      for (int j = 0; j < MC; ++j) ring[(r + PF - 1) % PF][j] = b[j][kn * 64];
+      const double x = xl[k * 64];
+#pragma unroll
+      for (int j = 0; j < MC; ++j) acc[j] = __builtin_amdgcn_mfma_f64_16x16x4f64(ring[r][j], x, acc[j], 0, 0, 0);
+    };
+    constexpr int TRIPS = KI / PF, REM = KI % PF;
+#pragma unroll 1
+    for (int t = 0; t < TRIPS; ++t)
+      static_for<PF>([&](auto jc) __attribute__((always_inline)) { step(jc, t * PF + decltype(jc)::value); });
+    static_for<REM>([&](auto jc) __attribute__((always_inline)) { step(jc, TRIPS * PF + decltype(jc)::value); });
+#pragma unroll
+    for (int j = 0; j < MC; ++j)
+      if (base + wave + j * OSC_W < MO16) {
+#pragma unroll
+        for (int i = 0; i < 4; ++i) {
+          const int mb = 4 * (base + wave + j * OSC_W) + i;
+          if (mb < MO) out(mb, acc[j][i]);
+        }
+      }
+  }
+}
+constexpr int OSC_MZ_MC = 3;
+
 struct OscFieldsIn {
   const double* A[4];
   const double* rho[4];
@@ -84,11 +136,12 @@
 __host__ __device__ constexpr int osc_fields_lds(int NBK) { return (2 * NBK + 2 * NBK + 4) * 64; }
 __host__ __device__ constexpr int osc_pairs_lds(int NBK) { return (3 * 2 * NBK + 2 * NBK) * 64; }
 
-template <int NBK>
+template <int NBK, int FOLD = 0>
 __global__ void __launch_bounds__(OSC_W * 64)
 osc_fields_kernel(OscFieldsIn in, OscMats m, int K, int KX, int KR, int NQ, int64_t Dt, int nout,
                   double* __restrict__ B4 , double* __restrict__ At ,
-                  double* __restrict__ ab , int64_t Drho, int nts, int nt, int t0) {
+                  double* __restrict__ ab , int64_t Drho, int nts, int nt, int t0,
+                  int M = 0, double* __restrict__ C4 = nullptr, double* __restrict__ zb = nullptr) {
   constexpr int NBX = 2 * NBK;
   extern __shared__ double sm[];
   const int f = blockIdx.y;
@@ -118,6 +171,35 @@
   }
   __syncthreads();
   auto zero = [](int) { return 0.0; };
+  if constexpr (FOLD == 1) {
+    auto raw_sums = [&]() __attribute__((always_inline)) {
+      osc_mm<NBK, 4>(m.Gk, wave, vr, lane, [&](int mb) { return va[mb * 64]; }, [&](int mb, double v) { vt1[mb * 64] = v; });
+      __syncthreads();
+    };
+    if (blockIdx.z == 1) {
+      osc_mm<NBX, NBX>(m.Yq, wave, va, lane, zero, [&](int mb, double v) {
+        if (dvalid && 4 * mb + g < NQ) At[((int64_t)f * NQ + 4 * mb + g) * Dt + d] = v;
+      });
+    } else if (blockIdx.z == 2) {
+      if (f < nout) {
+        raw_sums();
+        osc_mm_rows<OSC_MZ_MC, NBK>(m.Mz, (M + 3) / 4, wave, vt1, lane, [&](int mb, double v) {
+          if (dvalid && 4 * mb + g < M) zb[((int64_t)f * M + 4 * mb + g) * Dt + d] = v;
+        });
+      }
+    } else {
+      osc_mm<NBX, NBK>(m.Mab, wave, va, lane, zero, [&](int mb, double v) {
+        if (dvalid && 4 * mb + g < NQ) ab[((int64_t)f * NQ + 4 * mb + g) * Dt + d] = v;
+      });
+      if (f < nout) {
+        raw_sums();
+        osc_mm<NBK, NBK>(m.Mc, wave, vt1, lane, zero, [&](int mb, double v) {
+          if (dvalid) C4[((int64_t)f * (4 * NBK) + 4 * mb + g) * Dt + d] = v;
+        });
+      }
+    }
+    return;
+  }
   if (gridDim.z == 2 && blockIdx.z == 1) {
     osc_mm<NBX, NBX>(m.Yq, wave, va, lane, zero, [&](int mb, double v) {
       if (dvalid && 4 * mb + g < NQ) At[((int64_t)f * NQ + 4 * mb + g) * Dt + d] = v;
@@ -154,10 +236,10 @@
   const double* P[4];
 };
 
-template <int NBK>
+template <int NBK, int FOLD = 0>
 __global__ void __launch_bounds__(OSC_W * 64)
 osc_pairs_kernel(OscPairsIn in, OscMats m, const double* __restrict__ wq2, int K, int KX, int NQ, int64_t Dt,
-                 double* __restrict__ B3 ) {
+                 double* __restrict__ B3 , int M = 0, double* __restrict__ zf = nullptr) {
   constexpr int NBX = 2 * NBK;
   extern __shared__ double sm[];
   const int p = blockIdx.y;
@@ -198,9 +280,15 @@
                    },
                    [&](int mb, double v) { vF[mb * 64] = v; });
   __syncthreads();
-  osc_mm<NBK, NBK>(m.Tt, wave, vF, lane, zero, [&](int mb, double v) {
-    if (dvalid && 4 * mb + g < K) B3[((int64_t)p * K + 4 * mb + g) * Dt + d] = v;
-  });
-}
-
-}
+  if constexpr (FOLD == 1) {
+    osc_mm_rows<OSC_MZ_MC, NBK>(m.Mz, (M + 3) / 4, wave, vF, lane, [&](int mb, double v) {
+      if (dvalid && 4 * mb + g < M) zf[((int64_t)p * M + 4 * mb + g) * Dt + d] = v;
+    });
+  } else {
+    osc_mm<NBK, NBK>(m.Tt, wave, vF, lane, zero, [&](int mb, double v) {
+      if (dvalid && 4 * mb + g < K) B3[((int64_t)p * K + 4 * mb + g) * Dt + d] = v;
+    });
+  }
+}
+
+}
diff --git a/pytemdiags_amd/csrc/kernels_osp.hpp b/pytemdiags_amd/csrc/kernels_osp.hpp
--- /dev/null
+++ b/pytemdiags_amd/csrc/kernels_osp.hpp
@@ -0,0 +1,144 @@
+#pragma once
+#include "kernels_op2.hpp"
+
+namespace temx {
+
+constexpr int OSP_KR = 16;
+
+template <typename T, int NF>
+__global__ void __launch_bounds__(NF * 64)
+os_prepass_kernel(FieldPtrs<NF> fp, int64_t D, int KR, const double* __restrict__ ytab ,
+                  const int4* __restrict__ crow, const int2* __restrict__ csplit, const double* __restrict__ colscale,
+                  int sfield ,
+                  double* __restrict__ partial , int nsplit, int ncw ) {
+  int split, cw;
+  if (!wg_work(ncw, nsplit, split, cw)) return;
+  const int f = uniform_wave(), lane = threadIdx.x & 63;
+  const int64_t col = (int64_t)cw * 64 + lane;
+  const bool valid = col < D;
+  const int64_t colc = valid ? col : D - 1;
+  const int b0 = __builtin_amdgcn_readfirstlane(csplit[split].x);
+  const int b1 = __builtin_amdgcn_readfirstlane(csplit[split + 1].x);
+  int grp = __builtin_amdgcn_readfirstlane(csplit[split].y);
+  const T* __restrict__ xf = static_cast<const T*>(fp.p[f]) + colc;
+
+  double acc[OSP_KR];
+  double E[4], O[4];
+#pragma unroll
+  for (int l = 0; l < OSP_KR; ++l) acc[l] = 0.0;
+#pragma unroll
+  for (int k = 0; k < 4; ++k) E[k] = O[k] = 0.0;
+  auto flush = [&]() __attribute__((always_inline)) {
+#pragma unroll
+    for (int k = 0; k < 4; ++k) {
+      const double* __restrict__ y = ytab + ((int64_t)grp * 4 + k) * OSP_KR;
+#pragma unroll
+      for (int l = 0; l < OSP_KR; ++l) acc[l] = __builtin_fma(y[l], (l & 1) ? O[k] : E[k], acc[l]);
+      E[k] = O[k] = 0.0;
+      asm volatile("" ::: "memory");
+    }
+  };
+  int4 rq[4];
+  auto fetch_rows = [&](int b) __attribute__((always_inline)) {
+#pragma unroll
+    for (int k = 0; k < 4; ++k) rq[k] = crow[(int64_t)b * 4 + k];
+  };
+  auto issue = [&](int b, T (&x)[4][CLS_MB]) __attribute__((always_inline)) {
+    int info = 0;
+    const int4 rb[4] = {rq[0], rq[1], rq[2], rq[3]};
+    fetch_rows(b + 1);
+#pragma unroll
+    for (int k = 0; k < 4; ++k) {
+      const int4 rv = rb[k];
+      const int er[CLS_MB] = {__builtin_amdgcn_readfirstlane(rv.x), __builtin_amdgcn_readfirstlane(rv.y),
+                              __builtin_amdgcn_readfirstlane(rv.z), __builtin_amdgcn_readfirstlane(rv.w)};
+      if (k == 0) info = (er[0] >> 27) & 0xF;
+#pragma unroll
+      for (int j = 0; j < CLS_MB; ++j) {
+        x[k][j] = xf[(int64_t)(er[j] & CLS_ROWMASK) * D];
+        info |= (er[j] < 0 ? 1 : 0) << (8 + k * CLS_MB + j);
+      }
+    }
+    return info;
+  };
+  bool open = false;
+  auto take = [&](int info, const T (&x)[4][CLS_MB]) __attribute__((always_inline)) {
+    const bool south = (info & (CLS_SOUTH << 1)) != 0;
+#pragma unroll
+    for (int k = 0; k < 4; ++k) {
+      double v[CLS_MB];
+#pragma unroll
+      for (int j = 0; j < CLS_MB; ++j) v[j] = ((info >> (8 + k * CLS_MB + j)) & 1) ? 0.0 : (double)x[k][j];
+      const double bs = ((v[0] + v[1]) + v[2]) + v[3];
+      E[k] += bs;
+      O[k] += south ? -bs : bs;
+    }
+    open = true;
+    if (info & (CLS_LAST << 1)) {
+      flush();
+      open = false;
+      ++grp;
+    }
+  };
+  if (b0 < b1) {
+    T xa[4][CLS_MB], xb[4][CLS_MB];
+    fetch_rows(b0);
+    int ia = issue(b0, xa), ib = 0;
+    for (int b = b0; b < b1; b += 2) {
+      ib = issue(b + 1, xb);
+      take(ia, xa);
+      if (b + 1 < b1) {
+        ia = issue(b + 2, xa);
+        take(ib, xb);
+      }
+    }
+  }
+  if (open) flush();
+  const double sth = (f == sfield && colscale != nullptr) ? colscale[colc] : 1.0;
+  if (valid) {
+#pragma unroll
+    for (int l = 0; l < OSP_KR; ++l)
+      if (l < KR) partial[(((int64_t)split * NF + f) * KR + l) * D + col] = acc[l] * sth;
+  }
+}
+
+template <int SUM, int SOLVE>
+__global__ void __launch_bounds__(256)
+os_ref_kernel(const double* __restrict__ partial, int nsplit, int nf, int KR, int64_t D, const double* __restrict__ Gsinv,
+              double* __restrict__ As, double* __restrict__ rho, int* __restrict__ flag) {
+  __shared__ double sg[16 * 16];
+  __shared__ double sa[16][17];
+  const int f = blockIdx.y;
+  const int c = threadIdx.x & 15, r = threadIdx.x >> 4;
+  const int64_t d = (int64_t)blockIdx.x * 16 + c;
+  const bool live = d < D && r < KR;
+  if constexpr (SOLVE != 0)
+    for (int i = threadIdx.x; i < KR * KR; i += 256) sg[i] = Gsinv[i];
+  double a = 0.0;
+  if (live) {
+    const int64_t o = ((int64_t)f * KR + r) * D + d;
+    if constexpr (SUM != 0) {
+      const int64_t stride = (int64_t)nf * KR * D;
+      for (int sp = 0; sp < nsplit; ++sp) a += partial[(int64_t)sp * stride + o];
+      As[o] = a;
+      if (!(fabs(a) <= 1.79769313486231570815e308)) atomicOr(flag, 1);
+    } else {
+      a = As[o];
+    }
+  }
+  if constexpr (SOLVE != 0) {
+    sa[r][c] = a;
+    __syncthreads();
+    if (!live) return;
+    double v0 = 0.0, v1 = 0.0;
+    int m = 0;
+    for (; m + 2 <= KR; m += 2) {
+      v0 = __builtin_fma(sg[r * KR + m], sa[m][c], v0);
+      v1 = __builtin_fma(sg[r * KR + m + 1], sa[m + 1][c], v1);
+    }
+    if (m < KR) v0 = __builtin_fma(sg[r * KR + m], sa[m][c], v0);
+    rho[((int64_t)f * KR + r) * D + d] = v0 + v1;
+  }
+}
+
+}
diff --git a/pytemdiags_amd/csrc/os_compose.hpp b/pytemdiags_amd/csrc/os_compose.hpp
--- /dev/null
+++ b/pytemdiags_amd/csrc/os_compose.hpp
@@ -0,0 +1,83 @@
+#pragma once
+#include <cmath>
+#include <cstddef>
+#include <vector>
+
+namespace temx {
+
+struct SolveMats {
+  std::vector<double> Mc;
+  std::vector<double> Mz;
+};
+
+inline SolveMats compose_solve(const double* Ginv, const double* T, const double* Qp, int K, int M) {
+  std::vector<long double> mc((size_t)K * K, 0.0L);
+  for (int i = 0; i < K; ++i)
+    for (int j = 0; j < K; ++j) {
+      long double s = 0.0L;
+      for (int k = 0; k < K; ++k) s += (long double)Ginv[(size_t)i * K + k] * (long double)T[(size_t)j * K + k];
+      mc[(size_t)i * K + j] = s;
+    }
+  SolveMats out;
+  out.Mc.resize((size_t)K * K);
+  out.Mz.resize((size_t)M * K);
+  for (size_t i = 0; i < mc.size(); ++i) out.Mc[i] = (double)mc[i];
+  for (int m = 0; m < M; ++m)
+    for (int j = 0; j < K; ++j) {
+      long double s = 0.0L;
+      for (int k = 0; k < K; ++k) s += (long double)Qp[(size_t)m * K + k] * mc[(size_t)k * K + j];
+      out.Mz[(size_t)m * K + j] = (double)s;
+    }
+  return out;
+}
+
+template <typename Q>
+inline std::vector<double> compose_synthesis(const double* Ginv, const double* T, const Q* Yq, int ldq, int NQ, int K) {
+  std::vector<long double> gt((size_t)K * K), a((size_t)K * K);
+  for (int i = 0; i < K; ++i)
+    for (int j = 0; j < K; ++j) {
+      long double s = 0.0L;
+      for (int k = 0; k < K; ++k) s += (long double)Ginv[(size_t)i * K + k] * (long double)T[(size_t)j * K + k];
+      gt[(size_t)i * K + j] = s;
+    }
+  for (int i = 0; i < K; ++i)
+    for (int j = 0; j < K; ++j) {
+      long double s = 0.0L;
+      for (int k = 0; k < K; ++k) s += (long double)T[(size_t)i * K + k] * gt[(size_t)k * K + j];
+      a[(size_t)i * K + j] = s;
+    }
+  std::vector<double> out((size_t)NQ * K);
+  for (int q = 0; q < NQ; ++q)
+    for (int j = 0; j < K; ++j) {
+      long double s = 0.0L;
+      for (int k = 0; k < K; ++k) s += (long double)Yq[(size_t)q * ldq + k] * a[(size_t)k * K + j];
+      out[(size_t)q * K + j] = (double)s;
+    }
+  return out;
+}
+
+inline std::vector<double> os_ytable(const std::vector<double>& xc, int KR, int stride) {
+  std::vector<double> norm((size_t)KR), tab(xc.size() * (size_t)stride, 0.0);
+  for (int l = 0; l < KR; ++l) norm[(size_t)l] = std::sqrt((2.0 * l + 1.0) / (4.0 * 3.14159265358979323846));
+  for (size_t c = 0; c < xc.size(); ++c) {
+    const double xv = xc[c];
+    double pm1 = 1.0, pc = xv;
+    for (int l = 0; l < KR; ++l) {
+      double P;
+      if (l == 0) {
+        P = 1.0;
+      } else if (l == 1) {
+        P = xv;
+      } else {
+        const double pn = ((2 * l - 1) * xv * pc - (l - 1) * pm1) / l;
+        pm1 = pc;
+        pc = pn;
+        P = pn;
+      }
+      tab[c * (size_t)stride + (size_t)l] = norm[(size_t)l] * P;
+    }
+  }
+  return tab;
+}
+
+}
diff --git a/pytemdiags_amd/csrc/temx.hip b/pytemdiags_amd/csrc/temx.hip
--- a/pytemdiags_amd/csrc/temx.hip
+++ b/pytemdiags_amd/csrc/temx.hip
@@ -32,6 +32,7 @@
 #include "kernels_op.hpp"
 #include "kernels_op2.hpp"
 #include "kernels_osc.hpp"
+#include "kernels_osp.hpp"
 #include "kernels_miss.hpp"
 #include "kernels_mtracer.hpp"
 #include "kernels_bin.hpp"
@@ -53,6 +54,7 @@
 #include "host_math.hpp"
 #include "launch_shapes.hpp"
 #include "mgclim_shapes.hpp"
+#include "os_compose.hpp"
 #include "wave_tables.hpp"
 
 using namespace temx;
@@ -161,8 +163,13 @@
   std::vector<double> h_Gx_own;
   std::vector<double> h_Gx, h_Gs;
   std::vector<double> h_T, h_Ginv, h_G, h_Yq;
+  std::vector<double> h_Qp;
   DevBuf oscblk, osAt, osAb, osAtq, osAbq, Bqp;
+  DevBuf osp_ytab;
+  Split sp_osp;
   OscMats osc{};
+  bool os_long = false;
+  int opt_os_chain = -1;
   bool osc_lds = false;
   int opt_os_contract = -1;
   bool os_barrier = false;
@@ -408,6 +415,28 @@
   return TEMX_OK;
 }
 
+static int launch_reduce2(temx_plan* pl, const double* partial, int nsplit, int64_t n1, int64_t n2, double* B, hipStream_t st,
+                          const SliceMap& map) {
+  int* flag = static_cast<int*>(pl->flag.p);
+  const int64_t n = n1 + n2;
+  if (nsplit <= 16 && n >= 32768) {
+    const dim3 grid((unsigned)((n + 255) / 256));
+    if (nsplit <= 2)
+      hipLaunchKernelGGL(reduce_partials2_flat_kernel<2>, grid, dim3(256), 0, st, partial, nsplit, n1, n2, B, flag, map);
+    else if (nsplit <= 4)
+      hipLaunchKernelGGL(reduce_partials2_flat_kernel<4>, grid, dim3(256), 0, st, partial, nsplit, n1, n2, B, flag, map);
+    else if (nsplit <= 8)
+      hipLaunchKernelGGL(reduce_partials2_flat_kernel<8>, grid, dim3(256), 0, st, partial, nsplit, n1, n2, B, flag, map);
+    else
+      hipLaunchKernelGGL(reduce_partials2_flat_kernel<16>, grid, dim3(256), 0, st, partial, nsplit, n1, n2, B, flag, map);
+  } else {
+    hipLaunchKernelGGL(reduce_partials2_kernel, dim3((unsigned)((n + 15) / 16)), dim3(256), 0, st, partial, nsplit, n1, n2, B,
+                       flag, map);
+  }
+  HIPCHK(hipGetLastError());
+  return TEMX_OK;
+}
+
 static int launch_reduce_rows(temx_plan* pl, const double* partial, int nsplit, int64_t stride, int nf, int rows_in,
                               int rows, int64_t D, double* out, hipStream_t st) {
   const int64_t n = (int64_t)nf * rows * D;
@@ -526,6 +555,10 @@
 static int os_cuts_dev(temx_plan* pl, bool sub, int nsub, const int2** out) {
   if (!sub) return class_cuts_dev(pl, nsub, out, true);
   return cached_cuts(pl->csplits_s, pl->sgbatch0, pl->sgroups, pl->sbatches, nsub, true, out);
+}
+
+static int osp_cuts_dev(temx_plan* pl, const int2** out) {
+  return cached_cuts(pl->csplits_s, pl->sgbatch0, pl->sgroups, pl->sbatches, pl->sp_osp.nsplit, false, out);
 }
 
 #ifndef TEMX_CLS_E_WPS
@@ -822,6 +855,7 @@
     }
     if ((rc = upload(pl->Gsinv, Gi))) return rc;
   }
+  if ((rc = upload(pl->osp_ytab, os_ytable(ss.xc, KR, OSP_KR)))) return rc;
   {
     const int nq = 2 * L + 2;
     pl->NQ = nq;
@@ -843,7 +877,7 @@
   const int NBK = pl->TB, NBX = 2 * pl->TBX;
   if (4 * NBK < K || 4 * NBX < KX || 4 * NBX < NQ) return fail(TEMX_EUNSUPPORTED, "single-sweep contraction: no instantiation for L = %d", pl->L);
   std::vector<double> blk;
-  size_t off[9];
+  size_t off[12] = {};
   const double* T = pl->h_T.data();
   const double* Yq = pl->h_Yq.data();
   off[0] = blk.size(); append_blocks16(blk, T, K, K, K, true, NBK, NBK);
@@ -855,10 +889,19 @@
   off[6] = blk.size(); append_blocks16(blk, Yq, K, NQ, KX, true, NBK, NBX);
   off[7] = blk.size(); append_blocks16(blk, Yq, KX, NQ, KX, true, NBX, NBX);
   off[8] = blk.size(); append_blocks16(blk, pl->h_Gx.data(), K, KX, KX, false, NBK, NBX);
+  const bool fold = pl->h_Qp.size() == (size_t)pl->M * K;
+  if (fold) {
+    const SolveMats sm = compose_solve(pl->h_Ginv.data(), T, pl->h_Qp.data(), K, pl->M);
+    off[9] = blk.size(); append_blocks16(blk, sm.Mc.data(), K, K, K, false, NBK, NBK);
+    off[10] = blk.size(); append_blocks16(blk, sm.Mz.data(), pl->M, K, K, false, (pl->M + 3) / 4, NBK);
+    const std::vector<double> mab = compose_synthesis(pl->h_Ginv.data(), T, Yq, KX, NQ, K);
+    off[11] = blk.size(); append_blocks16(blk, mab.data(), NQ, K, K, false, NBX, NBK);
+  }
   HIPCHK(hipDeviceSynchronize());
   if (int rc = upload(pl->oscblk, blk.data(), blk.size() * 8)) return rc;
   const double* b = pl->oscblk.d();
-  pl->osc = OscMats{b + off[0], b + off[1], b + off[2], b + off[3], b + off[4], b + off[5], b + off[6], b + off[7], b + off[8]};
+  pl->osc = OscMats{b + off[0], b + off[1], b + off[2], b + off[3], b + off[4], b + off[5], b + off[6], b + off[7], b + off[8],
+                    fold ? b + off[9] : nullptr, fold ? b + off[10] : nullptr, fold ? b + off[11] : nullptr};
   return TEMX_OK;
 }
 
@@ -984,10 +1027,53 @@
   return fail(TEMX_EUNSUPPORTED, "single-sweep contraction: no instantiation for L = %d", pl->L);
 }
 
+template <int NBK>
+static int launch_osc_fold_t(temx_plan* pl, const OscFieldsIn& fin, const OscPairsIn& pin, int64_t Dt, hipStream_t st) {
+  const unsigned gx = (unsigned)((Dt + 15) / 16);
+  double* zb = pl->zb.d();
+  hipLaunchKernelGGL((osc_fields_kernel<NBK, 1>), dim3(gx, 4, 3), dim3(OSC_W * 64), (size_t)osc_fields_lds(NBK) * 8, st, fin, pl->osc,
+                     pl->K, pl->KX, pl->KR, pl->NQ, Dt, 4, (double*)nullptr, pl->osAt.d(), pl->osAb.d(), pl->D, (int)pl->tnt,
+                     (int)pl->nt, (int)pl->tt0, pl->M, pl->C4.d(), zb);
+  HIPCHK(hipGetLastError());
+  hipLaunchKernelGGL((osc_pairs_kernel<NBK, 1>), dim3(gx, 3), dim3(OSC_W * 64), (size_t)osc_pairs_lds(NBK) * 8, st, pin, pl->osc,
+                     pl->wq2.d(), pl->K, pl->KX, pl->NQ, Dt, (double*)nullptr, pl->M, zb + (int64_t)4 * pl->M * Dt);
+  HIPCHK(hipGetLastError());
+  return TEMX_OK;
+}
+static int launch_osc_fold(temx_plan* pl, const OscFieldsIn& fin, const OscPairsIn& pin, int64_t Dt, hipStream_t st) {
+  if (!pl->osc.Mc || !pl->osc.Mz) return fail(TEMX_EINTERNAL, "single-sweep contraction: the composed solve matrices are not built");
+  if (pl->TB == 13 && pl->TBX == 13) return launch_osc_fold_t<13>(pl, fin, pin, Dt, st);
+  if (pl->TB == 8 && pl->TBX == 8) return launch_osc_fold_t<8>(pl, fin, pin, Dt, st);
+  if (pl->TB == 4 && pl->TBX == 4) return launch_osc_fold_t<4>(pl, fin, pin, Dt, st);
+  return fail(TEMX_EUNSUPPORTED, "single-sweep contraction: no instantiation for L = %d", pl->L);
+}
+
+static int launch_os_prepass(temx_plan* pl, const FieldPtrs<4>& fp, int dtype, hipStream_t st) {
+  const int2* cuts = nullptr;
+  if (int rc = osp_cuts_dev(pl, &cuts)) return rc;
+  const int ncw = (int)((pl->D + 63) / 64);
+  return by_dtype(dtype, [&](auto t) {
+    using T = typename decltype(t)::type;
+    return launch<os_prepass_kernel<T, 4>>(dim3(pl->sp_osp.grid), dim3(256), 0, st, fp, pl->D, pl->KR, pl->osp_ytab.d(),
+                                           static_cast<const int4*>(pl->crow_s.p), cuts, pl->colscale.d(), OsKind<0>::TF,
+                                           pl->partial.d(), pl->sp_osp.nsplit, ncw);
+  });
+}
+template <int SUM, int SOLVE>
+static int launch_os_ref(temx_plan* pl, double* As, hipStream_t st) {
+  return launch<os_ref_kernel<SUM, SOLVE>>(dim3((unsigned)((pl->D + 15) / 16), 4), dim3(256), 0, st, pl->partial.d(),
+                                           pl->sp_osp.nsplit, 4, pl->KR, pl->D, pl->Gsinv.d(), As, pl->rho.d(),
+                                           static_cast<int*>(pl->flag.p));
+}
+
 static int os_prepass(temx_plan* pl, const FieldPtrs<4>& fp, int dtype, double* As, hipStream_t st) {
   int rc;
   const int64_t D = pl->D, KD4 = (int64_t)4 * pl->KX * D;
   pl->op_valid = pl->c4_valid = pl->tq_valid = pl->os_valid = false;
+  if (!pl->os_long) {
+    if ((rc = launch_os_prepass(pl, fp, dtype, st))) return rc;
+    return launch_os_ref<1, 0>(pl, As, st);
+  }
   if ((rc = launch_sweep_os<0>(pl, fp, dtype, true, pl->rho0.d(), pl->partial.d(), pl->sp_os_s, st))) return rc;
   return launch_reduce_rows(pl, pl->partial.d(), pl->sp_os_s.nsplit, KD4, 4, pl->KX, pl->KR, D, As, st);
 }
@@ -997,15 +1083,22 @@
   const int64_t D = pl->D;
   const int64_t KD4 = (int64_t)4 * pl->KX * D, KD3 = (int64_t)3 * pl->K * D;
   pl->op_valid = pl->c4_valid = pl->tq_valid = pl->os_valid = false;
-  hipLaunchKernelGGL(os_ref_solve_kernel, dim3((unsigned)((D + 15) / 16), 4), dim3(256), 0, st, As, pl->KR, pl->KR, D,
-                     pl->Gsinv.d(), pl->rho.d());
-  HIPCHK(hipGetLastError());
+  if (As == nullptr) {
+  } else if (!pl->os_long) {
+    if ((rc = launch_os_ref<0, 1>(pl, const_cast<double*>(As), st))) return rc;
+  } else {
+    hipLaunchKernelGGL(os_ref_solve_kernel, dim3((unsigned)((D + 15) / 16), 4), dim3(256), 0, st, As, pl->KR, pl->KR, D,
+                       pl->Gsinv.d(), pl->rho.d());
+    HIPCHK(hipGetLastError());
+  }
   TimedLaunch tl{};
   time_begin(pl, 0, st, tl);
   rc = launch_sweep_os<0>(pl, fp, dtype, false, pl->rho.d(), pl->partial.d(), pl->sp_os, st);
   time_end(pl, 0, st, tl);
   if (rc) return rc;
   const int64_t rows = (int64_t)4 * pl->KX + 3 * pl->K;
+  if (!pl->os_long)
+    return launch_reduce2(pl, pl->partial.d(), pl->sp_os.nsplit, KD4, KD3, proj, st, slice_map(pl, nsl, rows, 0));
   if ((rc = launch_reduce(pl, pl->partial.d(), pl->sp_os.nsplit, KD4, proj, st, -1, nullptr, slice_map(pl, nsl, rows, 0)))) return rc;
   return launch_reduce(pl, pl->partial.d() + (int64_t)pl->sp_os.nsplit * KD4, pl->sp_os.nsplit, KD3, nsl > 1 ? proj : proj + KD4, st, -1,
                        nullptr, slice_map(pl, nsl, rows, (int64_t)4 * pl->KX));
@@ -1047,6 +1140,14 @@
         pin.ab_a[k] = pl->osAb.d() + KD::pa(k) * QD; pin.ab_b[k] = pl->osAb.d() + KD::pb(k) * QD;
         pin.P[k] = Pp + (int64_t)k * pl->K * Dt;
       }
+      if (!pl->os_long) {
+        if ((rc = launch_osc_fold(pl, fin, pin, Dt, st))) return rc;
+        time_end(pl, 1, st, t2);
+        if ((rc = tem_epilogue(pl, results, zonal, st))) return rc;
+        pl->c4_valid = true;
+        pl->os_valid = true;
+        return TEMX_OK;
+      }
       if ((rc = launch_osc(pl, fin, 4, 4, pl->B4.d(), pl->osAt.d(), pl->osAb.d(), pin, 3, pl->B3.d(), Dt, st))) return rc;
     }
     time_end(pl, 1, st, t2);
@@ -1061,6 +1162,13 @@
 static int tem_run_os(temx_plan* pl, const FieldPtrs<4>& fp, int dtype, double* results, double* zonal, void* stream) {
   hipStream_t st = S_(stream);
   int rc;
+  if (!pl->os_long) {
+    pl->op_valid = pl->c4_valid = pl->tq_valid = pl->os_valid = false;
+    if ((rc = launch_os_prepass(pl, fp, dtype, st))) return rc;
+    if ((rc = launch_os_ref<1, 1>(pl, pl->Axs.d(), st))) return rc;
+    if ((rc = os_sweep(pl, fp, dtype, nullptr, 1, pl->Ax.d(), st))) return rc;
+    return os_tail(pl, pl->Ax.d(), 0, pl->nt, results, zonal, st);
+  }
   if ((rc = os_prepass(pl, fp, dtype, pl->Axs.d(), st))) return rc;
   if ((rc = os_sweep(pl, fp, dtype, pl->Axs.d(), 1, pl->Ax.d(), st))) return rc;
   return os_tail(pl, pl->Ax.d(), 0, pl->nt, results, zonal, st);
@@ -1719,7 +1827,7 @@
   pl->ypblk.release();
   for (DevBuf* b : {&pl->T, &pl->Qp, &pl->GinvA, &pl->G2, &pl->xo, &pl->xc, &pl->ycx, &pl->ycx_s, &pl->crow_s, &pl->side_crow[0][0], &pl->side_crow[0][1], &pl->side_crow[1][0], &pl->side_crow[1][1],
                     &pl->side_gfirst[0][0], &pl->side_gfirst[0][1], &pl->side_gfirst[1][0], &pl->side_gfirst[1][1], &pl->rho,
-                    &pl->rho0, &pl->gaunt, &pl->wq2, &pl->Axq, &pl->rho_t, &pl->Gx, &pl->Gsinv, &pl->Ax, &pl->Axs, &pl->oscblk, &pl->osAt, &pl->osAb, &pl->osAtq, &pl->osAbq, &pl->Bqp})
+                    &pl->rho0, &pl->gaunt, &pl->wq2, &pl->Axq, &pl->rho_t, &pl->Gx, &pl->Gsinv, &pl->Ax, &pl->Axs, &pl->oscblk, &pl->osp_ytab, &pl->osAt, &pl->osAb, &pl->osAtq, &pl->osAbq, &pl->Bqp})
     b->release();
   for (DevBuf* b : {&pl->eblk, &pl->mtab, &pl->mB, &pl->mC, &pl->mCcov, &pl->mcov, &pl->mZ}) b->release();
   for (DevBuf* b : {&pl->mtB, &pl->mtB2, &pl->mtC, &pl->mtCcov, &pl->mtz}) b->release();
@@ -1754,6 +1862,9 @@
   if (blocks && pl->K <= 64) {
     std::vector<double> yp((size_t)pl->M * pl->K);
     HIPCHK(hipMemcpy(yp.data(), dst, yp.size() * 8, hipMemcpyDeviceToHost));
+    pl->h_Qp = yp;
+    if (pl->os_built)
+      if (int rcb = os_upload_blocks(pl)) return rcb;
     return upload(pl->ypblk, pack_blocks4(yp.data(), pl->M, pl->K, pl->TB));
   }
   return TEMX_OK;
@@ -2272,6 +2383,10 @@
   if (const char* e = getenv("TEMX_OS_SYNC")) return !strcmp(e, "barrier");
   return pl->opt_os_sync == 1;
 }
+static bool os_long_wanted(const temx_plan* pl) {
+  if (const char* e = getenv("TEMX_OS_CHAIN")) return !strcmp(e, "long");
+  return pl->opt_os_chain == 1;
+}
 static bool tracer_one_pass_wanted(const temx_plan* pl) {
   if (const char* e = getenv("TEMX_TRACER_ONE_PASS")) return e[0] == '1';
   return pl->opt_tracer_one_pass == 1;
@@ -2318,6 +2433,10 @@
       if (value != 0 && value != 1) return fail(TEMX_EINVAL, "TEMX_OPT_OS_SYNC: 0 (flags) or 1 (barriers), got %d", value);
       pl->opt_os_sync = value;
       break;
+    case TEMX_OPT_OS_CHAIN:
+      if (value != 0 && value != 1) return fail(TEMX_EINVAL, "TEMX_OPT_OS_CHAIN: 0 (short) or 1 (long), got %d", value);
+      pl->opt_os_chain = value;
+      break;
     case TEMX_OPT_LAT_BINS: {
       const int B = value == -1 ? BIN_DEFAULT : value;
       if (B != 0) {
@@ -2355,6 +2474,7 @@
     case TEMX_OPT_MIN_COVERAGE: return pl->opt_min_cov;
     case TEMX_OPT_MISSING_WEIGHT: return pl->opt_miss_w;
     case TEMX_OPT_OS_SYNC: return os_barrier_wanted(pl) ? 1 : 0;
+    case TEMX_OPT_OS_CHAIN: return os_long_wanted(pl) ? 1 : 0;
     case TEMX_OPT_LAT_BINS: return pl->opt_lat_bins;
     case TEMX_OPT_BIN_DEGREE: return pl->bin_J;
     default: return -1;
@@ -2381,6 +2501,7 @@
   }
   pl->op_tile = tile_map(pl->opt_op_map, "TEMX_OP_MAP");
   pl->os_barrier = os_barrier_wanted(pl);
+  pl->os_long = os_long_wanted(pl);
   pl->nlev = nlev;
   pl->nt = nt;
   pl->D = (int64_t)nlev * nt;
@@ -2483,8 +2604,19 @@
             if (want) {
               pl->sp_os = choose_split(D, cunits, pl->num_cu, 4, 8);
               pl->sp_os_s = choose_split(D, std::max<int64_t>(1, pl->sbatches / 4), pl->num_cu, 4, 2);
+              {
+                Split sp;
+                sp.dpw = 4;
+                sp.ndt = (int)((D + 15) / 16);
+                const int ncw = (int)((D + 63) / 64);
+                const int64_t most = std::max<int64_t>(1, std::min<int64_t>(64, pl->sbatches / 2));
+                sp.nsplit = (int)std::max<int64_t>(1, std::min<int64_t>(most, (int64_t)3 * pl->num_cu / ncw));
+                sp.grid = ((ncw * sp.nsplit + 7) / 8) * 8;
+                pl->sp_osp = sp;
+              }
               const size_t per = ((size_t)4 * pl->KX + 3 * pl->K) * D * 8;
               if ((rc = pl->partial.ensure(std::max((size_t)std::max(pl->sp_os.nsplit, pl->sp_os_s.nsplit) * per, pl->partial.bytes)))) return rc;
+              if ((rc = pl->partial.ensure(std::max((size_t)pl->sp_osp.nsplit * 4 * pl->KR * D * 8, pl->partial.bytes)))) return rc;
               if ((rc = pl->Ax.ensure(((size_t)4 * pl->KX + 3 * pl->K) * D * 8))) return rc;
               if ((rc = pl->Axs.ensure((size_t)4 * pl->KR * D * 8))) return rc;
               if ((rc = pl->osAt.ensure((size_t)4 * pl->NQ * D * 8))) return rc;
@@ -2495,6 +2627,7 @@
               const int2* cu = nullptr;
               if ((rc = os_cuts_dev(pl, false, pl->sp_os.nsplit, &cu))) return rc;
               if ((rc = os_cuts_dev(pl, true, pl->sp_os_s.nsplit, &cu))) return rc;
+              if ((rc = osp_cuts_dev(pl, &cu))) return rc;
               pl->os_on = true;
             }
           }
diff --git a/pytemdiags_amd/engine.py b/pytemdiags_amd/engine.py
--- a/pytemdiags_amd/engine.py
+++ b/pytemdiags_amd/engine.py
@@ -79,7 +79,7 @@
 
     def configure(self, form=None, os_map=None, op_map=None, os_subsample=None, tracer_one_pass=None,
                   single_sweep_min_groups=None, os_contract=None, missing=None, min_coverage=None,
-                  missing_weight=None, os_sync=None, lat_bins=None):
+                  missing_weight=None, os_sync=None, lat_bins=None, os_chain=None):
         def put(opt, val):
             check(self.lib.temx_plan_configure(self._h, opt, int(val)))
         if missing is not None:
@@ -114,6 +114,8 @@
             put(_lib.OPT_LAT_BINS, lat_bins_value(lat_bins))
         if os_sync is not None:
             put(_lib.OPT_OS_SYNC, {"flags": 0, "barrier": 1}[os_sync] if isinstance(os_sync, str) else os_sync)
+        if os_chain is not None:
+            put(_lib.OPT_OS_CHAIN, {"short": 0, "long": 1}[os_chain] if isinstance(os_chain, str) else os_chain)
         self.nlev = self.nt = self.D = None
 
     def option(self, opt):
```

Measured after the change: 192.6 billion grid-points/s (median of 2 runs). Within noise of the previous version (+0.3%).
